# dafyddstephenson/ucla-roms

Hardware: AMD Instinct MI355X
Metric: grid-cell-updates/sec (higher is better)
Workload: dtype f64; 1 GPU; C3: basin 1024x1024x100, NONLIN+SPLIT EOS, T+S, LMD KPP/BKPP/RIMIX/NONLOCAL, dt=300s, ndtfast=60 (nfast=82); NT=2, nfast=82, parallelism=domain decomposition 1x1, halo_transport=none (single rank), fast_exchange_interval=1, exchange_order=none (single rank), s2d_window=True, comm_bootstrap=none (single rank)

## Files before the change

include/roms_gpu.h:

```cpp
#ifndef ROMS_GPU_H
#define ROMS_GPU_H

#ifdef __cplusplus
extern "C" {
#endif

#define ROMS_GPU_ABI_VERSION 21
#define ROMS_MAX_FAST 288

typedef struct roms_dims {
  int Lm, Mm, N, NT;
  int LLm, MMm;
  int np_xi, np_eta, inode, jnode;
  int iSW_corn, jSW_corn;
  int ew_periodic, ns_periodic;
  int west_exchng, east_exchng, south_exchng, north_exchng;
} roms_dims;

#define ROMS_LMD_MIXING   1
#define ROMS_LMD_KPP      2
#define ROMS_LMD_BKPP     4
#define ROMS_LMD_RIMIX    8
#define ROMS_LMD_CONVEC   16
#define ROMS_LMD_NONLOCAL 32
#define ROMS_LMD_ALL      63
#define ROMS_LMD_ICELAND  47
#define ROMS_LMD_DDMIX    64

typedef struct roms_cfg {
  int nonlin_eos;
  int salinity;
  int lmd_mixing;
  int uv_vis2, ts_dif2;
  double dt;
  int ndtfast, nfast;
  double weight[2][ROMS_MAX_FAST];
  double g, rho0, rdrg, rdrg2, Zob, gamma2;
  double Akv_bak, Akt_bak[2];
  double Tcoef, T0, Scoef, S0;
  double theta_s, theta_b, hc;
  int obc;
  double ubind;
  int curvgrid;
  int uv_adv, uv_cor;
  int pot_tides;
  int bulk_frc;
  int adv_isoneutral;
} roms_cfg;

typedef struct roms_tlev {
  int iic, ntstart, forw_start, iif, nfast, kstp, knew, nstp, nrhs, nnew;
} roms_tlev;

enum roms_field {
  ROMS_ALL = -1,
  ROMS_h = 0, ROMS_hinv, ROMS_f, ROMS_fomn, ROMS_pm, ROMS_pn, ROMS_dm_r, ROMS_dn_r, ROMS_dm_u, ROMS_dn_u,
  ROMS_dm_v, ROMS_dn_v, ROMS_dm_p, ROMS_dn_p, ROMS_pmon_u, ROMS_pnom_v, ROMS_rmask, ROMS_pmask, ROMS_umask,
  ROMS_vmask,
  ROMS_Cs_w, ROMS_Cs_r,
  ROMS_zeta, ROMS_ubar, ROMS_vbar, ROMS_u, ROMS_v, ROMS_t, ROMS_FlxU, ROMS_FlxV, ROMS_We, ROMS_Wi,
  ROMS_Hz, ROMS_Hz_u, ROMS_Hz_v, ROMS_z_r, ROMS_z_w,
  ROMS_rufrc, ROMS_rvfrc, ROMS_rhoA, ROMS_rhoS, ROMS_r_D, ROMS_Zt_avg1, ROMS_DU_avg1, ROMS_DV_avg1,
  ROMS_DU_avg2, ROMS_DV_avg2, ROMS_DU_avg_bak, ROMS_DV_avg_bak,
  ROMS_rho, ROMS_rho1, ROMS_qp1, ROMS_bvf, ROMS_Akv, ROMS_Akt, ROMS_visc2_r, ROMS_visc2_p, ROMS_diff2,
  ROMS_hbls, ROMS_hbbl, ROMS_ghat, ROMS_swr_frac,
  ROMS_sustr, ROMS_svstr, ROMS_stflx, ROMS_srflx, ROMS_swflx,
  ROMS_ru, ROMS_rv,
  ROMS_zeta_west, ROMS_zeta_east, ROMS_zeta_south, ROMS_zeta_north,
  ROMS_ubar_west, ROMS_ubar_east, ROMS_ubar_south, ROMS_ubar_north,
  ROMS_vbar_west, ROMS_vbar_east, ROMS_vbar_south, ROMS_vbar_north,
  ROMS_u_west, ROMS_u_east, ROMS_u_south, ROMS_u_north,
  ROMS_v_west, ROMS_v_east, ROMS_v_south, ROMS_v_north,
  ROMS_t_west, ROMS_t_east, ROMS_t_south, ROMS_t_north,
  ROMS_dndx, ROMS_dmde,
  ROMS_ptide,
  ROMS_uwnd, ROMS_vwnd, ROMS_tair, ROMS_qair, ROMS_prate, ROMS_swrad, ROMS_lwrad, ROMS_sustr_r, ROMS_svstr_r,
  ROMS_NFIELDS
};

int  roms_gpu_abi_version(void);
int  roms_gpu_init(const roms_dims *dims, const roms_cfg *cfg, int device, void *comm);
int  roms_gpu_finalize(void);
const char *roms_gpu_last_error(void);
long roms_gpu_field_size(int field_id);
int  roms_gpu_register(int field_id, double *host_ptr, long count);
int  roms_gpu_upload(int field_id);
int  roms_gpu_download(int field_id);
int  roms_gpu_copy_in(int field_id, const double *src, long count);
int  roms_gpu_copy_out(int field_id, double *dst, long count);
int  roms_gpu_sync(void);
void *roms_gpu_stream(void);

int roms_gpu_rho_eos(int tidx, const roms_tlev *t);
int roms_gpu_set_huv(const roms_tlev *t);
int roms_gpu_omega(const roms_tlev *t);
int roms_gpu_lmd_vmix(int tind, const roms_tlev *t);
int roms_gpu_prsgrd(const roms_tlev *t);
int roms_gpu_pre_step3d(const roms_tlev *t);
int roms_gpu_set_huv1(const roms_tlev *t);
int roms_gpu_step3d_uv1(const roms_tlev *t);
int roms_gpu_visc3d(const roms_tlev *t);
int roms_gpu_step2d(const roms_tlev *t);
int roms_gpu_step3d_uv2(const roms_tlev *t);
int roms_gpu_step3d_t(const roms_tlev *t);
int roms_gpu_t3dmix(const roms_tlev *t);
int roms_gpu_swr_frac(const roms_tlev *t);
int roms_gpu_set_pipe_frc(int npip, const int *pipe_idx, const double *pipe_flx, const double *pipe_prf,
                          const double *pipe_trc);
int roms_gpu_set_river_frc(int nriv, const double *riv_uflx, const double *riv_vflx, const double *riv_vol,
                           const double *riv_trc);
int roms_gpu_bulk_flux(const roms_tlev *t);
int roms_gpu_set_ub_tune(const double *ub_west, const double *ub_east, const double *ub_south, const double *ub_north);
int roms_gpu_set_depth(const roms_tlev *t);

int roms_gpu_step(roms_tlev *t);
int roms_gpu_init_sequence(roms_tlev *t);

enum roms_case_id { ROMS_CASE_FILAMENT = 0, ROMS_CASE_BASIN = 1, ROMS_CASE_PIPES = 2, ROMS_CASE_RIVERS = 3 };
typedef struct roms_case {
  int case_id, LLm, MMm, N, NT;
  int salinity, nonlin_eos, lmd_mixing;
  double dt; int ndtfast;
  double sizex, sizey;
  int surf_flux;
  int obc;
  double v_sponge;
  int island;
  int curvgrid;
  int uv_adv, uv_cor;
  int bulk_frc;
  int adv_isoneutral;
} roms_case;
int roms_gpu_init_case(const roms_case *c, int device, roms_tlev *t);
int roms_gpu_init_case_comm(const roms_case *c, int np_xi, int np_eta, void *comm, int device, roms_tlev *t);

int roms_gpu_comm_unique_id(void *id128);
int roms_gpu_comm_create(const void *id128, int nranks, int rank, int device, void **comm);
int roms_gpu_comm_create_local(int group, int nranks, int rank, void **comm);
typedef int (*roms_host_allgather_fn)(void *ctx, const void *send, long nbytes, void *recv);
int roms_gpu_comm_create_host(int nranks, int rank, int device, roms_host_allgather_fn allgather, void *ctx,
                              void **comm);
int roms_gpu_comm_destroy(void *comm);
int roms_gpu_halo_transport(void);
int roms_gpu_halo_exchanges(long *per_step, int *fast_interval);
int roms_gpu_halo_overlap(void);
int roms_gpu_s2d_window(void);
#define ROMS_COLPATH_SEG 1
#define ROMS_COLPATH_GLOBAL 2
int roms_gpu_column_path(void);
int roms_gpu_kpp_lean(void);
int roms_gpu_vgrid(void);
int roms_gpu_vgrid2(void);
int roms_gpu_vgrid_check(long out[3]);
int roms_gpu_horizontal_path(int out[8]);
int roms_gpu_selftest_zero_fill(long n, int chunks, long *bad);
int roms_gpu_halo_plan(int Lm, int Mm, int np_xi, int np_eta, int inode, int jnode, int ew_periodic,
                       int ns_periodic, int peer[8], long count[8], int strip[4]);
long roms_gpu_halo_map(int Lm, int Mm, int np_xi, int np_eta, int inode, int jnode, int ew_periodic,
                       int ns_periodic, int dir, int unpack, int *i, int *j, long cap);
long roms_gpu_halo_map_wide(int Lm, int Mm, int np_xi, int np_eta, int inode, int jnode, int ew_periodic,
                            int ns_periodic, int width, int dir, int unpack, int *i, int *j, long cap);

#define ROMS_FRC_SURFACE 1
#define ROMS_FRC_BRY     2
int roms_gpu_frc_record(int field_id, int slot, double rec_time, const double *data);
int roms_gpu_frc_interp(double modtime, int kinds);
int roms_gpu_frc_clock(double start_time, int on);
int roms_gpu_set_tide_data(int ntides, const double *ftide, const double *pot_re, const double *pot_im,
                           const double *ztide_re, const double *ztide_im, const double *utide_re,
                           const double *utide_im, const double *vtide_re, const double *vtide_im);
int roms_gpu_set_tides(double time);

#define ROMS_WRT_Z    1
#define ROMS_WRT_UB   2
#define ROMS_WRT_VB   4
#define ROMS_WRT_U    8
#define ROMS_WRT_V    16
#define ROMS_WRT_T    32
#define ROMS_WRT_R    64
#define ROMS_WRT_O    128
#define ROMS_WRT_AKV  256
#define ROMS_WRT_AKT  512
#define ROMS_WRT_AKS  1024
#define ROMS_WRT_HBLS 2048
#define ROMS_WRT_HBBL 4096
#define ROMS_WRT_DEFAULT 63
int roms_gpu_wrt_rst(const char *path, int rec, int total_rec, double time, const roms_tlev *t);
int roms_gpu_wrt_his(const char *path, int rec, int total_rec, double time, const roms_tlev *t, int wrt_mask);
int roms_gpu_io_wait(void);
int roms_gpu_io_tracer_name(int itrc, const char *name, const char *units, const char *long_name);
int roms_gpu_get_init(const char *path, int req_rec, int tindx, roms_tlev *t, double *start_time);

int roms_gpu_diag(const roms_tlev *t, double norms[4]);
int roms_gpu_set_weights(int ndtfast, double weight[2][ROMS_MAX_FAST]);
int roms_gpu_time_steps(roms_tlev *t, int n, double *ms);
enum roms_routine {
  ROMS_R_RHO_EOS = 0, ROMS_R_SET_HUV, ROMS_R_OMEGA, ROMS_R_PRSGRD, ROMS_R_PRE_STEP3D, ROMS_R_SET_HUV1,
  ROMS_R_STEP3D_UV1, ROMS_R_VISC3D, ROMS_R_STEP2D, ROMS_R_STEP3D_UV2, ROMS_R_STEP3D_T, ROMS_R_T3DMIX,
  ROMS_R_LMD_VMIX,
  ROMS_R_K_S2D_FB,
  ROMS_R_K_PRE_UV_SEG,
  ROMS_R_K_UV1_SEG,
  ROMS_R_K_STEP3D_T_SEG,
  ROMS_R_K_PRSGRD_UV,
  ROMS_R_K_HALO_PACK,
  ROMS_R_K_HALO_WAIT,
  ROMS_R_K_HALO_UNPACK,
  ROMS_R_COUNT
};
int roms_gpu_time_routine(int routine, int nsteps, roms_tlev *t, double *avg_ms, long *launches);

#ifdef __cplusplus
}
#endif
#endif
```

ucla-roms_amd/csrc/k_colseg.h:

```cpp
#pragma once
#include "k_common.h"

namespace roms {


struct SegSpan {
  int s, S, c0, n;
  int col;
  int row;
  int l;
};
template <int CW = kSegCW>
__device__ __forceinline__ SegSpan seg_span(int N) {
  SegSpan r;
  const int t = (int)(threadIdx.x + blockDim.x * threadIdx.y);
  r.col = t % CW;
  r.row = (int)threadIdx.z;
  r.l = r.col + CW * r.row;
  r.s = t / CW;
  r.S = (int)(blockDim.x * blockDim.y) / CW;
  const int base = N / r.S, rem = N % r.S;
  r.c0 = 1 + r.s * base + min(r.s, rem);
  r.n = base + (r.s < rem ? 1 : 0);
  return r;
// ... 72 lines not shown
#ifndef ROMS_SEG_FASTDIV
#define ROMS_SEG_FASTDIV 1
#endif
#if ROMS_SEG_FASTDIV
#define SEG_DIV(a, b) ((a) * seg_rcp(b))
#else
#define SEG_DIV(a, b) ((a) / (b))
#endif

template <int KR>
struct SegTri {
  double C[KR], D[KR], E[KR];
  template <int G = kSegLoadGroup, class RowF>
  __device__ __forceinline__ void eliminate(int n, RowF row) {
    double Cp = 0.0, Dp = 0.0, Ep = 1.0;
#pragma unroll
    for (int q = 0; q < KR; q++) {
      double a, b, c, d;
      row(q, a, b, c, d);
      const double rm = seg_rcp(b - a * Cp);
      const double Cq = c * rm, Dq = (d - a * Dp) * rm, Eq = -a * Ep * rm;
      const bool live = seg_live(q, n);
      C[q] = live ? Cq : 0.0;
      D[q] = live ? Dq : 0.0;
      E[q] = live ? Eq : 0.0;
      Cp = C[q]; Dp = D[q]; Ep = E[q];
      if (q % G == G - 1) __builtin_amdgcn_sched_barrier(0);
    }
  }
  __device__ __forceinline__ void couple(const SegSpan& sp, int n, SegXchg& X, double& xL, double& xR) {
    const int s = sp.s, S = sp.S, l = sp.l;
    double y = 0.0, al = 0.0, be = 0.0, yl = 0.0, all = 0.0, bel = 0.0;
#pragma unroll
    for (int q = KR - 1; q >= 0; q--) {
      const bool last = seg_last(q, n), live = seg_live(q, n);
      const double yn = D[q] - C[q] * y, aln = E[q] - C[q] * al, ben = -C[q] * be;
      y = last ? D[q] : (live ? yn : y);
      al = last ? E[q] : (live ? aln : al);
      be = last ? -C[q] : (live ? ben : be);
      yl = last ? D[q] : yl;
      all = last ? E[q] : all;
      bel = last ? -C[q] : bel;
    }
    X.v[0][s][l] = y; X.v[1][s][l] = al; X.v[2][s][l] = be;
    X.v[3][s][l] = yl; X.v[4][s][l] = all; X.v[5][s][l] = bel;
    __syncthreads();
    double Pp = 0.0, Qp = 0.0, Ps = 0.0, Qs = 0.0, Us = 0.0, Vs = 0.0, ga = 0.0, gb = 1.0;
#pragma unroll
    for (int t = 0; t < kSegMaxS; t++) {
      if (t < S) {
        const double yf = X.v[0][t][l], af = X.v[1][t][l], bf = X.v[2][t][l];
        const double yL = X.v[3][t][l], aL = X.v[4][t][l], bL = X.v[5][t][l];
        const double rden = seg_rcp(1.0 - af * Qp);
        const double Ut = (yf + af * Pp) * rden;
        const double Vt = bf * rden;
        Us = t == s ? Ut : Us;
        Vs = t == s ? Vt : Vs;
        const double gan = ga + gb * Ut, gbn = gb * Vt;
        ga = t > s ? gan : ga;
        gb = t > s ? gbn : gb;
        const double Pn = yL + aL * Pp + aL * Qp * Ut;
        Qp = aL * Qp * Vt + bL;
        Pp = Pn;
        Ps = t == s - 1 ? Pp : Ps;
        Qs = t == s - 1 ? Qp : Qs;
      }
      if (t % kSegCoupleGroup == kSegCoupleGroup - 1) __builtin_amdgcn_sched_barrier(0);
    }
    xR = ga;
    xL = Ps + Qs * (Us + Vs * ga);
  }
  __device__ __forceinline__ void solve(int n, double xL, double xR) {
    double xn = xR;
#pragma unroll
    for (int q = KR - 1; q >= 0; q--) {
      const double v = D[q] + E[q] * xL - C[q] * xn;
      const bool live = seg_live(q, n);
      xn = live ? v : xn;
      D[q] = live ? v : D[q];
    }
  }
};

template <int KR>
__device__ __forceinline__ void spline_fc_seg(const SegSpan& sg, int N, SegXchg& X, const double (&w)[KR + 1],
                                              const double (&f)[KR], double (&fc)[KR]) {
  const int c0 = sg.c0, n = sg.n;
  const int ns = n + (sg.s == sg.S - 1 ? 1 : 0);
  SegTri<KR> T;
  T.eliminate(ns, [&](int q, double& a, double& bb, double& c, double& dd) {
    const int r = c0 - 1 + q;
    const int q1 = q + 1 < KR ? q + 1 : KR - 1;
    const double ai = w[q + 1], bi = 2.0 * (w[q] + w[q + 1]), ci = w[q];
    const double di = 3.0 * (w[q] * f[q1] + w[q + 1] * f[q]);
    a = r == 0 ? 0.0 : (r == N ? 1.0 : ai);
    bb = (r == 0 || r == N) ? 1.0 : bi;
    c = r == 0 ? 1.0 : (r == N ? 0.0 : ci);
    dd = r == 0 ? 2.0 * f[1] : (r == N ? 2.0 * f[q] : di);
  });
  double xL, xR;
  T.couple(sg, ns, X, xL, xR);
  T.solve(ns, xL, xR);
#pragma unroll
  for (int q = 0; q < KR; q++) fc[q] = seg_live(q, ns) ? T.D[q] : xR;
}

struct NoSplineRow {
  __device__ __forceinline__ void operator()(int, long, double, double, double) const {}
};
template <int KR, class RowF = NoSplineRow>
__device__ __forceinline__ void uv_spline_seg(const Dev& d, const SegSpan& sg, SegXchg& X, long ij, int nrhs, int dir,
                                              double (&fl)[KR], RowF row = RowF()) {
  const Bounds& b = d.b;
  const Fields& F = d.f;
  const int N = b.N, c0 = sg.c0, n = sg.n;
  if (!d.p.uv_adv) {
#pragma unroll
    for (int q = 0; q < KR; q++) fl[q] = 0.0;
    return;
  }
  const long n2 = b.n2, s = dir == 0 ? 1 : b.nx2;
  const double* __restrict__ Uv = (dir == 0 ? F.u : F.v) + (long)(nrhs - 1) * b.n3 + ij;
  const double* __restrict__ Hz = F.Hz + ij;
  const double* __restrict__ We = F.We + ij;
  const double* mask = dir == 0 ? F.umask : F.vmask;
  double dc[KR + 1], uu[KR];
#pragma unroll
  for (int q = 0; q < KR + 1; q++) {
    const long L = (long)(min(max(c0 - 1 + q, 1), N) - 1) * n2;
    const double h0 = Hz[L], h1 = Hz[L - s];
    dc[q] = 0.5625 * (h0 + h1) - 0.0625 * (Hz[L + s] + Hz[L - 2 * s]);
    if (q < KR) uu[q] = Uv[L];
    row(q, L, h0, h1, q < KR ? uu[q] : 0.0);
    if (q % kSegLoadGroup == kSegLoadGroup - 1) __builtin_amdgcn_sched_barrier(0);
  }
  spline_fc_seg<KR>(sg, N, X, dc, uu, fl);
  const double m1 = mask[ij + s], m0 = mask[ij - s];
  double wf[KR];
#pragma unroll
  for (int q = 0; q < KR; q++) {
    const long w = (long)min(max(c0 - 1 + q, 1), N - 1) * n2;
    wf[q] = We[w] + We[w - s] - 0.125 * ((We[w + s] - We[w]) * m1 - (We[w - s] - We[w - 2 * s]) * m0);
    if (q % kSegLoadGroup == kSegLoadGroup - 1) __builtin_amdgcn_sched_barrier(0);
  }
#pragma unroll
  for (int q = 0; q < KR; q++) pin(wf[q]);
#pragma unroll
  for (int q = 0; q < KR; q++) {
    const int r = c0 - 1 + q;
    fl[q] = (r == 0 || r == N) ? 0.0 : fl[q] * 0.5 * wf[q];
  }
}

struct NoSplineRowB {
  __device__ __forceinline__ void operator()(int, unsigned, double, double, double) const {}
};
template <int KR, class RowF = NoSplineRowB>
__device__ __forceinline__ void uv_spline_segb(const Dev& d, const SegSpan& sg, SegXchg& X, long ij, int nrhs, int dir,
                                               double (&fl)[KR], RowF row = RowF()) {
  const Bounds& b = d.b;
  const Fields& F = d.f;
  const int N = b.N, c0 = sg.c0, n = sg.n;
  if (!d.p.uv_adv) {
#pragma unroll
    for (int q = 0; q < KR; q++) fl[q] = 0.0;
    return;
  }
  const long s = dir == 0 ? 1 : b.nx2;
  const unsigned lv = (unsigned)b.n2 * 8u, vo = (unsigned)ij * 8u, ds = (unsigned)s * 8u;
  const unsigned vm = vo - ds, vp = vo + ds, vm2 = vo - 2u * ds;
  const BufF64 Uv((dir == 0 ? F.u : F.v) + (long)(nrhs - 1) * b.n3), Hz(F.Hz), We(F.We);
  const double* mask = dir == 0 ? F.umask : F.vmask;
  auto LD = [&](const BufF64& B, unsigned v, unsigned l) { return B.ld(v + l, 0u); };
  double dc[KR + 1], uu[KR];
#pragma unroll
  for (int q = 0; q < KR + 1; q++) {
    const unsigned L = (unsigned)(min(max(c0 - 1 + q, 1), N) - 1) * lv;
    const double h0 = LD(Hz, vo, L), h1 = LD(Hz, vm, L);
    dc[q] = 0.5625 * (h0 + h1) - 0.0625 * (LD(Hz, vp, L) + LD(Hz, vm2, L));
    if (q < KR) uu[q] = LD(Uv, vo, L);
    row(q, L, h0, h1, q < KR ? uu[q] : 0.0);
    if (q % kSegLoadGroup == kSegLoadGroup - 1) __builtin_amdgcn_sched_barrier(0);
  }
  spline_fc_seg<KR>(sg, N, X, dc, uu, fl);
  const double m1 = mask[ij + s], m0 = mask[ij - s];
  double wf[KR];
#pragma unroll
  for (int q = 0; q < KR; q++) {
    const unsigned w = (unsigned)min(max(c0 - 1 + q, 1), N - 1) * lv;
    const double we0 = LD(We, vo, w), wem = LD(We, vm, w);
    wf[q] = we0 + wem - 0.125 * ((LD(We, vp, w) - we0) * m1 - (wem - LD(We, vm2, w)) * m0);
    if (q % kSegLoadGroup == kSegLoadGroup - 1) __builtin_amdgcn_sched_barrier(0);
  }
#pragma unroll
  for (int q = 0; q < KR; q++) pin(wf[q]);
#pragma unroll
  for (int q = 0; q < KR; q++) {
    const int r = c0 - 1 + q;
    fl[q] = (r == 0 || r == N) ? 0.0 : fl[q] * 0.5 * wf[q];
  }
}

template <int KR>
__device__ __forceinline__ void tracer_spline_seg(const SegSpan& sg, int N, long n2, SegXchg& X,
                                                  const double (&hz)[KR + 1], const double (&tt)[KR],
                                                  const double* __restrict__ We, double (&fl)[KR]) {
  spline_fc_seg<KR>(sg, N, X, hz, tt, fl);
  double we[KR];
#pragma unroll
  for (int q = 0; q < KR; q++) we[q] = We[(long)min(max(sg.c0 - 1 + q, 1), N - 1) * n2];
#pragma unroll
  for (int q = 0; q < KR; q++) pin(we[q]);
#pragma unroll
  for (int q = 0; q < KR; q++) {
    const int r = sg.c0 - 1 + q;
    fl[q] = (r == 0 || r == N) ? 0.0 : fl[q] * we[q];
  }
}

struct SegCol {
  int i, j, dir;
  bool act, idle;
};
__device__ __forceinline__ void seg_uv_col(const Dev& d, const Range& R, const uint3& bI, const SegSpan& sg,
                                           SegCol& c) {
  const Bounds& b = d.b;
  c.dir = (int)bI.z;
  const int ilo = c.dir == 0 ? b.istrU : b.istr;
  const int jlo = c.dir == 1 ? (b.jstrV > R.j0 ? b.jstrV : R.j0) : R.j0;
  const int iu = tile_i0(R.i0) + (int)bI.x * kSegCW + sg.col;
  const int ju = R.j0 + (int)bI.y * (int)blockDim.z + sg.row;
  c.idle = R.j0 + (int)bI.y * (int)blockDim.z > R.j1;
  c.act = iu >= ilo && iu <= R.i1 && ju >= jlo && ju <= R.j1;
  c.i = iu < ilo ? ilo : (iu > R.i1 ? R.i1 : iu);
  c.j = ju < jlo ? jlo : (ju > R.j1 ? R.j1 : ju);
}
inline dim3 seg_grid_of(const Range& R, int nz, int jrows = 1) {
  return dim3((R.i1 - tile_i0(R.i0) + kSegCW) / kSegCW, (R.j1 - R.j0 + jrows) / jrows, nz);
}
inline dim3 seg_uv_grid(const Dev& d, const Range& R, int jrows) { return seg_grid_of(R, 2, jrows); }

}
```

ucla-roms_amd/csrc/k_pre_step3d.hip:

```cpp
#include "k_colseg.h"

namespace roms {

struct PreCoef {
  double dtau, cf_stp, cf_bak;
};

__global__ void __launch_bounds__(256) k_pre_tracer_h(Dev d, Range R, PreCoef c, int nstp, int nnew, int nrhs) {
  const uint3 bI = xcd_tile();
  __shared__ TracerWin W;
  const Bounds& b = d.b;
  const Fields& F = d.f;
  const int k = 1 + (int)bI.z, indx = 3 - nstp;
  const int i0 = tile_i0(R.i0) + (int)bI.x * kBX, j0 = R.j0 + (int)bI.y * kBY;
  const int ib = i0 - 2, jb = j0 - 2;
  const long kk = (long)(k - 1) * b.n2;
  tracer_win_fill(b, F, W, ib, jb, kk, nullptr);
  const int i = i0 + (int)threadIdx.x, j = j0 + (int)threadIdx.y;
  const bool act = i >= R.i0 && i <= R.i1 && j <= R.j1;
  const long ij = IJ(b, i, j), o = ij + kk;
  double hb = 0.0;
  if (act) {
    double hf;
    hz_bak_fwd(d, i, j, k, 0.5 * c.dtau, hb, hf);
    F.c2[o] = hf;
    F.c3[o] = hb;
  }
  const bool in = act && i >= b.istr && j >= b.jstr;
  const double hz = in ? F.Hz[o] : 0.0;
  const AccTL a{W.T, W.UM, W.VM, W.FU, W.FV, ib, jb};
  for (int itrc = 1; itrc <= b.NT; itrc++) {
    const long tb = (long)(itrc - 1) * 3 * b.n3;
    const double* Tr = F.t + (long)(nrhs - 1) * b.n3 + tb;
    __syncthreads();
    tracer_win_fill(b, F, W, ib, jb, kk, Tr);
    __syncthreads();
    if (!in) continue;
    double* Tn = F.t + (long)(nnew - 1) * b.n3 + tb;
    double* Ti = F.t + (long)(indx - 1) * b.n3 + tb;
    const double* Ts = F.t + (long)(nstp - 1) * b.n3 + tb;
    double FX0 = tracer_fx(b, a, i, j, false), FX1 = tracer_fx(b, a, i + 1, j, false);
    double FE0 = tracer_fe(b, a, i, j, false), FE1 = tracer_fe(b, a, i, j + 1, false);
    if (d.p.nriv > 0) {
      river_tracer_flux(d, 0, i, j, k, itrc, FX0); river_tracer_flux(d, 0, i + 1, j, k, itrc, FX1);
      river_tracer_flux(d, 1, i, j, k, itrc, FE0); river_tracer_flux(d, 1, i, j + 1, k, itrc, FE1);
    }
    const double tsk = Ts[o];
    Tn[o] = hb * (c.cf_stp * tsk + c.cf_bak * Ti[o]) - c.dtau * F.pm[ij] * F.pn[ij] * (FX1 - FX0 + FE1 - FE0);
    Ti[o] = hz * tsk;
  }
}

template <int NTT>
struct TracerWinN {
  static constexpr int kN = kUVW * (kBY + 4);
  double UM[kN], VM[kN], FU[kN], FV[kN], T[NTT][kN];
};
template <int NTT, bool kHB>
__global__ void __launch_bounds__(kBX * kBY) k_pre_tracer_h1(Dev d, Range R, PreCoef c, int nstp, int nnew, int nrhs) {
  const uint3 bI = xcd_tile();
  __shared__ TracerWinN<NTT> W;
  const Bounds& b = d.b;
  const Fields& F = d.f;
  const int k = 1 + (int)bI.z, indx = 3 - nstp;
  const int i0 = tile_i0(R.i0) + (int)bI.x * kBX, j0 = R.j0 + (int)bI.y * kBY;
  const int ib = i0 - 2, jb = j0 - 2;
  const long kk = (long)(k - 1) * b.n2, n2 = b.n2;
  const int tid = threadIdx.x + kBX * threadIdx.y;
  constexpr int NW = kUVW * (kBY + 4), NR = (NW + kBX * kBY - 1) / (kBX * kBY);
  double wUM[NR], wVM[NR], wFU[NR], wFV[NR], wT[NTT][NR];
#pragma unroll
  for (int r = 0; r < NR; r++) {
    const int q = tid + r * kBX * kBY;
    const int i = ib + q % kUVW, j = jb + q / kUVW;
    const bool ok = q < NW && i >= -1 && i <= b.Lm + 2 && j >= -1 && j <= b.Mm + 2;
    const long o = ok ? IJ(b, i, j) : 0;
    wUM[r] = ok ? F.umask[o] : 0.0;
    wVM[r] = ok ? F.vmask[o] : 0.0;
    wFU[r] = ok ? F.FlxU[o + kk] : 0.0;
    wFV[r] = ok ? F.FlxV[o + kk] : 0.0;
#pragma unroll
    for (int t = 0; t < NTT; t++)
      wT[t][r] = ok ? F.t[(long)(nrhs - 1) * b.n3 + (long)t * 3 * b.n3 + o + kk] : 0.0;
  }
  const int i = i0 + (int)threadIdx.x, j = j0 + (int)threadIdx.y;
  const bool act = i >= R.i0 && i <= R.i1 && j <= R.j1;
  const bool in = act && i >= b.istr && j >= b.jstr;
  const long ij = act ? IJ(b, i, j) : IJ(b, R.i0, R.j0), o = ij + kk, w = ij + (long)k * n2;
  const bool formed = kHB && in;
  double fu0 = 0.0, fu1 = 0.0, fv0 = 0.0, fv1 = 0.0, we1 = 0.0, wi1 = 0.0, we0 = 0.0, wi0 = 0.0, hbo = 0.0;
  if (formed) {
    hbo = F.c3[o];
  } else {
    fu0 = F.FlxU[o]; fu1 = F.FlxU[o + 1]; fv0 = F.FlxV[o]; fv1 = F.FlxV[o + b.nx2];
    we1 = F.We[w]; wi1 = F.Wi[w]; we0 = F.We[w - n2]; wi0 = F.Wi[w - n2];
  }
  const double pm = F.pm[ij], pn = F.pn[ij], hzo = F.Hz[o];
  double ts[NTT], ti[NTT];
#pragma unroll
  for (int t = 0; t < NTT; t++) {
    const long tb = (long)t * 3 * b.n3;
    ts[t] = F.t[(long)(nstp - 1) * b.n3 + tb + o];
    ti[t] = F.t[(long)(indx - 1) * b.n3 + tb + o];
  }
#pragma unroll
  for (int r = 0; r < NR; r++) {
    const int q = tid + r * kBX * kBY;
    if (q < NW) {
      W.UM[q] = wUM[r]; W.VM[q] = wVM[r]; W.FU[q] = wFU[r]; W.FV[q] = wFV[r];
#pragma unroll
      for (int t = 0; t < NTT; t++) W.T[t][q] = wT[t][r];
    }
  }
  __syncthreads();
  if (!act) return;
  double hb;
  if (formed) {
    hb = hbo;
  } else {
    const double cff = 0.5 * c.dtau;
    const double FlxDiv = cff * pm * pn * (fu1 - fu0 + fv1 - fv0 + we1 + wi1 - we0 - wi0);
    hb = hzo + FlxDiv;
    const double hf = hzo - FlxDiv;
    F.c2[o] = hf;
    F.c3[o] = hb;
  }
  if (!in) return;
  const double hz = hzo;
#pragma unroll
  for (int t = 0; t < NTT; t++) {
    const int itrc = t + 1;
    const AccTL a{W.T[t], W.UM, W.VM, W.FU, W.FV, ib, jb};
    double FX0 = tracer_fx(b, a, i, j, false), FX1 = tracer_fx(b, a, i + 1, j, false);
    double FE0 = tracer_fe(b, a, i, j, false), FE1 = tracer_fe(b, a, i, j + 1, false);
    if (d.p.nriv > 0) {
      river_tracer_flux(d, 0, i, j, k, itrc, FX0); river_tracer_flux(d, 0, i + 1, j, k, itrc, FX1);
      river_tracer_flux(d, 1, i, j, k, itrc, FE0); river_tracer_flux(d, 1, i, j + 1, k, itrc, FE1);
    }
    const long tb = (long)t * 3 * b.n3;
    const double tsk = ts[t];
    F.t[(long)(nnew - 1) * b.n3 + tb + o] =
        hb * (c.cf_stp * tsk + c.cf_bak * ti[t]) - c.dtau * pm * pn * (FX1 - FX0 + FE1 - FE0);
    F.t[(long)(indx - 1) * b.n3 + tb + o] = hz * tsk;
  }
}

template <int NTT>
struct TracerRing {
  double UM[kRingH * kUVW], VM[kRingH * kUVW], FU[kRingH * kUVW], FV[kRingH * kUVW], T[NTT][kRingH * kUVW];
};
template <int NTT, int NR>
struct TracerRows {
  double um[NR], vm[NR], fu[NR], fv[NR], t[NTT][NR];
  __device__ __forceinline__ void load(const Bounds& b, const Fields& F, int tid, int ib, int r0, int nr, long kk,
                                       long tlev) {
#pragma unroll
    for (int m = 0; m < NR; m++) {
      const int q = tid + m * kBX * kBY;
      const int i = ib + q % kUVW, j = r0 + q / kUVW;
      const bool ok = q < nr * kUVW && i >= -1 && i <= b.Lm + 2 && j >= -1 && j <= b.Mm + 2;
      const long o = ok ? IJ(b, i, j) : 0;
      um[m] = ok ? F.umask[o] : 0.0;
      vm[m] = ok ? F.vmask[o] : 0.0;
      fu[m] = ok ? F.FlxU[o + kk] : 0.0;
      fv[m] = ok ? F.FlxV[o + kk] : 0.0;
#pragma unroll
      for (int t = 0; t < NTT; t++) this->t[t][m] = ok ? F.t[tlev + (long)t * 3 * b.n3 + o + kk] : 0.0;
    }
  }
  __device__ __forceinline__ void store(TracerRing<NTT>& W, int tid, int r0, int nr, int jb) const {
#pragma unroll
    for (int m = 0; m < NR; m++) {
      const int q = tid + m * kBX * kBY;
      if (q < nr * kUVW) {
        const int s = (q % kUVW) + ((r0 + q / kUVW - jb) & (kRingH - 1)) * kUVW;
        W.UM[s] = um[m]; W.VM[s] = vm[m]; W.FU[s] = fu[m]; W.FV[s] = fv[m];
#pragma unroll
        for (int t = 0; t < NTT; t++) W.T[t][s] = this->t[t][m];
      }
    }
  }
};
template <int NTT, bool kHB>
__global__ void __launch_bounds__(kBX * kBY) k_pre_tracer_hj(Dev d, Range R, PreCoef c, int nstp, int nnew, int nrhs,
                                                           int jc) {
  const uint3 bI = xcd_tile();
  __shared__ TracerRing<NTT> W;
  const Bounds& b = d.b;
  const Fields& F = d.f;
  const int k = 1 + (int)bI.z, indx = 3 - nstp;
  const int i0 = tile_i0(R.i0) + (int)bI.x * kBX, jc0 = R.j0 + (int)bI.y * jc;
  const int jend = min(jc0 + jc - 1, R.j1);
  const int ib = i0 - 2, jb = jc0 - 2;
  const long kk = (long)(k - 1) * b.n2, n2 = b.n2, tlev = (long)(nrhs - 1) * b.n3;
  const int tid = threadIdx.x + kBX * threadIdx.y;
  constexpr int NT = kBX * kBY;
  constexpr int NR0 = (kRingH * kUVW + NT - 1) / NT, NR4 = (kBY * kUVW + NT - 1) / NT;
  struct Lane {
    double fu0, fu1, fv0, fv1, we1, wi1, we0, wi0, hbo, pm, pn, hzo, ts[NTT], ti[NTT];
  };
  const int i = i0 + (int)threadIdx.x;
  auto load_lane = [&](Lane& L, int j) {
    const bool act = i >= R.i0 && i <= R.i1 && j <= jend;
    const bool formed = kHB && act && i >= b.istr && j >= b.jstr;
    const long ij = act ? IJ(b, i, j) : IJ(b, R.i0, R.j0), o = ij + kk, w = ij + (long)k * n2;
    L.fu0 = L.fu1 = L.fv0 = L.fv1 = L.we1 = L.wi1 = L.we0 = L.wi0 = L.hbo = 0.0;
    if (formed) {
      L.hbo = F.c3[o];
// ... 411 lines not shown
}

template <class C>
__global__ void __launch_bounds__(64) k_pre_uv(Dev d, Range R, PreCoef c, int nstp, int nnew, int nrhs) {
  ROMS_IJC_OR_RETURN(R)
  col_lds_poison<C>(2, d.b.N);
  const Bounds& b = d.b;
  const long ij = IJ(b, i, j);
  const C A = ColMake<C>::at(d, 0, (int)bI.z, ij), B = ColMake<C>::at(d, 1, (int)bI.z, ij);
  if (bI.z == 0) {
    if (i >= b.istrU && i <= b.iend && j >= b.jstr && j <= b.jend) pre_uv_col(d, i, j, 0, c, nstp, nnew, nrhs, A, B);
  } else {
    if (i >= b.istr && i <= b.iend && j >= b.jstrV && j <= b.jend) pre_uv_col(d, i, j, 1, c, nstp, nnew, nrhs, A, B);
  }
}

__global__ void __launch_bounds__(kSegBlock, 2) k_pre_tracer_seg(Dev d, Range R, PreCoef c, int nnew, int nrhs) {
  const uint3 bI = seg_tile(d.p.seg_order, d.p.seg_xg);
  __shared__ SegXchg X;
  constexpr int KR = kSegRows + 1;
  const Bounds& b = d.b;
  const Fields& F = d.f;
  const int N = b.N;
  const SegSpan sg = seg_span(N);
  const int iu = tile_i0(R.i0) + (int)bI.x * kSegCW + sg.col;
  const bool act = iu >= R.i0 && iu <= R.i1;
  const int i = act ? iu : (iu < R.i0 ? R.i0 : R.i1), j = R.j0 + (int)bI.y;
  const int itrc = 1 + (int)bI.z;
  const long n2 = b.n2, ij = IJ(b, i, j);
  const int c0 = sg.c0, n = sg.n;
  auto cell = [&](int k) { return (long)(min(max(k, 1), N) - 1) * n2; };
  const double* __restrict__ Hz = F.Hz + ij;
  const double* __restrict__ Hf = F.c2 + ij;
  const long tb = (long)(itrc - 1) * 3 * b.n3;
  const double* __restrict__ Tr = F.t + (long)(nrhs - 1) * b.n3 + tb + ij;
  double* __restrict__ Tn = F.t + (long)(nnew - 1) * b.n3 + tb + ij;
  double hz[KR + 1], tt[KR], fl[KR];
#pragma unroll
  for (int q = 0; q < KR + 1; q++) {
    hz[q] = Hz[cell(c0 - 1 + q)];
    if (q < KR) tt[q] = Tr[cell(c0 - 1 + q)];
  }
  tracer_spline_seg<KR>(sg, N, n2, X, hz, tt, F.We + ij, fl);
  __builtin_amdgcn_sched_barrier(0);
#pragma unroll
  for (int q = 0; q < KR + 1; q++) hz[q] = Hf[cell(c0 - 1 + q)];
  const int iAkt = itrc < b.nTS ? itrc : b.nTS;
  const double* __restrict__ Akt = F.Akt + (long)(iAkt - 1) * b.n3w + ij;
  const double* __restrict__ Wi = F.Wi + ij;
  const double DC0 = c.dtau * F.pm[ij] * F.pn[ij];
  auto fcw = [&](int q, double& fc, double& wc) {
    const int r = c0 - 1 + q;
    const long w = (long)min(max(r, 1), N - 1) * n2;
    const bool in = r > 0 && r < N;
    const int qa = q + 1 < KR + 1 ? q + 1 : KR;
    const double f = SEG_DIV(2.0 * c.dtau * Akt[w], hz[qa] + hz[q]);
    const double wv = DC0 * Wi[w];
    fc = in ? f : 0.0;
    wc = in ? wv : 0.0;
  };
  double fcl, wcl;
  fcw(0, fcl, wcl);
  __syncthreads();
  SegTri<KR> T;
  T.eliminate(n, [&](int p, double& a, double& bb, double& cc, double& dd) {
    double fcu, wcu;
    fcw(p + 1, fcu, wcu);
    a = -(fcl + fmax0(wcl));
    bb = hz[p + 1] + fcu + fmax0(wcu) + fcl - fmin0(wcl);
    cc = -(fcu - fmin0(wcu));
    dd = Tn[cell(c0 + p)] - c.dtau * F.pm[ij] * F.pn[ij] * (fl[p + 1 < KR ? p + 1 : KR - 1] - fl[p]);
    fcl = fcu; wcl = wcu;
  });
  double xL, xR;
  T.couple(sg, n, X, xL, xR);
  T.solve(n, xL, xR);
  if (act) {
#pragma unroll
    for (int p = 0; p < KR; p++)
      if (p < n) Tn[cell(c0 + p)] = T.D[p];
  }
}

__global__ void __launch_bounds__(kSegBlock, ROMS_PRE_T_SEG_WAVES) k_pre_tracer_segb(Dev d, Range R, PreCoef c, int nnew,
                                                                                   int nrhs) {
  const uint3 bI = seg_tile(d.p.seg_order, d.p.seg_xg);
  __shared__ SegXchg X;
  constexpr int KR = kSegRows + 1;
  const Bounds& b = d.b;
  const Fields& F = d.f;
  const int N = b.N;
  const SegSpan sg = seg_span(N);
  auto LD = [&](const BufF64& B, unsigned v, unsigned l) { return B.ld(v + l, 0u); };
  const int iu = tile_i0(R.i0) + (int)bI.x * kSegCW + sg.col;
  const bool act = iu >= R.i0 && iu <= R.i1;
  const int i = act ? iu : (iu < R.i0 ? R.i0 : R.i1), j = R.j0 + (int)bI.y;
  const int itrc = 1 + (int)bI.z;
  const long n2 = b.n2, ij = IJ(b, i, j);
  const int c0 = sg.c0, n = sg.n;
  const unsigned vo = (unsigned)ij * 8u;
  auto lev = [&](int k) { return (unsigned)(min(max(k, 1), N) - 1) * (unsigned)n2 * 8u; };
  auto wlev = [&](int r) { return (unsigned)min(max(r, 1), N - 1) * (unsigned)n2 * 8u; };
  const BufF64 Hz(F.Hz), Hf(F.c2), We(F.We), Wi(F.Wi);
  const long tb = (long)(itrc - 1) * 3 * b.n3;
  const BufF64 Tr(F.t + (long)(nrhs - 1) * b.n3 + tb), Tn(F.t + (long)(nnew - 1) * b.n3 + tb);
  double hz[KR + 1], tt[KR], fl[KR];
#pragma unroll
  for (int q = 0; q < KR + 1; q++) {
    hz[q] = LD(Hz, vo, lev(c0 - 1 + q));
    if (q < KR) tt[q] = LD(Tr, vo, lev(c0 - 1 + q));
  }
  spline_fc_seg<KR>(sg, N, X, hz, tt, fl);
  {
    double we[KR];
#pragma unroll
    for (int q = 0; q < KR; q++) we[q] = LD(We, vo, wlev(c0 - 1 + q));
#pragma unroll
    for (int q = 0; q < KR; q++) pin(we[q]);
#pragma unroll
    for (int q = 0; q < KR; q++) {
      const int r = c0 - 1 + q;
      fl[q] = (r == 0 || r == N) ? 0.0 : fl[q] * we[q];
    }
  }
  __builtin_amdgcn_sched_barrier(0);
#pragma unroll
  for (int q = 0; q < KR + 1; q++) hz[q] = LD(Hf, vo, lev(c0 - 1 + q));
  const int iAkt = itrc < b.nTS ? itrc : b.nTS;
  const BufF64 Akt(F.Akt + (long)(iAkt - 1) * b.n3w);
  const BufF64 Pm(F.pm), Pn(F.pn);
  const double pm = LD(Pm, vo, 0), pn = LD(Pn, vo, 0);
  const double DC0 = c.dtau * pm * pn;
  auto fcw = [&](int q, double& fc, double& wc) {
    const int r = c0 - 1 + q;
    const unsigned w = wlev(r);
    const bool in = r > 0 && r < N;
    const int qa = q + 1 < KR + 1 ? q + 1 : KR;
    const double f = SEG_DIV(2.0 * c.dtau * LD(Akt, vo, w), hz[qa] + hz[q]);
    const double wv = DC0 * LD(Wi, vo, w);
    fc = in ? f : 0.0;
    wc = in ? wv : 0.0;
  };
  double fcl, wcl;
  fcw(0, fcl, wcl);
  __syncthreads();
  SegTri<KR> T;
  T.eliminate(n, [&](int p, double& a, double& bb, double& cc, double& dd) {
    double fcu, wcu;
    fcw(p + 1, fcu, wcu);
    a = -(fcl + fmax0(wcl));
    bb = hz[p + 1] + fcu + fmax0(wcu) + fcl - fmin0(wcl);
    cc = -(fcu - fmin0(wcu));
    dd = LD(Tn, vo, lev(c0 + p)) - c.dtau * pm * pn * (fl[p + 1 < KR ? p + 1 : KR - 1] - fl[p]);
    fcl = fcu; wcl = wcu;
  });
  double xL, xR;
  T.couple(sg, n, X, xL, xR);
  T.solve(n, xL, xR);
  const unsigned vs = act ? vo : kBufOff;
#pragma unroll
  for (int p = 0; p < KR; p++)
    if (p < n) Tn.st(T.D[p], vs + lev(c0 + p), 0u);
}

template <bool kLds>
__global__ void __launch_bounds__(kSegBlock * kSegJMax, 2) k_pre_uv_seg(Dev d, Range R, PreCoef c, int nstp, int nnew, int nrhs) {
  const uint3 bI = seg_tile(d.p.seg_order, d.p.seg_xg);
  __shared__ SegXchg X;
  constexpr int KR = kSegRows + 1;
  const Bounds& b = d.b;
  const Fields& F = d.f;
  const int N = b.N, indx = 3 - nstp;
  const SegSpan sg = seg_span(N);
  SegCol col;
  seg_uv_col(d, R, bI, sg, col);
  if (col.idle) return;
  const int dir = col.dir;
  const bool act = col.act;
  const long n2 = b.n2, ij = IJ(b, col.i, col.j), s = dir == 0 ? 1 : b.nx2;
  const int c0 = sg.c0, n = sg.n;
  auto cell = [&](int k) { return (long)(min(max(k, 1), N) - 1) * n2; };
  double* Uall = dir == 0 ? F.u : F.v;
  const int nthr = (int)(blockDim.x * blockDim.y * blockDim.z);
  const int tid = (int)(threadIdx.x + blockDim.x * (threadIdx.y + blockDim.y * threadIdx.z));
  double* const Sb = roms_smem + tid;
  double* const Su = roms_smem + (long)(KR - 1) * nthr + tid;
  double fl[KR];
  if constexpr (kLds) {
    const double* __restrict__ Uix = Uall + (long)(indx - 1) * b.n3 + ij;
    uv_spline_seg<KR>(d, sg, X, ij, nrhs, dir, fl, [&](int q, long L, double h0, double h1, double u) {
      if (q >= 1 && q < KR) {
        Sb[(q - 1) * nthr] = c.cf_stp * u + c.cf_bak * Uix[L];
        Su[(q - 1) * nthr] = 0.5 * (h0 + h1) * u;
      }
    });
  } else {
    uv_spline_seg<KR>(d, sg, X, ij, nrhs, dir, fl);
  }
  __builtin_amdgcn_sched_barrier(0);
  const double* __restrict__ rr = (dir == 0 ? F.ru : F.rv) + ij;
  const double* __restrict__ Ustp = Uall + (long)(nstp - 1) * b.n3 + ij;
  double* __restrict__ Uidx = Uall + (long)(indx - 1) * b.n3 + ij;
  double* __restrict__ Unew = Uall + (long)(nnew - 1) * b.n3 + ij;
  const double* __restrict__ Hz = F.Hz + ij;
  const double* __restrict__ Akv = F.Akv + ij;
  const double* __restrict__ Wi = F.Wi + ij;
  const double* __restrict__ Hf = F.c2 + ij;
  const double* __restrict__ Hb = F.c3 + ij;
  const double sstr = dir == 0 ? F.sustr[ij] : F.svstr[ij];
  const double DC0 = c.dtau * 0.25 * (F.pm[ij] + F.pm[ij - s]) * (F.pn[ij] + F.pn[ij - s]);
  auto rhs = [&](int p) {
    const int k = c0 + p;
    const long o = cell(k);
    const double r = k == 1 ? rr[o] - fl[1] : rr[o] - fl[p + 1 < KR ? p + 1 : KR - 1] + fl[p];
    double ub;
    if constexpr (kLds) ub = Sb[(p < KR - 1 ? p : KR - 2) * nthr];
    else ub = c.cf_stp * Ustp[o] + c.cf_bak * Uidx[o];
    const double v = 0.5 * (Hb[o] + Hb[o - s]) * ub + DC0 * r;
    return k == N ? v + c.dtau * sstr : v;
  };
  double hf[KR + 1], hfm[KR + 1];
#pragma unroll
  for (int q = 0; q < KR + 1; q++) {
    const long L = cell(c0 - 1 + q);
    hf[q] = Hf[L];
    hfm[q] = Hf[L - s];
  }
  auto fcw = [&](int q, double& fc, double& wc) {
    const int r = c0 - 1 + q;
    const long w = (long)min(max(r, 1), N - 1) * n2;
    const bool in = r > 0 && r < N;
    const int qa = q + 1 < KR + 1 ? q + 1 : KR;
    const double f = SEG_DIV(2.0 * c.dtau * (Akv[w] + Akv[w - s]), hf[qa] + hfm[qa] + hf[q] + hfm[q]);
    const double wv = DC0 * 0.5 * (Wi[w] + Wi[w - s]);
    fc = in ? f : 0.0;
    wc = in ? wv : 0.0;
  };
  const double rd = F.r_D[ij], rdm = F.r_D[ij - s];
  double fcl, wcl;
  fcw(0, fcl, wcl);
  __syncthreads();
  SegTri<KR> T;
  T.eliminate(n, [&](int p, double& a, double& bb, double& cc, double& dd) {
    double fcu, wcu;
    fcw(p + 1, fcu, wcu);
    const int k = c0 + p;
    a = -(fcl + fmax0(wcl));
    cc = -(fcu - fmin0(wcu));
    const double b1 = 0.5 * (hf[p + 1] + hfm[p + 1]) + 0.5 * c.dtau * (rd + rdm) + fcu + fmax0(wcu);
    const double bk = 0.5 * (hf[p + 1] + hfm[p + 1]) + fcl - fmin0(wcl) + fcu + fmax0(wcu);
    bb = k == 1 ? b1 : bk;
    dd = rhs(p);
    fcl = fcu; wcl = wcu;
  });
  double xL, xR;
  T.couple(sg, n, X, xL, xR);
  T.solve(n, xL, xR);
  if (act) {
    double uix[KR];
#pragma unroll
    for (int p = 0; p < KR; p++) {
      const long o = cell(c0 + p);
      if constexpr (kLds) uix[p] = Su[(p < KR - 1 ? p : KR - 2) * nthr];
      else uix[p] = 0.5 * (Hz[o] + Hz[o - s]) * Ustp[o];
    }
#pragma unroll
    for (int p = 0; p < KR; p++)
      if (p < n) {
        Unew[cell(c0 + p)] = T.D[p];
        Uidx[cell(c0 + p)] = uix[p];
      }
  }
}

__global__ void __launch_bounds__(kSegBlock * kSegJMax, 2) k_pre_uv_segb(Dev d, Range R, PreCoef c, int nstp, int nnew,
                                                                         int nrhs) {
  const uint3 bI = seg_tile(d.p.seg_order, d.p.seg_xg);
  __shared__ SegXchg X;
  constexpr int KR = kSegRows + 1;
  const Bounds& b = d.b;
  const Fields& F = d.f;
  const int N = b.N, indx = 3 - nstp;
  const SegSpan sg = seg_span(N);
  auto LD = [&](const BufF64& B, unsigned v, unsigned l) { return B.ld(v + l, 0u); };
  SegCol col;
  seg_uv_col(d, R, bI, sg, col);
  if (col.idle) return;
  const int dir = col.dir;
  const bool act = col.act;
  const long n2 = b.n2, ij = IJ(b, col.i, col.j), s = dir == 0 ? 1 : b.nx2;
  const int c0 = sg.c0, n = sg.n;
  const unsigned lv = (unsigned)n2 * 8u, vo = (unsigned)ij * 8u, vm = vo - (unsigned)s * 8u;
  auto lev = [&](int k) { return (unsigned)(min(max(k, 1), N) - 1) * lv; };
  double* Uall = dir == 0 ? F.u : F.v;
  const int nthr = (int)(blockDim.x * blockDim.y * blockDim.z);
  const int tid = (int)(threadIdx.x + blockDim.x * (threadIdx.y + blockDim.y * threadIdx.z));
  double* const Sb = roms_smem + tid;
  double* const Su = roms_smem + (long)(KR - 1) * nthr + tid;
  const BufF64 Uix(Uall + (long)(indx - 1) * b.n3), Unew(Uall + (long)(nnew - 1) * b.n3), Hf(F.c2);
  double hf[KR + 1], hfm[KR + 1];
  double fl[KR];
  uv_spline_segb<KR>(d, sg, X, ij, nrhs, dir, fl, [&](int q, unsigned L, double h0, double h1, double u) {
    if (q >= 1 && q < KR) {
      Sb[(q - 1) * nthr] = c.cf_stp * u + c.cf_bak * LD(Uix, vo, L);
      Su[(q - 1) * nthr] = 0.5 * (h0 + h1) * u;
    }
  });
  __builtin_amdgcn_sched_barrier(0);
  const BufF64 rr(dir == 0 ? F.ru : F.rv), Akv(F.Akv), Wi(F.Wi), Hb(F.c3);
  const double sstr = dir == 0 ? F.sustr[ij] : F.svstr[ij];
  const double DC0 = c.dtau * 0.25 * (F.pm[ij] + F.pm[ij - s]) * (F.pn[ij] + F.pn[ij - s]);
  auto rhs = [&](int p) {
    const int k = c0 + p;
    const unsigned o = lev(k);
    const double rro = LD(rr, vo, o);
    const double r = k == 1 ? rro - fl[1] : rro - fl[p + 1 < KR ? p + 1 : KR - 1] + fl[p];
    const double ub = Sb[(p < KR - 1 ? p : KR - 2) * nthr];
    const double v = 0.5 * (LD(Hb, vo, o) + LD(Hb, vm, o)) * ub + DC0 * r;
    return k == N ? v + c.dtau * sstr : v;
  };
#pragma unroll
  for (int q = 0; q < KR + 1; q++) {
    const unsigned L = lev(c0 - 1 + q);
    hf[q] = LD(Hf, vo, L);
    hfm[q] = LD(Hf, vm, L);
  }
  auto fcw = [&](int q, double& fc, double& wc) {
    const int r = c0 - 1 + q;
    const unsigned w = (unsigned)min(max(r, 1), N - 1) * lv;
    const bool in = r > 0 && r < N;
    const int qa = q + 1 < KR + 1 ? q + 1 : KR;
    const double f = SEG_DIV(2.0 * c.dtau * (LD(Akv, vo, w) + LD(Akv, vm, w)), hf[qa] + hfm[qa] + hf[q] + hfm[q]);
    const double wv = DC0 * 0.5 * (LD(Wi, vo, w) + LD(Wi, vm, w));
    fc = in ? f : 0.0;
    wc = in ? wv : 0.0;
  };
  const double rd = F.r_D[ij], rdm = F.r_D[ij - s];
  double fcl, wcl;
  fcw(0, fcl, wcl);
  __syncthreads();
  SegTri<KR> T;
  T.eliminate(n, [&](int p, double& a, double& bb, double& cc, double& dd) {
    double fcu, wcu;
    fcw(p + 1, fcu, wcu);
    const int k = c0 + p;
    a = -(fcl + fmax0(wcl));
    cc = -(fcu - fmin0(wcu));
    const double b1 = 0.5 * (hf[p + 1] + hfm[p + 1]) + 0.5 * c.dtau * (rd + rdm) + fcu + fmax0(wcu);
    const double bk = 0.5 * (hf[p + 1] + hfm[p + 1]) + fcl - fmin0(wcl) + fcu + fmax0(wcu);
    bb = k == 1 ? b1 : bk;
    dd = rhs(p);
    fcl = fcu; wcl = wcu;
  });
  double xL, xR;
  T.couple(sg, n, X, xL, xR);
  T.solve(n, xL, xR);
  const unsigned vs = act ? vo : kBufOff;
#pragma unroll
  for (int p = 0; p < KR; p++)
    if (p < n) {
      const unsigned o = lev(c0 + p);
      Unew.st(T.D[p], vs + o, 0u);
      Uix.st(Su[(p < KR - 1 ? p : KR - 2) * nthr], vs + o, 0u);
    }
}

static size_t pre_uv_seg_lds_bytes(unsigned nthr) {
  return (size_t)2 * kSegRows * nthr * sizeof(double);
}
void setup_pre_uv_seg() {
  (void)hipFuncSetAttribute((const void*)k_pre_uv_seg<true>, hipFuncAttributeMaxDynamicSharedMemorySize,
                            (int)pre_uv_seg_lds_bytes(kSegBlock * kSegJMax));
  (void)hipFuncSetAttribute((const void*)k_pre_uv_segb, hipFuncAttributeMaxDynamicSharedMemorySize,
                            (int)pre_uv_seg_lds_bytes(kSegBlock * kSegJMax));
}

void setup_column_kernels_t(size_t bytes);
void setup_column_kernels_uv1(size_t bytes);
bool setup_column_kernels(int N) {
  const size_t bytes = col_lds_bytes(2, N);
  if (bytes > 160 * 1024) return false;
  if (bytes > 64 * 1024) {
    (void)hipFuncSetAttribute((const void*)k_pre_tracer_v<ColLds>, hipFuncAttributeMaxDynamicSharedMemorySize,
                              (int)bytes);
    (void)hipFuncSetAttribute((const void*)k_pre_uv<ColLds>, hipFuncAttributeMaxDynamicSharedMemorySize, (int)bytes);
    setup_column_kernels_t(bytes);
    setup_column_kernels_uv1(bytes);
  }
  return true;
}

double pre_step3d_dtau(const Dev& d, const Tlev& t) {
  const double AM3_crv = 1.0 / 6.0;
  return t.iic == t.forw_start ? 0.5 * d.p.dt : d.p.dt * (1.0 - AM3_crv);
}

void launch_pre_step3d(const Dev& d, hipStream_t s, const Tlev& t, bool uv_done, bool hb_done, const Side* side) {
  const Bounds& b = d.b;
  PreCoef c;
  const double AM3_crv = 1.0 / 6.0;
  if (t.iic == t.forw_start) { c.dtau = 0.5 * d.p.dt; c.cf_stp = 1.0; c.cf_bak = 0.0; }
  else { c.dtau = d.p.dt * (1.0 - AM3_crv); c.cf_stp = 0.5 + AM3_crv; c.cf_bak = 0.5 - AM3_crv; }
  c.dtau = pre_step3d_dtau(d, t);
  hb_done = hb_done && d.p.hoist && b.NT <= 2;
  Range RI{b.istr, b.iend, b.jstr, b.jend};
  Range RH{b.istr - 1, b.iend, b.jstr - 1, b.jend};
  auto horiz_tiles = [&](const Range& rh) {
    const dim3 gh = grid3_of(rh, b.N), bh(kBX, kBY);
    if (d.p.hoist && d.p.h_jc > 0 && (b.NT == 1 || b.NT == 2)) {
      const dim3 g = grid3_jc(rh, b.N, d.p.h_jc);
      const int jc = d.p.h_jc;
      if (b.NT == 2 && hb_done)
        hipLaunchKernelGGL((k_pre_tracer_hj<2, true>), g, bh, 0, s, d, rh, c, t.nstp, t.nnew, t.nrhs, jc);
      else if (b.NT == 2)
        hipLaunchKernelGGL((k_pre_tracer_hj<2, false>), g, bh, 0, s, d, rh, c, t.nstp, t.nnew, t.nrhs, jc);
      else if (hb_done)
        hipLaunchKernelGGL((k_pre_tracer_hj<1, true>), g, bh, 0, s, d, rh, c, t.nstp, t.nnew, t.nrhs, jc);
      else
        hipLaunchKernelGGL((k_pre_tracer_hj<1, false>), g, bh, 0, s, d, rh, c, t.nstp, t.nnew, t.nrhs, jc);
    } else if (d.p.hoist && b.NT == 2 && hb_done)
      hipLaunchKernelGGL((k_pre_tracer_h1<2, true>), gh, bh, 0, s, d, rh, c, t.nstp, t.nnew, t.nrhs);
    else if (d.p.hoist && b.NT == 2)
      hipLaunchKernelGGL((k_pre_tracer_h1<2, false>), gh, bh, 0, s, d, rh, c, t.nstp, t.nnew, t.nrhs);
    else if (d.p.hoist && b.NT == 1 && hb_done)
      hipLaunchKernelGGL((k_pre_tracer_h1<1, true>), gh, bh, 0, s, d, rh, c, t.nstp, t.nnew, t.nrhs);
    else if (d.p.hoist && b.NT == 1)
      hipLaunchKernelGGL((k_pre_tracer_h1<1, false>), gh, bh, 0, s, d, rh, c, t.nstp, t.nnew, t.nrhs);
    else
      hipLaunchKernelGGL(k_pre_tracer_h, gh, bh, 0, s, d, rh, c, t.nstp, t.nnew, t.nrhs);
  };
  {
    int jA = 0, jB = -1;
    if (d.p.hoist && d.p.h_jc == 0 &&
        launch_tracer_strip(d, s, RH, 1, false, hb_done, t.nnew, t.nrhs, c.dtau, c.cf_stp, c.cf_bak, t.nstp, jA, jB)) {
      if (jA > RH.j0) horiz_tiles(Range{RH.i0, RH.i1, RH.j0, jA - 1});
      if (jB < RH.j1) horiz_tiles(Range{RH.i0, RH.i1, jB + 1, RH.j1});
    } else {
      horiz_tiles(RH);
    }
  }
  hipStream_t st = s;
  if (side) {
    (void)hipEventRecord(side->efork, s);
    (void)hipStreamWaitEvent(side->s2, side->efork, 0);
    st = side->s2;
  }
  dim3 gt = gridc_of(RI);
  gt.z = b.NT;
  if (d.p.colseg && d.p.seg_buf)
    hipLaunchKernelGGL(k_pre_tracer_segb, seg_grid_of(RI, b.NT), dim3(kCX, seg_waves(b.N)), 0, st, d, RI, c, t.nnew,
                       t.nrhs);
  else if (d.p.colseg)
    hipLaunchKernelGGL(k_pre_tracer_seg, seg_grid_of(RI, b.NT), dim3(kCX, seg_waves(b.N)), 0, st, d, RI, c, t.nnew,
                       t.nrhs);
  else if ((d.p.colreg & 2) && b.N == 50 && !d.f.colscr)
    hipLaunchKernelGGL(k_pre_tracer_v_reg<50>, gt, dim3(kCX), col_lds_bytes(1, 50), st, d, RI, c, t.nnew, t.nrhs);
  else if (d.f.colscr)
    hipLaunchKernelGGL(k_pre_tracer_v<ColGlb>, gt, dim3(kCX), 0, st, d, RI, c, t.nnew, t.nrhs);
  else
    hipLaunchKernelGGL(k_pre_tracer_v<ColLds>, gt, dim3(kCX), col_lds_bytes(2, b.N), st, d, RI, c, t.nnew, t.nrhs);
  for (int itrc = 1; itrc <= b.NT && side; itrc++) launch_t3dbc(d, st, t, itrc);
  if (side) launch_exchange_tracers(d, st, t.nnew);
  if (!uv_done) launch_uv_horiz(d, s, t.nrhs, 0);
  Range Rd{b.istrU - 1, b.iend, b.jstrV - 1, b.jend};
  hipLaunchKernelGGL(k_rd, grid_of(Rd), dim3(kBX, kBY), 0, s, d, Rd, t.nstp);
  dim3 gu = gridc_of(RI);
  gu.z = 2;
  if (d.p.colseg) {
    const dim3 gs = seg_uv_grid(d, RI, d.p.seg_jrows), bs(kCX, seg_waves(b.N), d.p.seg_jrows);
    const bool lds = d.p.preuv_lds && d.p.uv_adv && t.nrhs == t.nstp;
    ktimer_mark(s, kTimedPreUvSeg, 0);
    if (lds && d.p.seg_buf)
      hipLaunchKernelGGL(k_pre_uv_segb, gs, bs, pre_uv_seg_lds_bytes(bs.x * bs.y * bs.z), s, d, RI, c, t.nstp, t.nnew,
                         t.nrhs);
    else if (lds)
      hipLaunchKernelGGL(k_pre_uv_seg<true>, gs, bs, pre_uv_seg_lds_bytes(bs.x * bs.y * bs.z), s, d, RI, c, t.nstp,
                         t.nnew, t.nrhs);
    else
      hipLaunchKernelGGL(k_pre_uv_seg<false>, gs, bs, 0, s, d, RI, c, t.nstp, t.nnew, t.nrhs);
    ktimer_mark(s, kTimedPreUvSeg, 1, 1);
  }
  else if (d.f.colscr)
    hipLaunchKernelGGL(k_pre_uv<ColGlb>, gu, dim3(kCX), 0, s, d, RI, c, t.nstp, t.nnew, t.nrhs);
  else
    hipLaunchKernelGGL(k_pre_uv<ColLds>, gu, dim3(kCX), col_lds_bytes(2, b.N), s, d, RI, c, t.nstp, t.nnew, t.nrhs);
  launch_river_uv(d, s, t.nnew, 1);
  launch_u3dbc(d, s, t);
  launch_v3dbc(d, s, t);
  if (side) {
    (void)hipEventRecord(side->ejoin, st);
    (void)hipStreamWaitEvent(s, side->ejoin, 0);
    return;
  }
  for (int itrc = 1; itrc <= b.NT; itrc++) launch_t3dbc(d, s, t, itrc);
  launch_exchange_tracers(d, s, t.nnew);
}

}
```

ucla-roms_amd/csrc/k_step3d_t.hip:

```cpp
#include "k_colseg.h"

namespace roms {

__global__ void __launch_bounds__(256) k_step3d_t_h(Dev d, Range R, int nnew, int nrhs, int up) {
  const uint3 bI = xcd_tile();
  __shared__ TracerWin W;
  const Bounds& b = d.b;
  const Fields& F = d.f;
  const int k = 1 + (int)bI.z;
  const int i0 = tile_i0(R.i0) + (int)bI.x * kBX, j0 = R.j0 + (int)bI.y * kBY;
  const int ib = i0 - 2, jb = j0 - 2;
  const long kk = (long)(k - 1) * b.n2;
  tracer_win_fill(b, F, W, ib, jb, kk, nullptr);
  const int i = i0 + (int)threadIdx.x, j = j0 + (int)threadIdx.y;
  const bool act = i >= R.i0 && i <= R.i1 && j <= R.j1;
  const long ij = IJ(b, i, j), o = ij + kk;
  const AccTL a{W.T, W.UM, W.VM, W.FU, W.FV, ib, jb};
  for (int itrc = 1; itrc <= b.NT; itrc++) {
    const long tb = (long)(itrc - 1) * 3 * b.n3;
    const double* Tr = F.t + (long)(nrhs - 1) * b.n3 + tb;
    __syncthreads();
    tracer_win_fill(b, F, W, ib, jb, kk, Tr);
    __syncthreads();
    if (!act) continue;
// ... 231 lines not shown
  const double stf = F.stflx[ij + (long)(itrc - 1) * n2];
  double rhs[KR];
#pragma unroll
  for (int p = 0; p < KR; p++) rhs[p] = Tn[cell(c0 + p)] - dt * F.pm[ij] * F.pn[ij] * (tt[p + 1 < KR ? p + 1 : KR - 1] - tt[p]);
  if (P.npip > 0) {
    const int pidx = F.pipe_idx[ij];
    if (pidx > 0) {
      const double pflx = F.pipe_flx[ij], ptrc = F.pipe_trc[(pidx - 1) + (itrc - 1) * P.npip];
#pragma unroll
      for (int p = 0; p < KR; p++) {
        const int k = min(c0 + p, N);
        rhs[p] = rhs[p] + dt * F.pm[ij] * F.pn[ij] * pflx * F.pipe_prf[(pidx - 1) + (k - 1) * P.npip] * ptrc;
      }
    }
  }
  {
    const bool top = last;
    double t = 0.0;
#pragma unroll
    for (int p = 0; p < KR; p++) t = p == n - 1 ? rhs[p] : t;
    const double swf = F.swflx[ij], hzN = Hz[cell(N)];
    if (itrc == 1) t = t + dt * swf * (P.bulk_frc ? F.tair[ij] : t / hzN);
    t = t + dt * stf;
#pragma unroll
    for (int p = 0; p < KR; p++) rhs[p] = (top && p == n - 1) ? t : rhs[p];
  }
  if (kppT || kppS) {
    auto gh = [&](long o) { return P.lmd_nonlocal ? F.ghat[ij + o] : 0.0; };
#pragma unroll
    for (int p = 0; p < KR; p++) {
      const int k = min(c0 + p, N);
      const long ou = (long)min(k, N - 1) * n2, ol = (long)max(k - 1, 1) * n2;
      double t = rhs[p];
      if (kppT) {
        const double up = dt * (sr * F.swr_frac[ij + ou] - gh(ou) * (stf - sr));
        const double lo = dt * (sr * F.swr_frac[ij + ol] - gh(ol) * (stf - sr));
        t = k <= N - 1 ? t + up : t;
        t = k >= 2 ? t - lo : t;
      } else {
        const double up = -dt * F.ghat[ij + ou] * stf, lo = -dt * F.ghat[ij + ol] * stf;
        t = k <= N - 1 ? t + up : t;
        t = k >= 2 ? t - lo : t;
      }
      rhs[p] = t;
    }
  }
  auto fcw = [&](int q, double& fc, double& wc) {
    const int r = c0 - 1 + q;
    const long w = (long)min(max(r, 1), N - 1) * n2;
    const bool in = r > 0 && r < N;
    const int qa = q + 1 < KR + 1 ? q + 1 : KR;
    const double f = SEG_DIV(2.0 * dt * Akt[w], hz[q] + hz[qa]);
    const double c = DC0 * Wi[w];
    fc = in ? f : 0.0;
    wc = in ? c : 0.0;
  };
  double fcl, wcl;
  fcw(0, fcl, wcl);
  __syncthreads();
  SegTri<KR> T;
  T.eliminate(n, [&](int p, double& a, double& bb, double& c, double& dd) {
    double fcu, wcu;
    fcw(p + 1, fcu, wcu);
    a = -(fcl + fmax0(wcl));
    bb = hz[p + 1] + fcu + fmax0(wcu) + fcl - fmin0(wcl);
    c = -(fcu - fmin0(wcu));
    dd = rhs[p];
    fcl = fcu; wcl = wcu;
  });
  double xL, xR;
  T.couple(sg, n, X, xL, xR);
  T.solve(n, xL, xR);
  if (act) {
    const double rm = F.rmask[ij];
#pragma unroll
    for (int p = 0; p < KR; p++)
      if (p < n) Tn[cell(c0 + p)] = T.D[p] * rm;
  }
}

#ifndef ROMS_SEG_T_GROUP
#define ROMS_SEG_T_GROUP kSegLoadGroup
#endif
__global__ void __launch_bounds__(kSegBlock, ROMS_T_SEG_WAVES) k_step3d_t_segb(Dev d, Range R, int nnew, int nrhs) {
  const uint3 bI = seg_tile(d.p.seg_order, d.p.seg_xg);
  __shared__ SegXchg X;
  constexpr int KR = kSegRows + 1;
  const Bounds& b = d.b;
  const Fields& F = d.f;
  const Params& P = d.p;
  const int N = b.N;
  const double dt = P.dt;
  const SegSpan sg = seg_span(N);
  auto LD = [&](const BufF64& B, unsigned v, unsigned l) { return B.ld(v + l, 0u); };
  const int iu = tile_i0(R.i0) + (int)bI.x * kSegCW + sg.col;
  const bool act = iu >= R.i0 && iu <= R.i1;
  const int i = act ? iu : (iu < R.i0 ? R.i0 : R.i1), j = R.j0 + (int)bI.y;
  const int itrc = 1 + (int)bI.z;
  const long n2 = b.n2, ij = IJ(b, i, j);
  const int c0 = sg.c0, n = sg.n;
  const bool last = sg.s == sg.S - 1;
  const unsigned vo = (unsigned)ij * 8u;
  auto lev = [&](int k) { return (unsigned)(min(max(k, 1), N) - 1) * (unsigned)n2 * 8u; };
  auto wlev = [&](int r, int lo, int hi) { return (unsigned)min(max(r, lo), hi) * (unsigned)n2 * 8u; };
  const BufF64 Hz(F.Hz), We(F.We), Wi(F.Wi);
  const BufF64 Tr(F.t + (long)(nrhs - 1) * b.n3 + (long)(itrc - 1) * 3 * b.n3);
  const BufF64 Tn(F.t + (long)(nnew - 1) * b.n3 + (long)(itrc - 1) * 3 * b.n3);
  double hz[KR + 1], tt[KR], tn[KR];
#pragma unroll
  for (int q = 0; q < KR + 1; q++) {
    hz[q] = LD(Hz, vo, lev(c0 - 1 + q));
    if (q < KR) tt[q] = LD(Tr, vo, lev(c0 - 1 + q));
  }
#pragma unroll
  for (int p = 0; p < KR; p++) tn[p] = LD(Tn, vo, lev(c0 + p));
  {
    double fc[KR];
    spline_fc_seg<KR>(sg, N, X, hz, tt, fc);
    double we[KR];
#pragma unroll
    for (int q = 0; q < KR; q++) we[q] = LD(We, vo, wlev(c0 - 1 + q, 1, N - 1));
#pragma unroll
    for (int q = 0; q < KR; q++) pin(we[q]);
#pragma unroll
    for (int q = 0; q < KR; q++) {
      const int r = c0 - 1 + q;
      tt[q] = (r == 0 || r == N) ? 0.0 : fc[q] * we[q];
    }
  }
  __builtin_amdgcn_sched_barrier(0);
  const int iAkt = itrc < b.nTS ? itrc : b.nTS;
  const BufF64 Akt(F.Akt + (long)(iAkt - 1) * b.n3w);
  const BufF64 Pm(F.pm), Pn(F.pn);
  const double pm = Pm.ld(vo, 0), pn = Pn.ld(vo, 0);
  const double DC0 = dt * pm * pn;
  const bool kppT = P.lmd && itrc == 1, kppS = P.lmd_nonlocal && itrc == 2 && P.salinity;
  const double sr = BufF64(F.srflx).ld(vo, 0);
  const double stf = BufF64(F.stflx).ld(vo, (unsigned)(itrc - 1) * (unsigned)n2 * 8u);
  double rhs[KR];
#pragma unroll
  for (int p = 0; p < KR; p++)
    rhs[p] = tn[p] - dt * pm * pn * (tt[p + 1 < KR ? p + 1 : KR - 1] - tt[p]);
  if (P.npip > 0) {
    const int pidx = F.pipe_idx[ij];
    if (pidx > 0) {
      const double pflx = F.pipe_flx[ij], ptrc = F.pipe_trc[(pidx - 1) + (itrc - 1) * P.npip];
#pragma unroll
      for (int p = 0; p < KR; p++) {
        const int k = min(c0 + p, N);
        rhs[p] = rhs[p] + dt * pm * pn * pflx * F.pipe_prf[(pidx - 1) + (k - 1) * P.npip] * ptrc;
      }
    }
  }
  if (last) {
    double t = 0.0;
#pragma unroll
    for (int p = 0; p < KR; p++) t = p == n - 1 ? rhs[p] : t;
    if (itrc == 1) {
      const double swf = BufF64(F.swflx).ld(vo, 0);
      t = t + dt * swf * (P.bulk_frc ? BufF64(F.tair).ld(vo, 0) : t / LD(Hz, vo, lev(N)));
    }
    t = t + dt * stf;
#pragma unroll
    for (int p = 0; p < KR; p++) rhs[p] = p == n - 1 ? t : rhs[p];
  }
  if (kppT || kppS) {
    const BufF64 Sw(F.swr_frac), Gh(F.ghat);
    const bool nl = P.lmd_nonlocal;
    double swv[KR + 1], ghv[KR + 1];
    if (kppT) {
#pragma unroll
      for (int q = 0; q < KR + 1; q++) {
        const unsigned o = wlev(c0 - 1 + q, 1, N - 1);
        swv[q] = LD(Sw, vo, o);
        ghv[q] = LD(Gh, vo, o);
      }
    } else {
#pragma unroll
      for (int q = 0; q < KR + 1; q++) {
        swv[q] = 0.0;
        ghv[q] = LD(Gh, vo, wlev(c0 - 1 + q, 1, N - 1));
      }
    }
    auto term = [&](int q) {
      return kppT ? dt * (sr * swv[q] - (nl ? ghv[q] : 0.0) * (stf - sr)) : -dt * ghv[q] * stf;
    };
    double lo = term(0);
#pragma unroll
    for (int p = 0; p < KR; p++) {
      const int k = min(c0 + p, N);
      const double up = term(p + 1);
      double t = rhs[p];
      t = k <= N - 1 ? t + up : t;
      t = k >= 2 ? t - lo : t;
      rhs[p] = t;
      lo = up;
    }
  }
  auto fcw = [&](int q, double& fc, double& wc) {
    const int r = c0 - 1 + q;
    const unsigned w = wlev(r, 1, N - 1);
    const bool in = r > 0 && r < N;
    const int qa = q + 1 < KR + 1 ? q + 1 : KR;
    const double f = SEG_DIV(2.0 * dt * LD(Akt, vo, w), hz[q] + hz[qa]);
    const double c = DC0 * LD(Wi, vo, w);
    fc = in ? f : 0.0;
    wc = in ? c : 0.0;
  };
  double fcl, wcl;
  fcw(0, fcl, wcl);
  __syncthreads();
  SegTri<KR> T;
  T.template eliminate<ROMS_SEG_T_GROUP>(n, [&](int p, double& a, double& bb, double& c, double& dd) {
    double fcu, wcu;
    fcw(p + 1, fcu, wcu);
    a = -(fcl + fmax0(wcl));
    bb = hz[p + 1] + fcu + fmax0(wcu) + fcl - fmin0(wcl);
    c = -(fcu - fmin0(wcu));
    dd = rhs[p];
    fcl = fcu; wcl = wcu;
  });
  double xL, xR;
  T.couple(sg, n, X, xL, xR);
  T.solve(n, xL, xR);
  const double rm = BufF64(F.rmask).ld(vo, 0);
  const unsigned vs = act ? vo : kBufOff;
#pragma unroll
  for (int p = 0; p < KR; p++) Tn.st(T.D[p] * rm, (p < n ? vs : kBufOff) + lev(c0 + p), 0u);
}

void setup_column_kernels_t(size_t bytes) {
  (void)hipFuncSetAttribute((const void*)k_step3d_t_v<ColLds>, hipFuncAttributeMaxDynamicSharedMemorySize,
                            (int)bytes);
  (void)hipFuncSetAttribute((const void*)k_step3d_t_v<ColLds, true>, hipFuncAttributeMaxDynamicSharedMemorySize,
                            (int)bytes);
}

void launch_step3d_t(const Dev& d, hipStream_t s, const Tlev& t, bool exchange) {
  const Bounds& b = d.b;
  Range R{b.istr, b.iend, b.jstr, b.jend};
  if (d.p.iso) {
    hipLaunchKernelGGL(k_step3d_t_h, grid3_of(R, b.N), dim3(kBX, kBY), 0, s, d, R, t.nnew, t.nrhs, 0);
    for (int itrc = 1; itrc <= b.NT; itrc++) launch_iso_tracer(d, s, t, itrc);
    dim3 gt = gridc_of(R);
    gt.z = b.NT;
    if (d.f.colscr)
      hipLaunchKernelGGL((k_step3d_t_v<ColGlb, true>), gt, dim3(kCX), 0, s, d, R, t.nnew, t.nrhs);
    else
      hipLaunchKernelGGL((k_step3d_t_v<ColLds, true>), gt, dim3(kCX), col_lds_bytes(2, b.N), s, d, R, t.nnew, t.nrhs);
    for (int itrc = 1; itrc <= b.NT; itrc++) launch_t3dbc(d, s, t, itrc);
    launch_exchange_tracers(d, s, t.nnew);
    return;
  }
  auto h_tiles = [&](const Range& r) {
    const dim3 gh = grid3_of(r, b.N), bh(kBX, kBY);
    if (d.p.hoist && b.NT == 2)
      hipLaunchKernelGGL(k_step3d_t_h1<2>, gh, bh, 0, s, d, r, t.nnew, t.nrhs);
    else if (d.p.hoist && b.NT == 1)
      hipLaunchKernelGGL(k_step3d_t_h1<1>, gh, bh, 0, s, d, r, t.nnew, t.nrhs);
    else
      hipLaunchKernelGGL(k_step3d_t_h, gh, bh, 0, s, d, r, t.nnew, t.nrhs, 1);
  };
  auto run = [&](const Range& r) {
    int jA = 0, jB = -1;
    if (d.p.hoist && launch_tracer_strip(d, s, r, 0, true, false, t.nnew, t.nrhs, 0.0, 0.0, 0.0, 0, jA, jB)) {
      if (jA > r.j0) h_tiles(Range{r.i0, r.i1, r.j0, jA - 1});
      if (jB < r.j1) h_tiles(Range{r.i0, r.i1, jB + 1, r.j1});
    } else {
      h_tiles(r);
    }
    dim3 gt = gridc_of(r);
    gt.z = b.NT;
    if (d.p.colseg) {
      ktimer_mark(s, kTimedStep3dTSeg, 0);
      if (d.p.seg_buf)
        hipLaunchKernelGGL(k_step3d_t_segb, seg_grid_of(r, b.NT), dim3(kCX, seg_waves(b.N)), 0, s, d, r, t.nnew, t.nrhs);
      else
        hipLaunchKernelGGL(k_step3d_t_seg, seg_grid_of(r, b.NT), dim3(kCX, seg_waves(b.N)), 0, s, d, r, t.nnew, t.nrhs);
      ktimer_mark(s, kTimedStep3dTSeg, 1, 1);
    }
    else if (d.f.colscr)
      hipLaunchKernelGGL(k_step3d_t_v<ColGlb>, gt, dim3(kCX), 0, s, d, r, t.nnew, t.nrhs);
    else
      hipLaunchKernelGGL(k_step3d_t_v<ColLds>, gt, dim3(kCX), col_lds_bytes(2, b.N), s, d, r, t.nnew, t.nrhs);
  };
  auto edges = [&] {
    for (int itrc = 1; itrc <= b.NT; itrc++) launch_t3dbc(d, s, t, itrc);
  };
  ExchList L;
  if (!exchange) {
    run(R);
    edges();
  } else if (tracer_exch_list(d, t.nnew, L)) {
    launch_rim_first(d, s, R, L, run, edges);
  } else {
    run(R);
    edges();
    launch_exchange_tracers(d, s, t.nnew);
  }
}

__global__ void __launch_bounds__(256) k_t3dmix(Dev d, Range R, int nnew, int nrhs) {
  ROMS_IJ_OR_RETURN(R)
  const Bounds& b = d.b;
  const Fields& F = d.f;
  const long ij = IJ(b, i, j), sj = b.nx2, n2 = b.n2;
  const double* __restrict__ Hz = F.Hz;
  const double pmn = d.p.dt * F.pm[ij] * F.pn[ij];
  if (b.NT == 2) {
    double ax0[2], ax1[2], ay0[2], ay1[2];
    const double* __restrict__ Tr[2];
    double* __restrict__ Tn[2];
#pragma unroll
    for (int q = 0; q < 2; q++) {
      const double* d2 = F.diff2 + (long)q * n2;
      Tr[q] = F.t + (long)(nrhs - 1) * b.n3 + (long)q * 3 * b.n3;
      Tn[q] = F.t + (long)(nnew - 1) * b.n3 + (long)q * 3 * b.n3;
      ax0[q] = 0.25 * (d2[ij] + d2[ij - 1]) * F.pmon_u[ij];
      ax1[q] = 0.25 * (d2[ij + 1] + d2[ij]) * F.pmon_u[ij + 1];
      ay0[q] = 0.25 * (d2[ij] + d2[ij - sj]) * F.pnom_v[ij];
      ay1[q] = 0.25 * (d2[ij + sj] + d2[ij]) * F.pnom_v[ij + sj];
    }
    const double um0 = F.umask[ij], um1 = F.umask[ij + 1], vm0 = F.vmask[ij], vm1 = F.vmask[ij + sj];
#pragma unroll 2
    for (int k = 1; k <= b.N; k++) {
      const long o = ij + (long)(k - 1) * n2;
#pragma unroll
      for (int q = 0; q < 2; q++) {
        const double FX1 = ax1[q] * (Hz[o + 1] + Hz[o]) * (Tr[q][o + 1] - Tr[q][o]) * um1;
        const double FX0 = ax0[q] * (Hz[o] + Hz[o - 1]) * (Tr[q][o] - Tr[q][o - 1]) * um0;
        const double FE1 = ay1[q] * (Hz[o + sj] + Hz[o]) * (Tr[q][o + sj] - Tr[q][o]) * vm1;
        const double FE0 = ay0[q] * (Hz[o] + Hz[o - sj]) * (Tr[q][o] - Tr[q][o - sj]) * vm0;
        Tn[q][o] = Tn[q][o] + pmn * (FX1 - FX0 + FE1 - FE0) / Hz[o];
      }
    }
    return;
  }
  for (int itrc = 1; itrc <= b.NT; itrc++) {
    const double* d2 = F.diff2 + (long)(itrc - 1) * n2;
    const double* __restrict__ Tr = F.t + (long)(nrhs - 1) * b.n3 + (long)(itrc - 1) * 3 * b.n3;
    double* __restrict__ Tn = F.t + (long)(nnew - 1) * b.n3 + (long)(itrc - 1) * 3 * b.n3;
    const double ax0 = 0.25 * (d2[ij] + d2[ij - 1]) * F.pmon_u[ij], ax1 = 0.25 * (d2[ij + 1] + d2[ij]) * F.pmon_u[ij + 1];
    const double ay0 = 0.25 * (d2[ij] + d2[ij - sj]) * F.pnom_v[ij], ay1 = 0.25 * (d2[ij + sj] + d2[ij]) * F.pnom_v[ij + sj];
    const double um0 = F.umask[ij], um1 = F.umask[ij + 1], vm0 = F.vmask[ij], vm1 = F.vmask[ij + sj];
#pragma unroll 2
    for (int k = 1; k <= b.N; k++) {
      const long o = ij + (long)(k - 1) * n2;
      const double FX1 = ax1 * (Hz[o + 1] + Hz[o]) * (Tr[o + 1] - Tr[o]) * um1;
      const double FX0 = ax0 * (Hz[o] + Hz[o - 1]) * (Tr[o] - Tr[o - 1]) * um0;
      const double FE1 = ay1 * (Hz[o + sj] + Hz[o]) * (Tr[o + sj] - Tr[o]) * vm1;
      const double FE0 = ay0 * (Hz[o] + Hz[o - sj]) * (Tr[o] - Tr[o - sj]) * vm0;
      Tn[o] = Tn[o] + pmn * (FX1 - FX0 + FE1 - FE0) / Hz[o];
    }
  }
}

constexpr int kTMW = kBX + 2, kTMN = kTMW * (kBY + 2), kTMQ = (3 * kTMN + kBX * kBY - 1) / (kBX * kBY);
constexpr int kTMG = (kTMN + kBX * kBY - 1) / (kBX * kBY);
template <bool VG>
// ... 119 lines not shown
```

ucla-roms_amd/csrc/k_step3d_uv.hip:

```cpp
#include <vector>

#include "k_colseg.h"
#include "k_chain.h"

namespace roms {

void launch_uv_horiz(const Dev& d, hipStream_t s, int nrhs, int up);

#ifndef ROMS_UV1_PF
#define ROMS_UV1_PF 8
#endif
constexpr int kUv1PF = ROMS_UV1_PF;
template <class C>
__device__ __forceinline__ void uv1_col(const Dev& d, int i, int j, int dir, int nnew, int nrhs, const C& A,
                                        const C& B) {
  const Bounds& b = d.b;
  const Fields& F = d.f;
  const int N = b.N;
  const double dt = d.p.dt;
  const long n2 = b.n2, ij = IJ(b, i, j);
  const long s = dir == 0 ? 1 : b.nx2;
  uv_vert_flux_lds<(kUv1PF > 0)>(d, ij, nrhs, dir, A, B);
  double* __restrict__ Un = (dir == 0 ? F.u : F.v) + (long)(nnew - 1) * b.n3 + ij;
  double* __restrict__ rr = (dir == 0 ? F.ru : F.rv) + ij;
// ... 160 lines not shown
  if constexpr (!kLds) {
#pragma unroll
    for (int q = 0; q < KR + 1; q++) {
      const long L = cell(c0 - 1 + q);
      hz[q] = Hz[L];
      hzm[q] = Hz[L - s];
    }
  }
  int tl = tid;
  __asm__ volatile("" : "+v"(tl));
  auto HZ = [&](int q) { if constexpr (kLds) return roms_smem[tl + q * nthr]; else return hz[q]; };
  auto HZM = [&](int q) { if constexpr (kLds) return roms_smem[(KR + 1 + q) * nthr + tl]; else return hzm[q]; };
  auto fcw = [&](int q, double& fc, double& wc) {
    const int r = c0 - 1 + q;
    const long w = (long)min(max(r, 1), N - 1) * n2;
    const bool in = r > 0 && r < N;
    const int qa = q + 1 < KR + 1 ? q + 1 : KR;
    const double f = SEG_DIV(2.0 * dt * (Akv[w] + Akv[w - s]), HZ(qa) + HZM(qa) + HZ(q) + HZM(q));
    const double wv = DC0 * 0.5 * (Wi[w] + Wi[w - s]);
    fc = in ? f : 0.0;
    wc = in ? wv : 0.0;
  };
  const double rD = F.r_D[ij], rDm = F.r_D[ij - s];
  double fcl, wcl;
  fcw(0, fcl, wcl);
  __syncthreads();
  SegTri<KR> T;
  T.eliminate(n, [&](int p, double& a, double& bb, double& cc, double& dd) {
    double fcu, wcu;
    fcw(p + 1, fcu, wcu);
    const int k = c0 + p;
    a = -(fcl + fmax0(wcl));
    cc = -(fcu - fmin0(wcu));
    const double b1 = 0.5 * (HZ(p + 1) + HZM(p + 1)) + 0.5 * dt * (rD + rDm) + fcu + fmax0(wcu);
    const double bk = 0.5 * (HZ(p + 1) + HZM(p + 1)) + fcl - fmin0(wcl) + fcu + fmax0(wcu);
    bb = k == 1 ? b1 : bk;
    if constexpr (kLds) {
      const double v = Un[cell(k)] + DC0 * rk[p];
      dd = k == N ? v + dt * sstr : v;
    } else {
      dd = rhs[p];
    }
    fcl = fcu; wcl = wcu;
  });
  double xL, xR;
  T.couple(sg, n, X, xL, xR);
  T.solve(n, xL, xR);
  const double dmdn = dir == 0 ? F.dm_u[ij] * F.dn_u[ij] : F.dm_v[ij] * F.dn_v[ij];
  if constexpr (kLds) {
    const int S = sg.S, sl = sg.l;
    for (int t = 0; t < S; t++) {
      if (sg.s == t) {
        double frc;
        if (t == 0) frc = rk[0] + dmdn * (sstr - 0.5 * (rDm + rD) * T.D[0]);
        else frc = Lf[t - 1][sl] + rk[0];
#pragma unroll
        for (int p = 1; p < KR; p++) frc = p < n ? frc + rk[p] : frc;
        Lf[t][sl] = frc;
      }
      __syncthreads();
    }
    if (!act) return;
#pragma unroll
    for (int p = 0; p < KR; p++)
      if (p < n) Un[cell(c0 + p)] = T.D[p] * 0.5 * (HZ(p + 1) + HZM(p + 1));
    if (sg.s == 0) {
      if (dir == 0) F.rufrc[ij] = Lf[S - 1][sl];
      else F.rvfrc[ij] = Lf[S - 1][sl];
    }
  } else {
    if (!act) return;
#pragma unroll
    for (int p = 0; p < KR; p++)
      if (p < n) Un[cell(c0 + p)] = T.D[p] * 0.5 * (hz[p + 1] + hzm[p + 1]);
    if (sg.s == 0) {
      double frc = Sr[sg.l] + dmdn * (sstr - 0.5 * (rDm + rD) * T.D[0]);
      for (int k = 2; k <= N; k++) frc = frc + Sr[(k - 1) * ncol + sg.l];
      if (dir == 0) F.rufrc[ij] = frc;
      else F.rvfrc[ij] = frc;
    }
  }
}

__global__ void __launch_bounds__(kSegBlock * kSegJMax, 2) k_uv1_segb(Dev d, Range R, int nnew, int nrhs) {
  const uint3 bI = seg_tile(d.p.seg_order, d.p.seg_xg);
  __shared__ SegXchg X;
  __shared__ double Lf[kSegMaxS][kSegCW * kSegJMax];
  constexpr int KR = kSegRows + 1;
  const Bounds& b = d.b;
  const Fields& F = d.f;
  const int N = b.N;
  const double dt = d.p.dt;
  const SegSpan sg = seg_span(N);
  SegCol col;
  seg_uv_col(d, R, bI, sg, col);
  if (col.idle) return;
  const int dir = col.dir;
  const bool act = col.act;
  const long n2 = b.n2, ij = IJ(b, col.i, col.j), s = dir == 0 ? 1 : b.nx2;
  const int c0 = sg.c0, n = sg.n;
  const unsigned lv = (unsigned)n2 * 8u, vo = (unsigned)ij * 8u, vm = vo - (unsigned)s * 8u;
  auto lev = [&](int k) { return (unsigned)(min(max(k, 1), N) - 1) * lv; };
  const int nthr = (int)(blockDim.x * blockDim.y * blockDim.z);
  const int tid = (int)(threadIdx.x + blockDim.x * (threadIdx.y + blockDim.y * threadIdx.z));
  double* const Sh = roms_smem + tid;
  double* const Shm = roms_smem + (long)(KR + 1) * nthr + tid;
  const BufF64 Un((dir == 0 ? F.u : F.v) + (long)(nnew - 1) * b.n3);
  auto LD = [&](const BufF64& B, unsigned v, unsigned l) { return B.ld(v + l, 0u); };
  double fl[KR];
  uv_spline_segb<KR>(d, sg, X, ij, nrhs, dir, fl, [&](int q, unsigned, double h0, double h1, double) {
    Sh[q * nthr] = h0;
    Shm[q * nthr] = h1;
  });
  __builtin_amdgcn_sched_barrier(0);
  const BufF64 rr(dir == 0 ? F.ru : F.rv), Akv(F.Akv), Wi(F.Wi);
  const double sstr = dir == 0 ? F.sustr[ij] : F.svstr[ij];
  const double DC0 = dt * 0.25 * (F.pm[ij] + F.pm[ij - s]) * (F.pn[ij] + F.pn[ij - s]);
  double rk[KR];
#pragma unroll
  for (int p = 0; p < KR; p++) {
    const int k = c0 + p;
    const double rro = LD(rr, vo, lev(k));
    rk[p] = k == 1 ? rro - fl[1] : rro - fl[p + 1 < KR ? p + 1 : KR - 1] + fl[p];
  }
  int tl = tid;
  __asm__ volatile("" : "+v"(tl));
  auto HZ = [&](int q) { return roms_smem[tl + q * nthr]; };
  auto HZM = [&](int q) { return roms_smem[(KR + 1 + q) * nthr + tl]; };
  auto fcw = [&](int q, double& fc, double& wc) {
    const int r = c0 - 1 + q;
    const unsigned w = (unsigned)min(max(r, 1), N - 1) * lv;
    const bool in = r > 0 && r < N;
    const int qa = q + 1 < KR + 1 ? q + 1 : KR;
    const double f = SEG_DIV(2.0 * dt * (LD(Akv, vo, w) + LD(Akv, vm, w)), HZ(qa) + HZM(qa) + HZ(q) + HZM(q));
    const double wv = DC0 * 0.5 * (LD(Wi, vo, w) + LD(Wi, vm, w));
    fc = in ? f : 0.0;
    wc = in ? wv : 0.0;
  };
  const double rD = F.r_D[ij], rDm = F.r_D[ij - s];
  double fcl, wcl;
  fcw(0, fcl, wcl);
  __syncthreads();
  SegTri<KR> T;
  T.eliminate(n, [&](int p, double& a, double& bb, double& cc, double& dd) {
    double fcu, wcu;
    fcw(p + 1, fcu, wcu);
    const int k = c0 + p;
    a = -(fcl + fmax0(wcl));
    cc = -(fcu - fmin0(wcu));
    const double b1 = 0.5 * (HZ(p + 1) + HZM(p + 1)) + 0.5 * dt * (rD + rDm) + fcu + fmax0(wcu);
    const double bk = 0.5 * (HZ(p + 1) + HZM(p + 1)) + fcl - fmin0(wcl) + fcu + fmax0(wcu);
    bb = k == 1 ? b1 : bk;
    const double v = LD(Un, vo, lev(k)) + DC0 * rk[p];
    dd = k == N ? v + dt * sstr : v;
    fcl = fcu; wcl = wcu;
  });
  double xL, xR;
  T.couple(sg, n, X, xL, xR);
  T.solve(n, xL, xR);
  const double dmdn = dir == 0 ? F.dm_u[ij] * F.dn_u[ij] : F.dm_v[ij] * F.dn_v[ij];
  const int S = sg.S, sl = sg.l;
  for (int t = 0; t < S; t++) {
    if (sg.s == t) {
      double frc;
      if (t == 0) frc = rk[0] + dmdn * (sstr - 0.5 * (rDm + rD) * T.D[0]);
      else frc = Lf[t - 1][sl] + rk[0];
#pragma unroll
      for (int p = 1; p < KR; p++) frc = p < n ? frc + rk[p] : frc;
      Lf[t][sl] = frc;
    }
    __syncthreads();
  }
#pragma unroll
  for (int p = 0; p < KR; p++)
    if (p < n) Un.st(T.D[p] * 0.5 * (HZ(p + 1) + HZM(p + 1)), act ? vo + lev(c0 + p) : kBufOff, 0u);
  if (act && sg.s == 0) {
    if (dir == 0) F.rufrc[ij] = Lf[S - 1][sl];
    else F.rvfrc[ij] = Lf[S - 1][sl];
  }
}

void setup_column_kernels_uv1(size_t bytes) {
  (void)hipFuncSetAttribute((const void*)k_uv1<ColLds>, hipFuncAttributeMaxDynamicSharedMemorySize, (int)bytes);
}
static size_t uv1_seg_lds_bytes(unsigned nthr) { return (size_t)2 * (kSegRows + 2) * nthr * sizeof(double); }
void setup_uv1_seg() {
  (void)hipFuncSetAttribute((const void*)k_uv1_seg<false>, hipFuncAttributeMaxDynamicSharedMemorySize,
                            (int)((size_t)kSegRows * kSegMaxS * kSegCW * kSegJMax * sizeof(double)));
  (void)hipFuncSetAttribute((const void*)k_uv1_seg<true>, hipFuncAttributeMaxDynamicSharedMemorySize,
                            (int)uv1_seg_lds_bytes(kSegBlock * kSegJMax));
  (void)hipFuncSetAttribute((const void*)k_uv1_segb, hipFuncAttributeMaxDynamicSharedMemorySize,
                            (int)uv1_seg_lds_bytes(kSegBlock * kSegJMax));
}

void launch_step3d_uv1(const Dev& d, hipStream_t s, const Tlev& t, bool uv_done) {
  const Bounds& b = d.b;
  if (!uv_done) launch_uv_horiz(d, s, t.nrhs, 1);
  Range R{b.istr, b.iend, b.jstr, b.jend};
  dim3 g = gridc_of(R);
  g.z = 2;
  if (d.p.colseg) {
    const dim3 gs = seg_uv_grid(d, R, d.p.seg_jrows), bs(kCX, seg_waves(b.N), d.p.seg_jrows);
    ktimer_mark(s, kTimedUv1Seg, 0);
    if (d.p.uv1_lds && d.p.uv_adv && d.p.seg_buf)
      hipLaunchKernelGGL(k_uv1_segb, gs, bs, uv1_seg_lds_bytes(bs.x * bs.y * bs.z), s, d, R, t.nnew, t.nrhs);
    else if (d.p.uv1_lds && d.p.uv_adv)
      hipLaunchKernelGGL(k_uv1_seg<true>, gs, bs, uv1_seg_lds_bytes(bs.x * bs.y * bs.z), s, d, R, t.nnew, t.nrhs);
    else
      hipLaunchKernelGGL(k_uv1_seg<false>, gs, bs, (size_t)b.N * kSegCW * d.p.seg_jrows * sizeof(double), s, d, R,
                         t.nnew, t.nrhs);
    ktimer_mark(s, kTimedUv1Seg, 1, 1);
  }
  else if (d.f.colscr)
    hipLaunchKernelGGL(k_uv1<ColGlb>, g, dim3(kCX), 0, s, d, R, t.nnew, t.nrhs);
  else
    hipLaunchKernelGGL(k_uv1<ColLds>, g, dim3(kCX), col_lds_bytes(2, b.N), s, d, R, t.nnew, t.nrhs);
}

__device__ __forceinline__ void visc_rho(const Dev& d, int i, int j, int k, int nstp, double& UFx, double& VFe) {
  const Bounds& b = d.b;
  const Fields& F = d.f;
  const long ij = IJ(b, i, j), o = ij + (long)(k - 1) * b.n2, l = (long)(nstp - 1) * b.n3;
  const double* pm = F.pm;
  const double* pn = F.pn;
  const long sj = b.nx2;
  const double cff = 0.5 * F.Hz[o] * F.visc2_r[ij] *
                     (F.dn_r[ij] * pm[ij] * ((pn[ij] + pn[ij + 1]) * F.u[o + 1 + l] - (pn[ij - 1] + pn[ij]) * F.u[o + l]) -
                      F.dm_r[ij] * pn[ij] * ((pm[ij] + pm[ij + sj]) * F.v[o + sj + l] - (pm[ij - sj] + pm[ij]) * F.v[o + l]));
  UFx = cff * F.dn_r[ij] * F.dn_r[ij];
  VFe = -cff * F.dm_r[ij] * F.dm_r[ij];
}
__device__ __forceinline__ void visc_psi(const Dev& d, int i, int j, int k, int nstp, double& UFe, double& VFx) {
  const Bounds& b = d.b;
  const Fields& F = d.f;
  const long sj = b.nx2;
  const long ij = IJ(b, i, j), o = ij + (long)(k - 1) * b.n2, l = (long)(nstp - 1) * b.n3;
  const double* pm = F.pm;
  const double* pn = F.pn;
  const double cff =
      0.125 * (F.Hz[o - 1] + F.Hz[o] + F.Hz[o - 1 - sj] + F.Hz[o - sj]) * F.visc2_p[ij] *
      (0.25 * (pm[ij - 1] + pm[ij] + pm[ij - 1 - sj] + pm[ij - sj]) * F.dn_p[ij] *
           ((pn[ij - sj] + pn[ij]) * F.v[o + l] - (pn[ij - 1 - sj] + pn[ij - 1]) * F.v[o - 1 + l]) +
       0.25 * (pn[ij - 1] + pn[ij] + pn[ij - 1 - sj] + pn[ij - sj]) * F.dm_p[ij] *
           ((pm[ij - 1] + pm[ij]) * F.u[o + l] - (pm[ij - 1 - sj] + pm[ij - sj]) * F.u[o - sj + l])) *
      F.pmask[ij];
  UFe = cff * F.dm_p[ij] * F.dm_p[ij];
  VFx = cff * F.dn_p[ij] * F.dn_p[ij];
}

constexpr int kVW = kBX + 1, kVN = kVW * (kBY + 1), kVQ = (kVN + kBX * kBY - 1) / (kBX * kBY);
struct ViscRho {
  double v2, X, sx1, sx0, Y, sy1, sy0, dn, dm;
  long ij;
  bool on;
};
struct ViscPsi {
  double v2, P1, P2, a1, a0, b1, b0, msk, dm, dn;
  long ij;
  bool on;
};
__global__ void __launch_bounds__(256) k_visc3d(Dev d, Range R, int nstp) {
  const uint3 bI = xcd_tile();
  __shared__ double sUFx[kVN], sVFe[kVN], sUFe[kVN], sVFx[kVN];
  const Bounds& b = d.b;
  const Fields& F = d.f;
  const int indx = 3 - nstp;
  const int i0 = tile_i0(R.i0) + (int)bI.x * kBX, j0 = R.j0 + (int)bI.y * kBY;
  const long sj = b.nx2;
  const double* pm = F.pm;
  const double* pn = F.pn;
  const int tid = threadIdx.x + kBX * threadIdx.y;
  ViscRho gr[kVQ];
  ViscPsi gp[kVQ];
#pragma unroll
  for (int m = 0; m < kVQ; m++) {
    const int q = tid + m * kBX * kBY;
    const int li = q % kVW, lj = q / kVW;
    const int ir = i0 - 1 + li, jr = j0 - 1 + lj;
    ViscRho& r = gr[m];
    r.on = q < kVN && ir >= 0 && ir <= b.Lm + 1 && jr >= 0 && jr <= b.Mm + 1;
    r.ij = IJ(b, ir, jr);
    if (r.on) {
      const long ij = r.ij;
      r.v2 = F.visc2_r[ij];
      r.X = F.dn_r[ij] * pm[ij]; r.sx1 = pn[ij] + pn[ij + 1]; r.sx0 = pn[ij - 1] + pn[ij];
      r.Y = F.dm_r[ij] * pn[ij]; r.sy1 = pm[ij] + pm[ij + sj]; r.sy0 = pm[ij - sj] + pm[ij];
      r.dn = F.dn_r[ij]; r.dm = F.dm_r[ij];
    }
// ... 664 lines not shown
```

ucla-roms_amd/csrc/k_vertical.hip:

```cpp
#include "roms_dev.h"
#include "k_chain.h"
#include "k_colseg.h"

namespace roms {

__global__ void __launch_bounds__(256) k_set_depth(Dev d, Range R, int iic, int knew, int last) {
  ROMS_IJ_OR_RETURN(R)
  const Bounds& b = d.b;
  const Fields& F = d.f;
  const long ij = IJ(b, i, j);
  if (iic == 0) {
    F.hinv[ij] = 1.0 / (F.h[ij] + d.p.hc);
    if (i >= b.istr)
      F.DU_avg1[ij] = 0.5 * (F.h[IJ(b, i - 1, j)] + F.h[ij] + F.zeta[IJL(b, i, j, 1)] + F.zeta[IJL(b, i - 1, j, 1)]) *
                      F.dn_u[ij] * (F.ubar[IJL(b, i, j, 1)]);
    if (j >= b.jstr)
      F.DV_avg1[ij] = 0.5 * (F.h[ij] + F.h[IJ(b, i, j - 1)] + F.zeta[IJL(b, i, j, 1)] + F.zeta[IJL(b, i, j - 1, 1)]) *
                      F.dm_v[ij] * (F.vbar[IJL(b, i, j, 1)]);
  }
  const int N = b.N;
  const double hh = F.h[ij];
  const double hi = iic == 0 ? 1.0 / (hh + d.p.hc) : F.hinv[ij];
  double z;
  if (last) {
// ... 327 lines not shown
    wi = wi - cur.fu1 + cur.fu0 - cur.fv1 + cur.fv0;
    if (pidx > 0) wi = wi + pflx * prf[(long)(k - 1) * d.p.npip];
    double w = wi - wrk * (up.zw - zw0);
    const double cx_up = fmax0(up.fu1) - fmin0(up.fu0) + fmax0(up.fv1) - fmin0(up.fv0);
    const double hz_up = up.hz;
    const double c2d = dmax(cx_k, cx_up);
    const double dh = dmin(hz_k, hz_up);
    const double cw_max = cu_max * dh - c2d * CX0;
    double we;
    if (cw_max > 0.0) {
      const double cw_max2 = cw_max * cw_max;
      const double cw_min = cw_max * cmnx_ratio;
      const double cw = fabs(w) * CX0;
      double cff;
      if (cw < cw_min) cff = cw_max2;
      else if (cw < cutoff * cw_max) cff = cw_max2 + r4cmx * ((cw - cw_min) * (cw - cw_min));
      else cff = cw_max * cw;
      we = cw_max2 * w / cff;
      w = w - we;
    } else {
      we = 0.0;
    }
    We[o1] = we;
    Wi[o1] = w;
    cx_k = cx_up;
    hz_k = hz_up;
    cur = up;
  };
  constexpr int PF = ROMS_OMEGA_PF;
  Lv ring[PF];
#pragma unroll
  for (int q = 0; q < PF; q++) ring[q] = ld(2 + q);
  int k0 = 1;
  for (; k0 + PF - 1 <= N - 1; k0 += PF) {
#pragma unroll
    for (int q = 0; q < PF; q++) {
      const Lv up = ring[q];
      ring[q] = ld(k0 + q + 1 + PF);
      lev(k0 + q, up);
    }
  }
#pragma unroll
  for (int q = 0; q < PF; q++)
    if (k0 + q <= N - 1) lev(k0 + q, ring[q]);
}
#else
  double cx_k = cx(0), hz_k = Hz[0];
  wi = 0.0;
#pragma unroll 8
  for (int k = 1; k <= N - 1; k++) {
    const long o1 = (long)k * n2;
    wi = div(k, wi);
    double w = wi - wrk * (zw[o1] - zw0);
    const double cx_up = cx(o1);
    const double hz_up = Hz[o1];
    const double c2d = dmax(cx_k, cx_up);
    const double dh = dmin(hz_k, hz_up);
    const double cw_max = cu_max * dh - c2d * CX0;
    double we;
    if (cw_max > 0.0) {
      const double cw_max2 = cw_max * cw_max;
      const double cw_min = cw_max * cmnx_ratio;
      const double cw = fabs(w) * CX0;
      double cff;
      if (cw < cw_min) cff = cw_max2;
      else if (cw < cutoff * cw_max) cff = cw_max2 + r4cmx * ((cw - cw_min) * (cw - cw_min));
      else cff = cw_max * cw;
      we = cw_max2 * w / cff;
      w = w - we;
    } else {
      we = 0.0;
    }
    We[o1] = we;
    Wi[o1] = w;
    cx_k = cx_up;
    hz_k = hz_up;
  }
}
#endif

constexpr int kOmR = kSegRows;
constexpr int kOmCW = kCX, kOmBlock = kSegMaxS * kOmCW;
template <bool kHB, int CW = kOmCW, bool VG = false>
__global__ void __launch_bounds__(kSegMaxS * CW, 2) k_omega_seg(Dev d, Range R, double dtau, double hcff) {
  const uint3 bI = xcd_tile();
  const Bounds& b = d.b;
  const Fields& F = d.f;
  const int N = b.N;
  const double cu_min = 0.6, cu_max = 1.0, cmnx_ratio = cu_min / cu_max, cutoff = 2.0 - cmnx_ratio,
               r4cmx = 0.25 / (1.0 - cmnx_ratio);
  SegSpan sg = seg_span<CW>(N);
  constexpr bool kU = CW == kCX;
  if constexpr (kU) seg_uniform<CW>(sg);
  const int s = sg.s, S = sg.S, c0 = sg.c0, n = sg.n, l = sg.col;
  const int iu = tile_i0(R.i0) + (int)bI.x * CW + l, ju = R.j0 + (int)bI.y;
  const bool act = iu >= R.i0 && iu <= R.i1 && ju <= R.j1;
  const int i = iu < R.i0 ? R.i0 : (iu < R.i1 ? iu : R.i1), j = ju < R.j1 ? ju : R.j1;
  const long ij = IJ(b, i, j), n2 = b.n2, sj = b.nx2;
  const unsigned vo = (unsigned)ij * 8u, lv = (unsigned)n2 * 8u;
  const BufF64 FU(F.FlxU), FV(F.FlxV), Hz(F.Hz), zw(F.z_w);
  auto LD = [&](const BufF64& B, unsigned v, unsigned o) { return kU ? B.ld(v, o) : B.ld(v + o, 0u); };
  auto ST = [&](const BufF64& B, double x, unsigned v, unsigned o) {
    if constexpr (kU) B.st(x, v, o);
    else B.st(x, v + o, 0u);
  };
  __shared__ double Lw[kSegMaxS][CW], Lcx[kSegMaxS][CW], Lhz[kSegMaxS][CW];
  __shared__ double Lte[kHB ? kSegMaxS : 1][CW], Lti[kHB ? kSegMaxS : 1][CW];
  double fu1[kOmR], fu0[kOmR], fv1[kOmR], fv0[kOmR], cx[kOmR], hz[kOmR], zk[kOmR];
  const int kb = min(c0, N) - 1;
  const double csb = VG ? F.Cs_w[kb] : 0.0, csN = VG ? F.Cs_w[N] : 0.0;
#pragma unroll
  for (int q = 0; q < kOmR; q++) {
    const int k = min(c0 + q, N);
    const unsigned o = (unsigned)(k - 1) * lv;
    fu1[q] = LD(FU, vo + 8u, o); fu0[q] = LD(FU, vo, o); fv1[q] = LD(FV, vo + (unsigned)sj * 8u, o); fv0[q] = LD(FV, vo, o);
    if constexpr (VG) {
      zk[q] = F.Cs_w[k];
    } else {
      hz[q] = LD(Hz, vo, o);
      zk[q] = LD(zw, vo, (unsigned)k * lv);
    }
  }
  double zw0, zwN;
  if constexpr (VG) {
    const VGrid g = vg_column(d, ij);
    zw0 = g.zw0();
    zwN = g.zw1(N, csN);
    double zb = g.zw(kb, csb);
#pragma unroll
    for (int q = 0; q < kOmR; q++) {
      const double z = g.zw1(min(c0 + q, N), zk[q]);
      hz[q] = q == 0 || c0 + q <= N ? z - zb : hz[q > 0 ? q - 1 : 0];
      zk[q] = z;
      zb = z;
    }
  } else {
    zw0 = zw.ld(vo, 0);
    zwN = zw.ld(vo, (unsigned)N * lv);
  }
  const double wsrf = F.swflx[ij] * F.dm_r[ij] * F.dn_r[ij];
  const double CX0 = dtau * F.pm[ij] * F.pn[ij];
  const int pidx = d.p.npip > 0 ? F.pipe_idx[ij] : 0;
  const double pflx = pidx > 0 ? F.pipe_flx[ij] : 0.0;
  const double* __restrict__ prf = pidx > 0 ? F.pipe_prf + (pidx - 1) : nullptr;
#pragma unroll
  for (int q = 0; q < kOmR; q++) cx[q] = fmax0(fu1[q]) - fmin0(fu0[q]) + fmax0(fv1[q]) - fmin0(fv0[q]);
  const int nthr = (int)(blockDim.x * blockDim.y);
  int tl = (int)(threadIdx.x + blockDim.x * threadIdx.y);
  __asm__ volatile("" : "+v"(tl));
  if constexpr (kHB) {
#pragma unroll
    for (int q = 0; q < kOmR; q++) roms_smem[q * nthr + tl] = fu1[q] - fu0[q] + fv1[q] - fv0[q];
  }
  Lcx[s][l] = cx[0];
  Lhz[s][l] = hz[0];
  double wk[kOmR];
  for (int t = 0; t < S; t++) {
    if (s == t) {
      double wi = t == 0 ? 0.0 : Lw[t - 1][l];
#pragma unroll
      for (int q = 0; q < kOmR; q++) {
        double v = wi - fu1[q] + fu0[q] - fv1[q] + fv0[q];
        if (pidx > 0) v = v + pflx * prf[(long)(min(c0 + q, N) - 1) * d.p.npip];
        wi = q < n ? v : wi;
        wk[q] = wi;
      }
      Lw[t][l] = wi;
    }
    __syncthreads();
  }
  const double wrk = (Lw[S - 1][l] + wsrf) / (zwN - zw0);
  const double cx_top = s + 1 < S ? Lcx[s + 1][l] : 0.0, hz_top = s + 1 < S ? Lhz[s + 1][l] : 0.0;
  if (!kHB && !act) return;
  const BufF64 Wi(F.Wi), We(F.We);
  const unsigned vs = act ? vo : kBufOff;
  const double hbf = kHB ? hcff * F.pm[ij] * F.pn[ij] : 0.0;
  const BufF64 Hf(F.c2), Hb(F.c3);
  double we_p = 0.0, wi_p = 0.0, we_f = 0.0, wi_f = 0.0;
  int tr = tl;
  __asm__ volatile("" : "+v"(tr));
  auto hb_store = [&](int q, double we1, double wi1, double we0, double wi0) {
    const double div = roms_smem[q * nthr + tr];
    const double FlxDiv = hbf * (div + we1 + wi1 - we0 - wi0);
    const unsigned o = (unsigned)(c0 + q - 1) * lv;
    ST(Hf, hz[q] - FlxDiv, vs, o);
    ST(Hb, hz[q] + FlxDiv, vs, o);
  };
  if (s == 0) {
    ST(Wi, 0.0, vs, 0);
    ST(We, 0.0, vs, 0);
    ST(Wi, 0.0, vs, (unsigned)N * lv);
    ST(We, 0.0, vs, (unsigned)N * lv);
  }
#pragma unroll
  for (int q = 0; q < kOmR; q++) {
    const int k = c0 + q;
    double w = wk[q] - wrk * (zk[q] - zw0);
    const double cx_up = q + 1 < n ? cx[q + 1 < kOmR ? q + 1 : kOmR - 1] : cx_top;
    const double hz_up = q + 1 < n ? hz[q + 1 < kOmR ? q + 1 : kOmR - 1] : hz_top;
    const double c2d = dmax(cx[q], cx_up);
    const double dh = dmin(hz[q], hz_up);
    const double cw_max = cu_max * dh - c2d * CX0;
    double we;
    if (cw_max > 0.0) {
      const double cw_max2 = cw_max * cw_max;
      const double cw_min = cw_max * cmnx_ratio;
      const double cw = fabs(w) * CX0;
      double cff;
      if (cw < cw_min) cff = cw_max2;
      else if (cw < cutoff * cw_max) cff = cw_max2 + r4cmx * ((cw - cw_min) * (cw - cw_min));
      else cff = cw_max * cw;
      we = cw_max2 * w / cff;
      w = w - we;
    } else {
      we = 0.0;
    }
    if (q < n && k <= N - 1) {
      ST(We, we, vs, (unsigned)k * lv);
      ST(Wi, w, vs, (unsigned)k * lv);
    }
    if constexpr (kHB) {
      const double we1 = k <= N - 1 ? we : 0.0, wi1 = k <= N - 1 ? w : 0.0;
      if (q == 0) { we_f = we1; wi_f = wi1; }
      if (q >= 1 && q < n) hb_store(q, we1, wi1, we_p, wi_p);
      if (q == n - 1) { Lte[s][l] = we1; Lti[s][l] = wi1; }
      we_p = we1; wi_p = wi1;
    }
  }
  if constexpr (kHB) {
    __syncthreads();
    const double we0 = s > 0 ? Lte[s - 1][l] : 0.0, wi0 = s > 0 ? Lti[s - 1][l] : 0.0;
    hb_store(0, we_f, wi_f, we0, wi0);
  }
}

__global__ void k_omega_edges(Dev d) {
  const Bounds& b = d.b;
  const Fields& F = d.f;
  const int p = blockIdx.x * blockDim.x + threadIdx.x, k = (int)blockIdx.y;
  const int nj = b.jend - b.jstr + 1, ni = b.iend - b.istr + 1;
  int di = 0, dj = 0, si = 0, sj = 0;
  if (p < nj) {
    if (!b.west_edge) return;
    dj = sj = b.jstr + p; di = b.istr - 1; si = b.istr;
  } else if (p < 2 * nj) {
    if (!b.east_edge) return;
    dj = sj = b.jstr + p - nj; di = b.iend + 1; si = b.iend;
  } else if (p < 2 * nj + ni) {
    if (!b.south_edge) return;
    di = si = b.istr + p - 2 * nj; dj = b.jstr - 1; sj = b.jstr;
  } else if (p < 2 * nj + 2 * ni) {
    if (!b.north_edge) return;
    di = si = b.istr + p - 2 * nj - ni; dj = b.jend + 1; sj = b.jend;
  } else {
    const int c = p - 2 * nj - 2 * ni;
    if (c == 0 && b.west_edge && b.south_edge) { di = b.istr - 1; dj = b.jstr - 1; si = b.istr; sj = b.jstr; }
    else if (c == 1 && b.west_edge && b.north_edge) { di = b.istr - 1; dj = b.jend + 1; si = b.istr; sj = b.jend; }
    else if (c == 2 && b.east_edge && b.south_edge) { di = b.iend + 1; dj = b.jstr - 1; si = b.iend; sj = b.jstr; }
    else if (c == 3 && b.east_edge && b.north_edge) { di = b.iend + 1; dj = b.jend + 1; si = b.iend; sj = b.jend; }
    else return;
  }
  const long dst = IJ(b, di, dj) + (long)k * b.n2, src = IJ(b, si, sj) + (long)k * b.n2;
  F.We[dst] = F.We[src];
  F.Wi[dst] = F.Wi[src];
}

static size_t omega_hb_lds_bytes(unsigned nthr) { return (size_t)kOmR * nthr * sizeof(double); }
void setup_omega_seg() {
  (void)hipFuncSetAttribute((const void*)k_omega_seg<true>, hipFuncAttributeMaxDynamicSharedMemorySize,
                            (int)omega_hb_lds_bytes(kOmBlock));
  (void)hipFuncSetAttribute((const void*)k_omega_seg<true, kOmCW, true>, hipFuncAttributeMaxDynamicSharedMemorySize,
                            (int)omega_hb_lds_bytes(kOmBlock));
}

template <bool kHB, int CW>
static void omega_seg_cw(const Dev& d, hipStream_t s, const Range& r, double dtau, double hcff) {
  const Bounds& b = d.b;
  const dim3 gs((r.i1 - tile_i0(r.i0) + CW) / CW, r.j1 - r.j0 + 1), bs(kCX, seg_waves<CW>(b.N));
  const size_t lds = kHB ? omega_hb_lds_bytes(bs.x * bs.y) : 0;
  if (d.p.vg & (kVg2Omega << kVg2Shift)) hipLaunchKernelGGL((k_omega_seg<kHB, CW, true>), gs, bs, lds, s, d, r, dtau, hcff);
  else hipLaunchKernelGGL((k_omega_seg<kHB, CW, false>), gs, bs, lds, s, d, r, dtau, hcff);
}
template <bool kHB>
static void omega_seg(const Dev& d, hipStream_t s, const Range& r, double dtau, double hcff) {
  if (d.p.omega_cw == 16) omega_seg_cw<kHB, 16>(d, s, r, dtau, hcff);
  else if (d.p.omega_cw == 32) omega_seg_cw<kHB, 32>(d, s, r, dtau, hcff);
  else omega_seg_cw<kHB, kOmCW>(d, s, r, dtau, hcff);
}

bool omega_takes_seg(const Dev& d, int width) {
  return d.p.omega_seg && d.b.N <= kSegRows * kSegMaxS && width >= 32;
}
bool launch_omega(const Dev& d, hipStream_t s, const Tlev& t, double hcff) {
  const Bounds& b = d.b;
  double dtau;
  if (t.nrhs == 3) dtau = d.p.dt;
  else if (t.iic == t.forw_start) dtau = 0.5 * d.p.dt;
  else dtau = 0.6 * d.p.dt;
  Range R{b.istr, b.iend, b.jstr, b.jend};
  const bool hb = hcff > 0.0 && omega_takes_seg(d, R.i1 - R.i0 + 1) && !rim_overlap_on(d, R);
  launch_rim_first(
      d, s, R, ExchList{{d.f.We, d.f.Wi}, {b.N + 1, b.N + 1}, 2},
      [&](const Range& r) {
        if (hb)
          omega_seg<true>(d, s, r, dtau, hcff);
        else if (omega_takes_seg(d, r.i1 - r.i0 + 1))
          omega_seg<false>(d, s, r, dtau, 0.0);
        else
          hipLaunchKernelGGL(k_omega, grid_of(r), dim3(kBX, kBY), 0, s, d, r, dtau);
      },
      [&] {
        if (b.west_edge || b.east_edge || b.south_edge || b.north_edge) {
          const int n = 2 * (b.jend - b.jstr + 1) + 2 * (b.iend - b.istr + 1) + 4;
          hipLaunchKernelGGL(k_omega_edges, dim3((n + 255) / 256, b.N + 1), dim3(256), 0, s, d);
        }
      });
  return hb;
}

struct PColumn {
  double g, grho, HalfGRho, qp2, zwN, ptide;
  bool split, tides;
  BufF64 Pb{nullptr};
  unsigned vP, lv;
  int N;
  double zC, rC, qC;
  double eZk, eRk, dZ1, dR1, P1, z1, v1;
  __device__ __forceinline__ double rhov(double r1, double q1, double z) const {
    if (split) {
      const double dpth = -z;
      return r1 + q1 * dpth * (1.0 - qp2 * dpth);
    }
    return r1;
  }
  __device__ __forceinline__ double eRof(double ru, double rl, double qu, double ql, double zu, double zl) const {
    if (split) {
      const double dpth = -0.5 * (zu + zl);
      return ru - rl + (qu - ql) * dpth * (1.0 - qp2 * dpth);
    }
    return ru - rl;
  }
  __device__ __forceinline__ void iter(int m, double zM, double rM, double qM) {
    const double OneFifth = 0.2, OneTwelfth = 1.0 / 12.0;
    if (m == N) {
      eZk = zC - zM;
      eRk = eRof(rC, rM, qC, qM, zC, zM);
      dZ1 = 0.0; dR1 = 0.0; P1 = 0.0; z1 = 0.0; v1 = 0.0;
    }
    double eZm, eRm;
    if (m >= 2) { eZm = zC - zM; eRm = eRof(rC, rM, qC, qM, zC, zM); }
    else { eZm = eZk; eRm = eRk; }
    const double dZk = [&] { const double c = 2.0 * eZk * eZm; return c / (eZk + eZm); }();
    double dRk;
    {
      const double c = 2.0 * eRk * eRm;
      dRk = c > 0.0 ? c / (eRk + eRm) : 0.0;
    }
    const double v0 = rhov(rC, qC, zC);
    if (split) {
      const double dpth = -zC;
      dRk = dRk - qC * dZk * (1.0 - 2.0 * qp2 * dpth);
    }
    double Pk;
    if (m == N) {
      const double rNm = rhov(rM, qM, zM);
      Pk = g * zwN + grho * (v0 + 0.5 * (v0 - rNm) * (zwN - zC) / (zC - zM)) * (zwN - zC);
      if (tides) Pk = Pk - g * ptide;
    } else {
      Pk = P1 + HalfGRho * ((v1 + v0) * (z1 - zC) -
                            OneFifth * ((dR1 - dRk) * (z1 - zC - OneTwelfth * (dZ1 + dZk)) -
                                        (dZ1 - dZk) * (v1 - v0 - OneTwelfth * (dR1 + dRk))));
    }
    Pb.st(Pk, vP, (unsigned)(m - 1) * lv);
    P1 = Pk;
    dZ1 = dZk; dR1 = dRk;
    eZk = eZm; eRk = eRm;
    z1 = zC; v1 = v0;
  }
  __device__ __forceinline__ void level(int k, double z, double r, double q) {
    if (k < N) iter(k + 1, z, r, q);
    zC = z; rC = r; qC = q;
  }
  __device__ __forceinline__ void last() { iter(1, 0.0, 0.0, 0.0); }
};
__device__ __forceinline__ PColumn p_column(const Dev& d, int i, int j, long ij, bool split, bool have_zwN = false,
                                            double zwN = 0.0) {
  const Bounds& b = d.b;
  PColumn c;
// ... 212 lines not shown
```

ucla-roms_amd/csrc/roms_dev.h:

```cpp
#pragma once
#include <hip/hip_runtime.h>
#include <cstddef>
#include <cstdint>

namespace roms {

constexpr int kMaxFast = 288;
constexpr int kRowAlign = 16;
constexpr int kAlignOff = 14;

struct Bounds {
  int Lm, Mm, N, NT, nTS, nx2;
  long n2, n3, n3w;
  int gx;
  int istr, iend, jstr, jend;
  int istrU, istrR, iendR, jstrV, jstrR, jendR;
  int istrE, iendE, jstrE, jendE;
  int west_edge, east_edge, south_edge, north_edge;
  int ew_periodic, ns_periodic;
  int west_exch, east_exch, south_exch, north_exch;
};

struct Params {
  int nonlin_eos, salinity, lmd, uv_vis2, ts_dif2;
  int lmd_rimix, lmd_convec, lmd_nonlocal;
  int lmd_ddmix;
  int iso;
  int uv_adv, uv_cor;
  int tides;
  int bulk_frc;
  int prs_split;
  int s2d_split;
  int colseg;
  int colreg;
  int uv2_fused;
  int chain;
  int seg_order;
  int seg_xg;
  int s2d_fold;
  int hoist;
  int chain_dirz;
  int prs_fuse_uv;
  int h_jc;
  int prs_buf;
  int prs_strip;
  int t_strip;
  int visc_stg;
  int t3dmix_stg;
  int kpp_ty;
  int uv1_lds;
  int omega_seg;
  int omega_cw;
  int p_in_rho;
  int omega_hb;
  int preuv_lds;
  int seg_jrows;
  int seg_buf;
  int vgrid2;
  int reserved_[7];
  int s2d_k;
  int uv2e_nc, uv2e_nf;
  int npip;
  int nriv, nrivf;
  int curvgrid;
  int obc;
  short kpp_lean;
  short kpp_fckeep;
  short vgrid;
  short vg;
  double ubind;
  double dt, dtfast, g, rho0, vonKar, qp2, gamma2, hc;
  double rdrg, Zob, Tcoef, T0, Scoef, S0;
  double Akv_bak, Akt_bak[2];
};
static_assert(offsetof(Params, s2d_k) == 196 && offsetof(Params, ubind) == 240 && sizeof(Params) == 384,
              "Params: no member from s2d_k on may move");

struct Fields {
  double *h, *hinv, *f, *fomn, *pm, *pn, *dm_r, *dn_r, *dm_u, *dn_u, *dm_v, *dn_v, *dm_p, *dn_p,
      *pmon_u, *pnom_v, *rmask, *pmask, *umask, *vmask;
  double *dndx, *dmde;
  double* ptide;
  double *uwnd, *vwnd, *tair, *qair, *prate, *swrad, *lwrad, *sustr_r, *svstr_r;
  double *Cs_w, *Cs_r;
  double* z_sd;
  double *zeta, *ubar, *vbar, *u, *v, *t;
  double *FlxU, *FlxV, *We, *Wi, *Hz, *Hz_u, *Hz_v, *z_r, *z_w;
  double *rufrc, *rvfrc, *rhoA, *rhoS, *r_D, *Zt_avg1, *DU_avg1, *DV_avg1, *DU_avg2, *DV_avg2,
      *DU_avg_bak, *DV_avg_bak;
  double *rho, *rho1, *qp1, *bvf, *Akv, *Akt, *visc2_r, *visc2_p, *diff2;
  double *hbls, *hbbl, *ghat, *swr_frac;
  double *sustr, *svstr, *stflx, *srflx, *swflx;
  double *ru, *rv, *P, *rhos;
  double *c0, *c1, *c2, *c3;
  double *s0, *s1, *s2, *s3, *s4, *s5, *s6, *s7, *s8, *s9;
  double *lmd_rig, *lmd_hbl, *lmd_bbl, *lmd_Bo, *lmd_Bosol, *lmd_ustar;
  int* pipe_idx;
  double *pipe_flx, *pipe_prf, *pipe_trc;
  double *riv_uflx, *riv_vflx, *riv_vol, *riv_trc;
  int* riv_face;
  int *uv2e_couple, *uv2e_flux;
  double *bzeta[4], *bubar[4], *bvbar[4], *bu[4], *bv[4], *bt[4];
  double* ub[4];
  double* colscr;
  double *dRdx, *dRde, *idRz, *diff3u, *diff3v, *Akz;
  double *iso_dTdz, *iso_FSC, *iso_dTdx, *iso_dTde, *iso_LapT;
};

enum S2dWinField : int {
  kW_zeta, kW_ubar, kW_vbar, kW_h, kW_dn_u, kW_dm_v, kW_pm, kW_pn, kW_swflx, kW_rmask, kW_rhoS, kW_rhoA, kW_umask,
  kW_vmask, kW_rufrc, kW_rvfrc, kW_DU_avg1, kW_DV_avg1, kW_DU_avg2, kW_DV_avg2, kW_Zt_avg1, kW_DU_avg_bak,
  kW_DV_avg_bak, kW_s0, kW_s1, kWinN
};
struct S2dWin {
  const double* base;
  int lead;
  unsigned off[kWinN];
};

struct Halo;
struct Dev {
  Bounds b;
  Params p;
  Fields f;
  const Halo* halo;
  S2dWin w2;
};

__host__ __device__ __forceinline__ long IJ(const Bounds& b, int i, int j) {
  return (long)(i + 1) + (long)(j + 1) * b.nx2;
}
__host__ __device__ __forceinline__ long IJK(const Bounds& b, int i, int j, int k) {
  return IJ(b, i, j) + (long)(k - 1) * b.n2;
}
__host__ __device__ __forceinline__ long IJW(const Bounds& b, int i, int j, int k) {
  return IJ(b, i, j) + (long)k * b.n2;
}
__host__ __device__ __forceinline__ long IJL(const Bounds& b, int i, int j, int l) {
  return IJ(b, i, j) + (long)(l - 1) * b.n2;
}
__host__ __device__ __forceinline__ long IJKL(const Bounds& b, int i, int j, int k, int l) {
  return IJ(b, i, j) + (long)(k - 1) * b.n2 + (long)(l - 1) * b.n3;
}
__host__ __device__ __forceinline__ long TIDX(const Bounds& b, int i, int j, int k, int l, int itrc) {
  return IJKL(b, i, j, k, l) + (long)(itrc - 1) * 3 * b.n3;
}

__device__ __forceinline__ double fmax0(double a) { return a > 0.0 ? a : 0.0; }
__device__ __forceinline__ double fmin0(double a) { return a < 0.0 ? a : 0.0; }
__device__ __forceinline__ double dmax(double a, double b) { return a > b ? a : b; }
__device__ __forceinline__ double dmin(double a, double b) { return a < b ? a : b; }
__device__ __forceinline__ int iclamp(int x, int lo, int hi) { return x < lo ? lo : (x > hi ? hi : x); }

constexpr int kVgRho = 1, kVgKppExt = 2, kVgKppInt = 4, kVgHuv = 8, kVgAll = 15;
constexpr int kVgDefault = kVgRho | kVgKppExt | kVgHuv;
constexpr int kVg2Omega = 1, kVg2Huv1 = 2, kVg2Uv2 = 4, kVg2Visc = 8, kVg2T3dmix = 16, kVg2All = 31, kVg2Shift = 8;
constexpr int kVg2Default = kVg2All;
struct VGrid {
  const double *Cs_w, *Cs_r;
  double z, h, hinv, hc, ds;
  int N;
  __device__ __forceinline__ double zw0() const { return -h; }
  __device__ __forceinline__ double zw1(int k, double csw) const {
    const double cff_w = hc * ds * (double)(k - N);
    return z + (z + h) * (cff_w + csw * h) * hinv;
  }
  __device__ __forceinline__ double zr(int k, double csr) const {
    const double cff_r = hc * ds * ((double)(k - N) - 0.5);
    return z + (z + h) * (cff_r + csr * h) * hinv;
  }
  __device__ __forceinline__ double zw(int k, double csw) const { return k == 0 ? zw0() : zw1(k, csw); }
  __device__ __forceinline__ double zw1(int k) const { return zw1(k, Cs_w[k]); }
  __device__ __forceinline__ double zr(int k) const { return zr(k, Cs_r[k]); }
};
__device__ __forceinline__ double vg_zw(const VGrid& g, int k) { return k == 0 ? g.zw0() : g.zw1(k); }
__device__ __forceinline__ double vg_zr(const VGrid& g, int k) { return g.zr(k); }
__device__ __forceinline__ double vg_hz(const VGrid& g, int k) { return g.zw1(k) - vg_zw(g, k - 1); }
__device__ __forceinline__ VGrid vg_make(const Dev& d, double z, double h, double hinv) {
  return VGrid{d.f.Cs_w, d.f.Cs_r, z, h, hinv, d.p.hc, 1.0 / (double)d.b.N, d.b.N};
}
__device__ __forceinline__ VGrid vg_column(const Dev& d, long ij) {
  return vg_make(d, d.f.z_sd[ij], d.f.h[ij], d.f.hinv[ij]);
}

__device__ __forceinline__ uint3 xcd_tile() {
  const unsigned gx = gridDim.x, gy = gridDim.y;
  const unsigned total = gx * gy * gridDim.z;
  const unsigned phys = blockIdx.x + gx * (blockIdx.y + gy * blockIdx.z);
  const unsigned q = total >> 3, r = total & 7u, x = phys & 7u, slot = phys >> 3;
  const unsigned logical = x * q + (x < r ? x : r) + slot;
  uint3 t;
  t.x = logical % gx;
  t.y = (logical / gx) % gy;
  t.z = logical / (gx * gy);
  return t;
}

#define ROMS_LEVEL_FENCE() __asm__ volatile("" ::: "memory")
#ifndef ROMS_FENCE_EVERY
#define ROMS_FENCE_EVERY 1000
#endif
#define ROMS_LEVEL_FENCE_AT(k) do { if ((k) % ROMS_FENCE_EVERY == 0) ROMS_LEVEL_FENCE(); } while (0)

struct Range {
  int i0, i1, j0, j1;
};
constexpr int kBX = 64, kBY = 4;
#ifndef ROMS_TILE_ALIGN
#define ROMS_TILE_ALIGN 1
#endif
__host__ __device__ __forceinline__ int tile_i0(int i0) { return ROMS_TILE_ALIGN ? i0 - ((i0 - 1) & (kRowAlign - 1)) : i0; }
inline dim3 grid_of(const Range& r) {
  int ni = r.i1 - tile_i0(r.i0) + 1, nj = r.j1 - r.j0 + 1;
  if (ni < 1) ni = 1;
  if (nj < 1) nj = 1;
  return dim3((ni + kBX - 1) / kBX, (nj + kBY - 1) / kBY, 1);
}
inline dim3 grid3_of(const Range& r, int nk) {
  dim3 g = grid_of(r);
  g.z = nk;
  return g;
}
constexpr int kCX = 64;
#ifndef ROMS_SEG_ROWS
#define ROMS_SEG_ROWS 13
#endif
#ifndef ROMS_SEG_MAXS
#define ROMS_SEG_MAXS 8
#endif
constexpr int kSegRows = ROMS_SEG_ROWS;
constexpr int kSegMaxS = ROMS_SEG_MAXS;
#ifndef ROMS_SEG_CW
#define ROMS_SEG_CW 16
#endif
constexpr int kSegCW = ROMS_SEG_CW;
constexpr int kSegBlock = ((kSegMaxS * kSegCW + 63) / 64) * 64;
#ifndef ROMS_SEG_JMAX
#define ROMS_SEG_JMAX 1
#endif
constexpr int kSegJMax = ROMS_SEG_JMAX;
#ifndef ROMS_SEG_NMIN
#define ROMS_SEG_NMIN 11
#endif
constexpr int kSegNMin = ROMS_SEG_NMIN;
#ifndef ROMS_SEG_BUF_WAVES
#define ROMS_SEG_BUF_WAVES 2
#endif
#ifndef ROMS_PRE_T_SEG_WAVES
#define ROMS_PRE_T_SEG_WAVES ROMS_SEG_BUF_WAVES
#endif
#ifndef ROMS_T_SEG_WAVES
#define ROMS_T_SEG_WAVES ROMS_SEG_BUF_WAVES
#endif
inline int seg_count(int N) {
  const int per = kCX / kSegCW, S = (N + kSegRows - 1) / kSegRows;
  return (S + per - 1) / per * per;
}
inline bool seg_rows_ok(int N) { return N / seg_count(N) >= kSegNMin; }
inline dim3 gridc_of(const Range& r) {
  int ni = r.i1 - tile_i0(r.i0) + 1, nj = r.j1 - r.j0 + 1;
  if (ni < 1) ni = 1;
  if (nj < 1) nj = 1;
  return dim3((ni + kCX - 1) / kCX, nj, 1);
}
#define ROMS_IJC_OR_RETURN(R)                                       \
  const uint3 bI = xcd_tile();                                      \
  const int i = tile_i0((R).i0) + (int)(bI.x * kCX + threadIdx.x);  \
  const int j = (R).j0 + (int)bI.y;                                 \
  if (i < (R).i0 || i > (R).i1 || j > (R).j1) return;
#define ROMS_IJ_OR_RETURN(R)                                        \
  const uint3 bI = xcd_tile();                                      \
  const int i = tile_i0((R).i0) + (int)(bI.x * kBX + threadIdx.x); \
  const int j = (R).j0 + (int)(bI.y * kBY + threadIdx.y);           \
  if (i < (R).i0 || i > (R).i1 || j > (R).j1) return;

struct Tlev {
  int iic, ntstart, forw_start, iif, nfast, kstp, knew, nstp, nrhs, nnew;
};

constexpr int kTimedS2dFb = 13;
constexpr int kTimedPreUvSeg = 14, kTimedUv1Seg = 15, kTimedStep3dTSeg = 16;
constexpr int kTimedPrsgrdUv = 17;
constexpr int kTimedHaloPack = 18, kTimedHaloWait = 19, kTimedHaloUnpack = 20;
void ktimer_mark(hipStream_t s, int kernel_id, int end, int count = 0);

inline bool buffer_span_ok(const Bounds& b) { return b.n3w * 8 < 2147483648L; }

void launch_exchange(const Dev& d, hipStream_t s, double* a, int nlev);
constexpr int kExchMax = 16;
struct ExchList {
  double* p[kExchMax];
  int nlev[kExchMax];
  int n;
  int w = 2;
};
void launch_exchange_list(const Dev& d, hipStream_t s, const ExchList& L);
bool rim_overlap_on(const Dev& d, const Range& R);
void rim_fork(const Dev& d, hipStream_t s, const ExchList& L);
void rim_join(const Dev& d, hipStream_t s);
template <class Run, class Edges>
void launch_rim_first(const Dev& d, hipStream_t s, const Range& R, const ExchList& L, Run&& run, Edges&& edges) {
  if (!rim_overlap_on(d, R)) {
    run(R);
    edges();
    launch_exchange_list(d, s, L);
    return;
  }
  run(Range{R.i0, R.i0 + 1, R.j0, R.j1});
  run(Range{R.i1 - 1, R.i1, R.j0, R.j1});
  run(Range{R.i0 + 2, R.i1 - 2, R.j0, R.j0 + 1});
  run(Range{R.i0 + 2, R.i1 - 2, R.j1 - 1, R.j1});
  edges();
  rim_fork(d, s, L);
  run(Range{R.i0 + 2, R.i1 - 2, R.j0 + 2, R.j1 - 2});
  rim_join(d, s);
}
bool tracer_exch_list(const Dev& d, int tlev, ExchList& L);
void launch_exchange_tracers(const Dev& d, hipStream_t s, int tlev);
bool setup_column_kernels(int N);
void setup_uv1_seg();
void setup_pre_uv_seg();
inline size_t col_smem_bytes(const Dev& d, int nslots) {
  return d.f.colscr ? 0 : (size_t)nslots * (d.b.N + 1) * 64 * sizeof(double);
}
void launch_set_depth(const Dev& d, hipStream_t s, const Tlev& t, bool exchange = true, bool last = false);
void launch_set_huv(const Dev& d, hipStream_t s, const Tlev& t, bool store_huv = true);
void launch_vgrid_check(const Dev& d, hipStream_t s, unsigned long long* cnt);
void launch_set_huv1(const Dev& d, hipStream_t s, const Tlev& t);
bool launch_omega(const Dev& d, hipStream_t s, const Tlev& t, double hcff = 0.0);
void setup_omega_seg();
bool omega_takes_seg(const Dev& d, int width);
int s2d_edge_mode(const Dev& d);
int s2d_edge_modes_taken(bool reset = false);
bool prsgrd_takes_strips(const Dev& d, bool with_uv, int& jA, int& jB, int& nstrip);
double pre_step3d_dtau(const Dev& d, const Tlev& t);
void launch_rho_eos(const Dev& d, hipStream_t s, const Tlev& t, int tidx);
void launch_prsgrd(const Dev& d, hipStream_t s, const Tlev& t, int uv_up = -1, bool p_ready = false);
bool launch_tracer_strip(const Dev& d, hipStream_t s, const Range& R, int mode, bool up, bool hb_done, int nnew,
                         int nrhs, double dtau, double cf_stp, double cf_bak, int nstp, int& jA, int& jB);
bool p_in_rho(const Dev& d);
void launch_prsgrd_P(const Dev& d, hipStream_t s);
bool prsgrd_can_fuse_uv(const Dev& d);
struct Side {
  hipStream_t s2;
  hipEvent_t efork, ejoin;
};
void launch_pre_step3d(const Dev& d, hipStream_t s, const Tlev& t, bool uv_done = false, bool hb_done = false,
                       const Side* side = nullptr);
void launch_step3d_uv1(const Dev& d, hipStream_t s, const Tlev& t, bool uv_done = false);
void launch_visc3d(const Dev& d, hipStream_t s, const Tlev& t);
void launch_step2d(const Dev& d, hipStream_t s, const Tlev& t, const double* w1, const double* w2);
void launch_step3d_uv2(const Dev& d, hipStream_t s, const Tlev& t);
void launch_step3d_t(const Dev& d, hipStream_t s, const Tlev& t, bool exchange = true);
void launch_t3dmix(const Dev& d, hipStream_t s, const Tlev& t);
void launch_u3dbc(const Dev& d, hipStream_t s, const Tlev& t);
void launch_river_s2d(const Dev& d, hipStream_t s, int knew);
void launch_bulk_flux(const Dev& d, hipStream_t s, int nrhs);
void launch_river_uv(const Dev& d, hipStream_t s, int nnew, int pred);
void launch_v3dbc(const Dev& d, hipStream_t s, const Tlev& t);
void launch_t3dbc(const Dev& d, hipStream_t s, const Tlev& t, int itrc);
void launch_diag(const Dev& d, hipStream_t s, const Tlev& t, double* out);
// ... 10 lines not shown
```

ucla-roms_amd/csrc/roms_shim.cpp:

```cpp
#include <hip/hip_runtime.h>

#include <algorithm>
#include <cmath>
#include <cstdlib>
#include <cstdio>
#include <cstring>
#include <map>
#include <string>
#include <vector>

#include "../../include/roms_gpu.h"
#include "halo.h"
#include "host_init.h"
#include "roms_dev.h"
#include "shim_state.h"

using namespace roms;

namespace {

struct FieldDesc {
  double* d = nullptr;
  long count = 0;
  long hcount = 0;
// ... 3 lines not shown
};

struct Ctx {
  bool inited = false;
  Dev d{};
  hipStream_t s = nullptr;
  FieldDesc f[ROMS_NFIELDS];
  std::vector<double*> scratch;
  roms_dims dims{};
  roms_cfg cfg{};
  double w1[kMaxFast], w2[kMaxFast];
  double area = 0.0, volume = 0.0;
  bool have_volume = false;
  long riv_maxidx = 0;
  bool have_swr = false;
  long graph_frc_gen = 0;
  int rho_slot = 0;
  bool hzuv_env = false;
  bool hzuv_valid = true;
  bool rho_reuse = true;
  bool vgrid_valid = false;
  std::string err;
  std::map<long, hipGraphExec_t> graphs;
  bool use_graphs = true;
  double* h_diag = nullptr;
  double* d_diag = nullptr;
  Halo halo;
  int timed = -1;
  std::vector<hipEvent_t> ev;
  size_t nev = 0;
  long kcount = 0;
  bool guard = false;
  std::map<double*, double*> guard_base;
  double* arena = nullptr;
  long arena_n = 0, arena_used = 0;
  double* small = nullptr;
  long small_n = 0;
  long off = 0;
  Bounds hb{};
  double* stage = nullptr;
  long stage_n = 0;
  int par = 0;
  long step_exch = 0;
  hipStream_t s2 = nullptr;
  hipEvent_t pev[8] = {};
};
thread_local Ctx g;

double tree_sum(std::vector<double> v) {
  int size = (int)v.size();
  while (size > 1) {
    const int step = (size + 1) / 2;
    for (int r = 0; r < size - step; r++) v[r] = v[r] + v[r + step];
    size = step;
  }
  return v.empty() ? 0.0 : v[0];
}
void rank_extent(int LL, int np, int node, int& len, int& sw) {
  const int base = (LL + np - 1) / np, off = np * base - LL;
  sw = node == 0 ? 0 : node * base - off / 2;
  len = base;
  if (node == 0) len -= off / 2;
  if (node == np - 1) len -= (off + 1) / 2;
}
int min_rank_extent(int LL, int np) {
  int mn = LL, len, sw;
  for (int node : {0, np - 1}) {
    rank_extent(LL, np, node, len, sw);
    mn = len < mn ? len : mn;
  }
  if (np > 2) {
    rank_extent(LL, np, 1, len, sw);
    mn = len < mn ? len : mn;
  }
  return mn;
}

void drop_graphs() {
  for (auto& kv : g.graphs) (void)hipGraphExecDestroy(kv.second);
  g.graphs.clear();
}
void vg_set(bool valid) {
  g.vgrid_valid = valid;
  g.d.p.vg = valid ? (short)(g.d.p.vgrid | (g.d.p.vgrid2 << kVg2Shift)) : (short)0;
}
void vg_host_write(int id) {
  if (id != ROMS_Hz && id != ROMS_z_r && id != ROMS_z_w && id != ROMS_h && id != ROMS_hinv && id != ROMS_Cs_w &&
      id != ROMS_Cs_r)
    return;
  if (g.vgrid_valid && !g.graphs.empty()) {
    (void)hipStreamSynchronize(g.s);
    drop_graphs();
  }
  vg_set(false);
}

#define CHECK_HIP(x)                                                                  \
  do {                                                                                \
    hipError_t e_ = (x);                                                              \
    if (e_ != hipSuccess) {                                                           \
      g.err = std::string(#x) + ": " + hipGetErrorString(e_);                         \
      return -2;                                                                      \
    }                                                                                 \
  } while (0)

#define REQUIRE_INIT_NOJOIN()                           \
  do {                                                  \
    if (!g.inited) {                                    \
      g.err = "roms_gpu: not initialised";              \
      return -1;                                        \
    }                                                   \
  } while (0)
#define REQUIRE_HALO_OK()                                                                    \
  do {                                                                                       \
    if (g.d.halo && halo_failed(g.halo)) {                                                   \
      g.err = "roms_gpu: a halo exchange wait timed out (IPC transport, ROMS_GPU_IPC_TIMEOUT);" \
              " the state since is invalid";                                                 \
      return -6;                                                                             \
    }                                                                                        \
  } while (0)
#define REQUIRE_INIT()                                  \
  do {                                                  \
    REQUIRE_INIT_NOJOIN();                              \
    REQUIRE_HALO_OK();                                  \
    if (g.d.halo) halo_join(g.halo, g.s);               \
    g.rho_slot = 0;                                     \
  } while (0)
#define REQUIRE_INIT_RO()                               \
  const int rho_keep_ = g.rho_slot;                     \
  REQUIRE_INIT();                                       \
  g.rho_slot = rho_keep_

int post_launch() {
  hipError_t e = hipGetLastError();
  if (e != hipSuccess) {
    g.err = std::string("kernel launch: ") + hipGetErrorString(e);
    return -3;
  }
  return 0;
}

bool env_off(const char* name) {
  const char* e = getenv(name);
  return e && e[0] == '0';
}
bool env_on(const char* name) {
  const char* e = getenv(name);
  return e && e[0] == '1';
}
int env_int(const char* name, int def, int lo, int hi) {
  const char* e = getenv(name);
  if (!e || !((e[0] >= '0' && e[0] <= '9') || (e[0] == '-' && e[1] >= '0' && e[1] <= '9'))) return def;
  const int v = atoi(e);
  return v >= lo && v <= hi ? v : def;
}

Bounds make_bounds(const roms_dims& D, int pitch, int gx = 0) {
  Bounds b{};
  b.Lm = D.Lm; b.Mm = D.Mm; b.N = D.N; b.NT = D.NT;
  b.nTS = 1;
  b.nx2 = pitch;
  b.gx = gx;
  b.n2 = (long)pitch * (D.Mm + 4 + 2 * gx);
  b.n3 = b.n2 * D.N;
  b.n3w = b.n2 * (D.N + 1);
  b.istr = 1; b.iend = D.Lm; b.jstr = 1; b.jend = D.Mm;
  b.ew_periodic = D.ew_periodic; b.ns_periodic = D.ns_periodic;
// ... 480 lines not shown
    const int obc = cfg->obc & ((dims->ew_periodic ? 0 : 3) | (dims->ns_periodic ? 0 : 12));
    if (comm == nullptr || split || obc) k = 1;
    const int mext = std::min(min_rank_extent(dims->LLm, dims->np_xi), min_rank_extent(dims->MMm, dims->np_eta));
    while (k > 1 && mext < 2 * k + 2) k--;
    const int gx = 2 * (k - 1);
    g.off = pad ? kAlignOff : 0;
    const int w = hx + 2 * gx;
    g.d.b = make_bounds(*dims, pad ? (w + kRowAlign - 1) / kRowAlign * kRowAlign : w, gx);
    g.hb = make_bounds(*dims, hx);
    g.d.p.s2d_k = k;
  }
  if (!buffer_span_ok(g.d.b)) {
    g.err = "roms_gpu_init: subdomain too large for one GPU rank: a w-point field (n2*(N+1)*8 B) reaches 2 GiB, "
            "the limit of the kernels' 32-bit buffer offsets (k_common.h BufF64); split the grid over more ranks";
    return -1;
  }
  CHECK_HIP(hipSetDevice(device));
  g.d.b.nTS = g.hb.nTS = cfg->salinity ? 2 : 1;
  Params& P = g.d.p;
  {
    const int m = cfg->lmd_mixing, base = ROMS_LMD_MIXING | ROMS_LMD_KPP | ROMS_LMD_BKPP;
    if (m != 0 && ((m & ~(ROMS_LMD_ALL | ROMS_LMD_DDMIX)) || (m & base) != base ||
                   ((m & ROMS_LMD_CONVEC) && !(m & ROMS_LMD_RIMIX)) || ((m & ROMS_LMD_DDMIX) && !cfg->salinity))) {
      g.err = "roms_gpu_init: lmd_mixing must be 0 or LMD_MIXING|LMD_KPP|LMD_BKPP [|RIMIX|NONLOCAL|CONVEC(needs RIMIX)"
              "|DDMIX(needs SALINITY)]";
      return -1;
    }
  }
  P.nonlin_eos = cfg->nonlin_eos; P.salinity = cfg->salinity; P.lmd = cfg->lmd_mixing != 0;
  P.lmd_rimix = (cfg->lmd_mixing & ROMS_LMD_RIMIX) != 0;
  P.lmd_convec = (cfg->lmd_mixing & ROMS_LMD_CONVEC) != 0;
  P.lmd_nonlocal = (cfg->lmd_mixing & ROMS_LMD_NONLOCAL) != 0;
  P.lmd_ddmix = (cfg->lmd_mixing & ROMS_LMD_DDMIX) != 0;
  P.uv_adv = cfg->uv_adv != 0; P.uv_cor = cfg->uv_cor != 0;
  P.tides = cfg->pot_tides != 0;
  P.bulk_frc = cfg->bulk_frc != 0;
  P.iso = cfg->adv_isoneutral != 0;
  P.prs_split = !env_on("ROMS_GPU_PRSGRD_FUSED");
  P.uv_vis2 = cfg->uv_vis2; P.ts_dif2 = cfg->ts_dif2;
  P.s2d_split = env_on("ROMS_GPU_S2D_SPLIT");
  P.dt = cfg->dt; P.dtfast = cfg->dt / (double)cfg->ndtfast; P.g = cfg->g; P.rho0 = cfg->rho0;
  P.vonKar = 0.41; P.qp2 = 0.0000172; P.gamma2 = cfg->gamma2; P.hc = cfg->hc;
  P.rdrg = cfg->rdrg; P.Zob = cfg->Zob; P.Tcoef = cfg->Tcoef; P.T0 = cfg->T0; P.Scoef = cfg->Scoef; P.S0 = cfg->S0;
  P.Akv_bak = cfg->Akv_bak; P.Akt_bak[0] = cfg->Akt_bak[0]; P.Akt_bak[1] = cfg->Akt_bak[1];
  P.npip = 0;
  if (cfg->obc < 0 || cfg->obc > 15) { g.err = "roms_gpu_init: obc must be a 4-bit edge mask"; return -1; }
  P.obc = cfg->obc & ((dims->ew_periodic ? 0 : 3) | (dims->ns_periodic ? 0 : 12));
  P.ubind = cfg->ubind;
  P.curvgrid = cfg->curvgrid && cfg->uv_adv;
  if (P.obc) P.s2d_split = 1;
  for (int i = 0; i < kMaxFast; i++) { g.w1[i] = cfg->weight[0][i]; g.w2[i] = cfg->weight[1][i]; }
  const bool seg_fits = dims->N <= kSegRows * kSegMaxS && seg_rows_ok(dims->N);
  P.colseg = (size_t)2 * (dims->N + 1) * kCX * sizeof(double) > 64 * 1024 && seg_fits;
  if (env_off("ROMS_GPU_COLSEG")) P.colseg = 0;
  if (env_on("ROMS_GPU_COLSEG")) P.colseg = seg_fits;
  P.colreg = env_int("ROMS_GPU_COLREG", 2, 0, 3);
  P.uv2_fused = !env_off("ROMS_GPU_UV2_FUSED");
  P.chain = !env_off("ROMS_GPU_CHAIN");
  P.seg_order = env_int("ROMS_GPU_SEG_ORDER", 3, 0, 3);
  P.seg_xg = env_int("ROMS_GPU_SEG_XG", 8, 1, 1 << 30);
  P.s2d_fold = !env_on("ROMS_GPU_S2D_EDGES");
  P.chain_dirz = !env_off("ROMS_GPU_CHAIN_DIRZ");
  P.prs_fuse_uv = !env_off("ROMS_GPU_PRS_UV");
  P.uv1_lds = !env_off("ROMS_GPU_UV1_LDS");
  P.p_in_rho = !env_off("ROMS_GPU_P_IN_RHO");
  P.omega_hb = !env_off("ROMS_GPU_OMEGA_HB");
  P.omega_seg = !env_off("ROMS_GPU_OMEGA_SEG");
  {
    const int v = env_int("ROMS_GPU_OMEGA_CW", dims->N > 63 ? 16 : 64, 0, 1 << 30);
    P.omega_cw = v == 32 || v == 64 ? v : 16;
  }
  P.preuv_lds = !env_off("ROMS_GPU_PREUV_LDS");
  P.h_jc = env_int("ROMS_GPU_HJC", 0, 0, 1 << 30) / 4 * 4;
  P.visc_stg = !env_off("ROMS_GPU_VISC_STG");
  P.t3dmix_stg = !env_off("ROMS_GPU_T3DMIX_STG");
  {
    const int v = env_int("ROMS_GPU_KPP_TY", 4, 0, 43);
    P.kpp_ty = v == 0 || v == 2 || v == 8 || v == 43 ? v : 4;
  }
  P.kpp_lean = (short)env_int("ROMS_GPU_KPP_LEAN", 7, 0, 7);
  P.kpp_fckeep = (short)env_int("ROMS_GPU_KPP_FCKEEP", kKppFcKeepMax, 1, kKppFcKeepMax);
  P.vgrid = (short)env_int("ROMS_GPU_VGRID", kVgDefault, 0, kVgAll);
  P.vgrid2 = env_int("ROMS_GPU_VGRID2", kVg2Default, 0, kVg2All);
  P.vg = 0;
  g.vgrid_valid = false;
  P.hoist = !env_off("ROMS_GPU_HOIST");
  P.prs_buf = !env_off("ROMS_GPU_PRS_BUF");
  P.prs_strip = !env_off("ROMS_GPU_PRS_STRIP");
  P.t_strip = env_on("ROMS_GPU_T_STRIP");
  P.seg_buf = !env_off("ROMS_GPU_SEG_BUF");
  P.seg_jrows = env_int("ROMS_GPU_SEG_JROWS", kSegJMax < 2 ? kSegJMax : 2, 1, kSegJMax);
  bool col_global = (size_t)2 * (dims->N + 1) * kCX * sizeof(double) > 64 * 1024;
  if (env_on("ROMS_GPU_COL_GLOBAL")) col_global = true;
  if (env_off("ROMS_GPU_COL_GLOBAL")) col_global = false;
  setup_uv1_seg();
  setup_pre_uv_seg();
  setup_omega_seg();
  if (!col_global && !setup_column_kernels(dims->N)) {
    g.err = "roms_gpu_init: N too large for the LDS column kernels (2*(N+1)*512 B > 160 KB)";
    return -2;
  }
  CHECK_HIP(hipStreamCreateWithFlags(&g.s, hipStreamNonBlocking));
  CHECK_HIP(hipStreamCreateWithFlags(&g.s2, hipStreamNonBlocking));
  for (hipEvent_t& e : g.pev) CHECK_HIP(hipEventCreateWithFlags(&e, hipEventDisableTiming));
  {
    const char* em = getenv("ROMS_GPU_PAR_MASK");
    g.par = env_on("ROMS_GPU_PAR") ? 31 : 0;
    if (em) g.par = atoi(em) & 31;
  }
  g.guard = env_on("ROMS_GPU_GUARD");
  const Bounds& b = g.d.b;
  auto field = [&](int id) -> int {
    const long n = field_count(id, b);
    double* p = nullptr;
    CHECK_HIP(dev_alloc(p, n));
    g.f[id].d = p;
    g.f[id].count = n;
    g.f[id].hcount = field_count(id, g.hb);
    g.f[id].planar = planar_field(id);
    *field_slot(g.d.f, id) = p;
    return 0;
  };
  auto planar2d = [&](int id) { return planar_field(id) && field_count(id, b) <= 4 * b.n2; };
  {
    long n = 11 * dev_alloc_size(b.n2);
    for (int id = 0; id < ROMS_NFIELDS; id++)
      if (planar2d(id)) n += dev_alloc_size(field_count(id, b));
    if (n * 8 < 2147483648L - (1L << 20)) {
      CHECK_HIP(hipMalloc(&g.arena, (size_t)n * sizeof(double)));
      g.arena_n = n;
      g.arena_used = 0;
    }
  }
  for (int id = 0; id < ROMS_NFIELDS; id++)
    if (planar2d(id) && field(id)) return -2;
  auto scratch = [&](double*& p, long n) -> int {
    CHECK_HIP(dev_alloc(p, n));
    g.scratch.push_back(p);
    return 0;
  };
  Fields& F = g.d.f;
  double** s2[] = {&F.s0, &F.s1, &F.s2, &F.s3, &F.s4, &F.s5, &F.s6, &F.s7, &F.s8, &F.s9};
  for (double** q : s2)
    if (scratch(*q, b.n2)) return -2;
  if (scratch(F.z_sd, b.n2)) return -2;
  g.arena_n = g.arena_used;
  for (int id = 0; id < ROMS_NFIELDS; id++)
    if (!planar2d(id) && field(id)) return -2;
  if (scratch(F.P, b.n3) || scratch(F.rhos, b.n3) || scratch(F.c0, b.n3w) || scratch(F.c1, b.n3w) ||
      scratch(F.c2, b.n3w) || scratch(F.c3, b.n3w))
    return -2;
  {
    g.d.w2 = S2dWin{};
    const double* wp[kWinN] = {F.zeta,  F.ubar,  F.vbar,    F.h,       F.dn_u,    F.dm_v,       F.pm,
                               F.pn,    F.swflx, F.rmask,   F.rhoS,    F.rhoA,    F.umask,      F.vmask,
                               F.rufrc, F.rvfrc, F.DU_avg1, F.DV_avg1, F.DU_avg2, F.DV_avg2,    F.Zt_avg1,
                               F.DU_avg_bak, F.DV_avg_bak, F.s0, F.s1};
    const long lead = (long)b.gx * b.nx2 + b.gx + kRowAlign;
    uintptr_t lo = UINTPTR_MAX, hi = 0;
    for (int f = 0; f < kWinN; f++) {
      const long cnt = f <= kW_vbar ? 4 * b.n2 : b.n2;
      lo = std::min(lo, (uintptr_t)wp[f] - (uintptr_t)lead * 8u);
      hi = std::max(hi, (uintptr_t)wp[f] + (uintptr_t)cnt * 8u);
    }
    if (!env_off("ROMS_GPU_S2D_WIN") && hi - lo < (uintptr_t)2147483648u - (1u << 20)) {
      g.d.w2.base = (const double*)lo;
// ... 95 lines not shown
  }
  if (id < 0 || id >= ROMS_NFIELDS) { g.err = "bad field id"; return -1; }
  if (!g.f[id].host) { g.err = "field not registered"; return -1; }
  if (!up && !hzuv_readable(id)) return -5;
  if (up && (id == ROMS_Hz_u || id == ROMS_Hz_v)) g.hzuv_valid = true;
  if (up) vg_host_write(id);
  CHECK_HIP(up ? field_h2d(id, g.f[id].d, g.f[id].host) : field_d2h(id, g.f[id].host, g.f[id].d));
  return 0;
}
int roms_gpu_upload(int id) { REQUIRE_INIT(); return xfer(id, true); }
int roms_gpu_download(int id) { REQUIRE_INIT_RO(); return xfer(id, false); }

int roms_gpu_copy_in(int id, const double* src, long count) {
  REQUIRE_INIT();
  if (id < 0 || id >= ROMS_NFIELDS || count != g.f[id].hcount) { g.err = "roms_gpu_copy_in: bad field/size"; return -1; }
  if (id == ROMS_Hz_u || id == ROMS_Hz_v) g.hzuv_valid = true;
  vg_host_write(id);
  CHECK_HIP(field_h2d(id, g.f[id].d, src));
  return 0;
}
int roms_gpu_copy_out(int id, double* dst, long count) {
  REQUIRE_INIT_RO();
  if (id < 0 || id >= ROMS_NFIELDS || count != g.f[id].hcount) { g.err = "roms_gpu_copy_out: bad field/size"; return -1; }
  if (!hzuv_readable(id)) return -5;
  CHECK_HIP(field_d2h(id, dst, g.f[id].d));
  REQUIRE_HALO_OK();
  return 0;
}
int roms_gpu_sync(void) {
  REQUIRE_INIT_RO();
  CHECK_HIP(hipStreamSynchronize(g.s));
  REQUIRE_HALO_OK();
  return post_launch();
}

#define ROUTINE(name, call)           \
  int name(const roms_tlev* t) {      \
    REQUIRE_INIT();                   \
    const Tlev T = to_tlev(t);        \
    call;                             \
    return post_launch();             \
  }
ROUTINE(roms_gpu_set_huv, (launch_set_huv(g.d, g.s, T), g.hzuv_valid = true))
ROUTINE(roms_gpu_omega, launch_omega(g.d, g.s, T))
ROUTINE(roms_gpu_prsgrd, launch_prsgrd(g.d, g.s, T))
ROUTINE(roms_gpu_pre_step3d, launch_pre_step3d(g.d, g.s, T))
ROUTINE(roms_gpu_set_huv1, launch_set_huv1(g.d, g.s, T))
ROUTINE(roms_gpu_step3d_uv1, launch_step3d_uv1(g.d, g.s, T))
ROUTINE(roms_gpu_visc3d, launch_visc3d(g.d, g.s, T))
ROUTINE(roms_gpu_step3d_uv2, launch_step3d_uv2(g.d, g.s, T))
ROUTINE(roms_gpu_step3d_t, launch_step3d_t(g.d, g.s, T))
ROUTINE(roms_gpu_t3dmix, launch_t3dmix(g.d, g.s, T))
ROUTINE(roms_gpu_set_depth, (launch_set_depth(g.d, g.s, T), vg_set(true)))
#undef ROUTINE

int roms_gpu_halo_transport(void) {
  REQUIRE_INIT_NOJOIN();
  return g.d.halo ? halo_transport(g.halo) : 0;
}

int roms_gpu_halo_overlap(void) {
  REQUIRE_INIT_NOJOIN();
  return g.d.halo && g.halo.xoverlap > 0 ? 1 : 0;
}

int roms_gpu_s2d_window(void) {
  REQUIRE_INIT_NOJOIN();
  return g.d.w2.base ? 1 : 0;
}

int roms_gpu_column_path(void) {
  REQUIRE_INIT_NOJOIN();
  return (g.d.p.colseg ? ROMS_COLPATH_SEG : 0) | (g.d.f.colscr ? ROMS_COLPATH_GLOBAL : 0);
}

int roms_gpu_vgrid(void) {
  REQUIRE_INIT_NOJOIN();
  return g.d.p.vgrid + (g.vgrid_valid ? 256 : 0);
}

int roms_gpu_vgrid2(void) {
  REQUIRE_INIT_NOJOIN();
  return g.d.p.vgrid2 + (g.vgrid_valid ? 256 : 0);
}

int roms_gpu_vgrid_check(long out[3]) {
  REQUIRE_INIT_RO();
  if (!out) { g.err = "roms_gpu_vgrid_check: null argument"; return -1; }
  unsigned long long* cnt = (unsigned long long*)shim_scratch_small(3);
  if (!cnt) { g.err = "roms_gpu_vgrid_check: out of device memory"; return -2; }
  CHECK_HIP(hipMemsetAsync(cnt, 0, 3 * sizeof(unsigned long long), g.s));
  launch_vgrid_check(g.d, g.s, cnt);
  unsigned long long h[3] = {0, 0, 0};
  CHECK_HIP(copy_on(h, cnt, sizeof(h), hipMemcpyDeviceToHost, g.s));
  for (int q = 0; q < 3; q++) out[q] = (long)h[q];
  return post_launch();
}

int roms_gpu_kpp_lean(void) {
  REQUIRE_INIT_NOJOIN();
  return g.d.p.kpp_lean + 256 * g.d.p.kpp_fckeep;
}

int roms_gpu_horizontal_path(int out[8]) {
  REQUIRE_INIT_NOJOIN();
  if (!out) { g.err = "roms_gpu_horizontal_path: null argument"; return -1; }
  const Dev& d = g.d;
  int jA = 0, jB = -1, nstrip = 0;
  const bool strips = prsgrd_takes_strips(d, prsgrd_can_fuse_uv(d), jA, jB, nstrip);
  out[0] = s2d_edge_mode(d);
  out[1] = strips ? 1 : 0;
  out[2] = strips ? nstrip : 0;
  out[3] = strips ? jA : 0;
  out[4] = strips ? jB : -1;
  out[5] = omega_takes_seg(d, d.b.iend - d.b.istr + 1) ? 1 : 0;
  out[6] = s2d_edge_modes_taken();
  out[7] = 0;
  return 0;
}

int roms_gpu_halo_exchanges(long* per_step, int* fast_interval) {
  REQUIRE_INIT_NOJOIN();
  if (per_step) *per_step = g.step_exch;
  if (fast_interval) *fast_interval = g.d.p.s2d_k;
  return 0;
}

int roms_gpu_step2d(const roms_tlev* t) {
  REQUIRE_INIT_NOJOIN();
  REQUIRE_HALO_OK();
  const Tlev T = to_tlev(t);
  launch_step2d(g.d, g.s, T, g.w1, g.w2);
  if (T.iif == T.nfast) vg_set(true);
  return post_launch();
}

int roms_gpu_rho_eos(int tidx, const roms_tlev* t) {
  REQUIRE_INIT();
  launch_rho_eos(g.d, g.s, to_tlev(t), tidx);
  return post_launch();
}
int roms_gpu_lmd_vmix(int tind, const roms_tlev* t) {
  REQUIRE_INIT();
  if (!g.cfg.lmd_mixing) { g.err = "roms_gpu_lmd_vmix: library initialised without lmd_mixing"; return -4; }
  if (tind < 1 || tind > 3) { g.err = "roms_gpu_lmd_vmix: bad time index"; return -1; }
  launch_lmd_vmix(g.d, g.s, to_tlev(t), tind);
  return post_launch();
}
int roms_gpu_swr_frac(const roms_tlev* t) {
  (void)t;
  REQUIRE_INIT();
  launch_swr_frac(g.d, g.s);
  g.have_swr = true;
  return post_launch();
}
int roms_gpu_set_pipe_frc(int npip, const int* pipe_idx, const double* pipe_flx, const double* pipe_prf,
                          const double* pipe_trc) {
  REQUIRE_INIT();
  const Bounds& b = g.d.b;
  Fields& F = g.d.f;
  if (npip < 0 || (npip > 0 && (!pipe_idx || !pipe_flx || !pipe_prf || !pipe_trc))) {
    g.err = "roms_gpu_set_pipe_frc: bad argument";
    return -1;
  }
  if (npip == 0) { g.d.p.npip = 0; return 0; }
  for (long q = 0; q < g.hb.n2; q++)
// ... 517 lines not shown
```

ucla-roms_amd/romsgpu/__init__.py:

```python
import ctypes
import os

import numpy as np

_HERE = os.path.dirname(os.path.abspath(__file__))
_PKG = os.path.dirname(_HERE)
LIB_PATH = os.environ.get("ROMS_GPU_LIB") or os.path.join(_PKG, "libromsgpu.so")
MAX_FAST = 288

FIELDS = ["h", "hinv", "f", "fomn", "pm", "pn", "dm_r", "dn_r", "dm_u", "dn_u", "dm_v", "dn_v", "dm_p", "dn_p",
          "pmon_u", "pnom_v", "rmask", "pmask", "umask", "vmask", "Cs_w", "Cs_r",
          "zeta", "ubar", "vbar", "u", "v", "t", "FlxU", "FlxV", "We", "Wi", "Hz", "Hz_u", "Hz_v", "z_r", "z_w",
          "rufrc", "rvfrc", "rhoA", "rhoS", "r_D", "Zt_avg1", "DU_avg1", "DV_avg1", "DU_avg2", "DV_avg2",
          "DU_avg_bak", "DV_avg_bak", "rho", "rho1", "qp1", "bvf", "Akv", "Akt", "visc2_r", "visc2_p", "diff2",
          "hbls", "hbbl", "ghat", "swr_frac", "sustr", "svstr", "stflx", "srflx", "swflx", "ru", "rv"] + \
         ["%s_%s" % (v, e) for v in ("zeta", "ubar", "vbar", "u", "v", "t") for e in ("west", "east", "south", "north")] + \
         ["dndx", "dmde", "ptide", "uwnd", "vwnd", "tair", "qair", "prate", "swrad", "lwrad", "sustr_r", "svstr_r"]
FIELD_ID = {n: i for i, n in enumerate(FIELDS)}
CASE_FILAMENT, CASE_BASIN, CASE_PIPES, CASE_RIVERS = 0, 1, 2, 3
LMD_MIXING, LMD_KPP, LMD_BKPP, LMD_RIMIX, LMD_CONVEC, LMD_NONLOCAL = 1, 2, 4, 8, 16, 32
LMD_DDMIX = 64
LMD_ALL = 63
LMD_ICELAND = 47

# ... 386 lines not shown

    def frc_clock(self, start_time, on=True):
        self._chk(self.L.roms_gpu_frc_clock(start_time, int(on)), "frc_clock")

    def set_tide_data(self, ftide, pot=None, bry=None):
        D = ctypes.POINTER(ctypes.c_double)
        keep = [np.ascontiguousarray(ftide, dtype=np.float64)]
        def ptr(a):
            if a is None:
                return None
            keep.append(np.ascontiguousarray(a, dtype=np.float64))
            return keep[-1].ctypes.data_as(D)
        pr, pi = pot if pot is not None else (None, None)
        (zr, zi), (ur, ui), (vr, vi) = bry if bry is not None else ((None, None),) * 3
        self._chk(self.L.roms_gpu_set_tide_data(len(keep[0]), keep[0].ctypes.data_as(D), ptr(pr), ptr(pi), ptr(zr),
                                                ptr(zi), ptr(ur), ptr(ui), ptr(vr), ptr(vi)), "set_tide_data")

    def set_tides(self, time):
        self._chk(self.L.roms_gpu_set_tides(time), "set_tides")

    def bulk_flux(self):
        self._chk(self.L.roms_gpu_bulk_flux(ctypes.byref(self.t)), "bulk_flux")

    def _r(self, fn):
        self._chk(getattr(self.L, "roms_gpu_" + fn)(ctypes.byref(self.t)), fn)

    def set_HUV(self): self._r("set_huv")
    def omega(self): self._r("omega")
    def prsgrd(self): self._r("prsgrd")
    def pre_step3d(self): self._r("pre_step3d")
    def set_HUV1(self): self._r("set_huv1")
    def step3d_uv1(self): self._r("step3d_uv1")
    def visc3d(self): self._r("visc3d")
    def step2d(self): self._r("step2d")
    def step3d_uv2(self): self._r("step3d_uv2")
    def step3d_t(self): self._r("step3d_t")
    def t3dmix(self): self._r("t3dmix")
    def set_depth(self): self._r("set_depth")
    def swr_frac(self): self._r("swr_frac")
    def init_sequence(self): self._r("init_sequence")

    def step(self, n=1):
        for _ in range(n):
            self._r("step")

    def time_routine(self, routine, nsteps):
        ms = ctypes.c_double()
        n = ctypes.c_long()
        self._chk(self.L.roms_gpu_time_routine(ROUTINES.index(routine), nsteps, ctypes.byref(self.t), ctypes.byref(ms),
                                               ctypes.byref(n)), "time_routine")
        return ms.value, n.value

    def selftest_zero_fill(self, n, chunks=1):
        nz = ctypes.c_long()
        self._chk(self.L.roms_gpu_selftest_zero_fill(ctypes.c_long(n), ctypes.c_int(chunks), ctypes.byref(nz)),
                  "selftest_zero_fill")
        return nz.value

    def halo_transport(self):
        r = self.L.roms_gpu_halo_transport()
        return {1: "ipc", 0: "rccl", -1: "ipc-timeout"}.get(r, "error")

    def halo_overlap(self):
        return bool(self.L.roms_gpu_halo_overlap())

    def s2d_window(self):
        return bool(self.L.roms_gpu_s2d_window())

    def kpp_lean(self):
        r = self.L.roms_gpu_kpp_lean()
        self._chk(min(r, 0), "kpp_lean")
        return r % 256, r // 256

    def vgrid(self):
        r = self.L.roms_gpu_vgrid()
        self._chk(min(r, 0), "vgrid")
        return r % 256, bool(r // 256)

    def vgrid2(self):
        r = self.L.roms_gpu_vgrid2()
        self._chk(min(r, 0), "vgrid2")
        return r % 256, bool(r // 256)

    def vgrid_mismatch(self):
        out = (ctypes.c_long * 3)()
        self._chk(self.L.roms_gpu_vgrid_check(out), "vgrid_check")
        return out[0], out[1], out[2]

    def column_path(self):
        r = self.L.roms_gpu_column_path()
        self._chk(min(r, 0), "column_path")
        return bool(r & 1), bool(r & 2)

    def horizontal_path(self):
        out = (ctypes.c_int * 8)()
        self._chk(self.L.roms_gpu_horizontal_path(out), "horizontal_path")
        return {"edges": out[0], "strips": (out[2], out[3], out[4]) if out[1] else None, "omega_seg": bool(out[5])}

    def fast_step_edge_modes(self):
        out = (ctypes.c_int * 8)()
        self._chk(self.L.roms_gpu_horizontal_path(out), "horizontal_path")
        return {m for m in range(3) if out[6] >> m & 1}

    def halo_exchanges(self):
        n, k = ctypes.c_long(), ctypes.c_int()
        self._chk(self.L.roms_gpu_halo_exchanges(ctypes.byref(n), ctypes.byref(k)), "halo_exchanges")
        return n.value, k.value

    def diag(self):
        out = (ctypes.c_double * 4)()
        self._chk(self.L.roms_gpu_diag(ctypes.byref(self.t), out), "diag")
        return list(out)

    def time(self, dt):
        return dt * (self.t.iic - self.t.ntstart + 1) + getattr(self, "start_time", 0.0)

    def wrt_rst(self, path, rec, total_rec, time):
        self._chk(self.L.roms_gpu_wrt_rst(path.encode(), rec, total_rec, time, ctypes.byref(self.t)), "wrt_rst")

    def wrt_his(self, path, rec, total_rec, time, mask=WRT_DEFAULT):
        self._chk(self.L.roms_gpu_wrt_his(path.encode(), rec, total_rec, time, ctypes.byref(self.t), mask), "wrt_his")

    def io_wait(self):
        self._chk(self.L.roms_gpu_io_wait(), "io_wait")

    def get_init(self, path, req_rec, tindx):
        st = ctypes.c_double()
        rc = self.L.roms_gpu_get_init(path.encode(), req_rec, tindx, ctypes.byref(self.t), ctypes.byref(st))
        if rc < 0:
            self._chk(rc, "get_init")
        if tindx == 1:
            self.start_time = st.value
        return rc

    def restart(self, path, rec=0, exact=True):
        self.t.forw_start = 0
        if exact:
            nrec = rec if rec > 0 else self._nrecs(path)
            if nrec >= 2:
                self.get_init(path, nrec - 1, 2)
            rec = nrec
        self.get_init(path, rec, 1)
        self.init_sequence()

    @staticmethod
    def _nrecs(path):
        with open(path, "rb") as f:
            h = f.read(8)
        return int.from_bytes(h[4:8], "big")

    def time_steps(self, n):
        ms = ctypes.c_double()
        self._chk(self.L.roms_gpu_time_steps(ctypes.byref(self.t), n, ctypes.byref(ms)), "time_steps")
        return ms.value
```

Before: 2.381 billion cell-updates/s.

## Recompute Hz from vertical grid in segmented column kernels and store one HB buffer

Extends the analytic vertical-grid path to the segmented pre-step tracer, pre-step uv, step3d_t and uv1 kernels, so layer thicknesses are rebuilt from z_sd, h, hinv and Cs_w instead of loaded from the Hz array. Separately, an 'hb_one' mode makes omega and the horizontal pre-tracer kernel store only the flux divergence in one scratch buffer and rebuild both Hz±FlxDiv on the fly, cutting one 3D array write and read. Both paths are on by default. The cost is extra per-row arithmetic and register pressure in already heavy kernels, plus many more template instantiations.

```diff
diff --git a/include/roms_gpu.h b/include/roms_gpu.h
--- a/include/roms_gpu.h
+++ b/include/roms_gpu.h
@@ -5,7 +5,7 @@
 extern "C" {
 #endif
 
-#define ROMS_GPU_ABI_VERSION 21
+#define ROMS_GPU_ABI_VERSION 22
 #define ROMS_MAX_FAST 288
 
 typedef struct roms_dims {
@@ -151,6 +151,7 @@
 int roms_gpu_kpp_lean(void);
 int roms_gpu_vgrid(void);
 int roms_gpu_vgrid2(void);
+int roms_gpu_vgrid3(void);
 int roms_gpu_vgrid_check(long out[3]);
 int roms_gpu_horizontal_path(int out[8]);
 int roms_gpu_selftest_zero_fill(long n, int chunks, long *bad);
diff --git a/ucla-roms_amd/csrc/k_colseg.h b/ucla-roms_amd/csrc/k_colseg.h
--- a/ucla-roms_amd/csrc/k_colseg.h
+++ b/ucla-roms_amd/csrc/k_colseg.h
@@ -178,6 +178,30 @@
   }
 };
 
+__device__ __forceinline__ int seg_row_level(int c0, int q, int N) { return min(max(c0 - 1 + q, 1), N); }
+template <int KQ>
+__device__ __forceinline__ void seg_cs_rows(const Dev& d, int c0, double (&cs)[KQ], double& csb) {
+  const int N = d.b.N;
+  csb = d.f.Cs_w[seg_row_level(c0, 0, N) - 1];
+#pragma unroll
+  for (int q = 0; q < KQ; q++) cs[q] = d.f.Cs_w[seg_row_level(c0, q, N)];
+}
+__device__ __forceinline__ double seg_hz_row(const VGrid& g, int c0, int q, double cs, double& zb, double hzp) {
+  const int N = g.N, k = seg_row_level(c0, q, N);
+  const double z = g.zw1(k, cs);
+  const bool rep = q > 0 && k == seg_row_level(c0, q - 1, N);
+  const double hz = rep ? hzp : z - zb;
+  zb = z;
+  return hz;
+}
+template <int KQ>
+__device__ __forceinline__ void seg_hz_rows(const VGrid& g, int c0, const double (&cs)[KQ], double csb,
+                                            double (&hz)[KQ]) {
+  double zb = g.zw(seg_row_level(c0, 0, g.N) - 1, csb);
+#pragma unroll
+  for (int q = 0; q < KQ; q++) hz[q] = seg_hz_row(g, c0, q, cs[q], zb, hz[q > 0 ? q - 1 : 0]);
+}
+
 template <int KR>
 __device__ __forceinline__ void spline_fc_seg(const SegSpan& sg, int N, SegXchg& X, const double (&w)[KR + 1],
                                               const double (&f)[KR], double (&fc)[KR]) {
@@ -251,7 +275,7 @@
 struct NoSplineRowB {
   __device__ __forceinline__ void operator()(int, unsigned, double, double, double) const {}
 };
-template <int KR, class RowF = NoSplineRowB>
+template <int KR, bool VG = false, class RowF = NoSplineRowB>
 __device__ __forceinline__ void uv_spline_segb(const Dev& d, const SegSpan& sg, SegXchg& X, long ij, int nrhs, int dir,
                                                double (&fl)[KR], RowF row = RowF()) {
   const Bounds& b = d.b;
@@ -269,11 +293,29 @@
   const double* mask = dir == 0 ? F.umask : F.vmask;
   auto LD = [&](const BufF64& B, unsigned v, unsigned l) { return B.ld(v + l, 0u); };
   double dc[KR + 1], uu[KR];
+  VGrid g0{}, g1{}, gp{}, g2{};
+  double zb0 = 0.0, zb1 = 0.0, zbp = 0.0, zb2 = 0.0;
+  double h0 = 0.0, h1 = 0.0, hp = 0.0, h2 = 0.0;
+  if constexpr (VG) {
+    const BufF64 Zs(F.z_sd), Hh(F.h), Hi(F.hinv);
+    auto colg = [&](unsigned v) { return vg_make(d, Zs.ld(v, 0u), Hh.ld(v, 0u), Hi.ld(v, 0u)); };
+    g0 = colg(vo); g1 = colg(vm); gp = colg(vp); g2 = colg(vm2);
+    const int kb = seg_row_level(c0, 0, N) - 1;
+    const double csb = F.Cs_w[kb];
+    zb0 = g0.zw(kb, csb); zb1 = g1.zw(kb, csb); zbp = gp.zw(kb, csb); zb2 = g2.zw(kb, csb);
+  }
 #pragma unroll
   for (int q = 0; q < KR + 1; q++) {
     const unsigned L = (unsigned)(min(max(c0 - 1 + q, 1), N) - 1) * lv;
-    const double h0 = LD(Hz, vo, L), h1 = LD(Hz, vm, L);
-    dc[q] = 0.5625 * (h0 + h1) - 0.0625 * (LD(Hz, vp, L) + LD(Hz, vm2, L));
+    if constexpr (VG) {
+      const double cs = F.Cs_w[seg_row_level(c0, q, N)];
+      h0 = seg_hz_row(g0, c0, q, cs, zb0, h0); h1 = seg_hz_row(g1, c0, q, cs, zb1, h1);
+      hp = seg_hz_row(gp, c0, q, cs, zbp, hp); h2 = seg_hz_row(g2, c0, q, cs, zb2, h2);
+    } else {
+      h0 = LD(Hz, vo, L); h1 = LD(Hz, vm, L);
+      hp = LD(Hz, vp, L); h2 = LD(Hz, vm2, L);
+    }
+    dc[q] = 0.5625 * (h0 + h1) - 0.0625 * (hp + h2);
     if (q < KR) uu[q] = LD(Uv, vo, L);
     row(q, L, h0, h1, q < KR ? uu[q] : 0.0);
     if (q % kSegLoadGroup == kSegLoadGroup - 1) __builtin_amdgcn_sched_barrier(0);
diff --git a/ucla-roms_amd/csrc/k_pre_step3d.hip b/ucla-roms_amd/csrc/k_pre_step3d.hip
--- a/ucla-roms_amd/csrc/k_pre_step3d.hip
+++ b/ucla-roms_amd/csrc/k_pre_step3d.hip
@@ -57,7 +57,8 @@
   double UM[kN], VM[kN], FU[kN], FV[kN], T[NTT][kN];
 };
 template <int NTT, bool kHB>
-__global__ void __launch_bounds__(kBX * kBY) k_pre_tracer_h1(Dev d, Range R, PreCoef c, int nstp, int nnew, int nrhs) {
+__global__ void __launch_bounds__(kBX * kBY) k_pre_tracer_h1(Dev d, Range R, PreCoef c, int nstp, int nnew, int nrhs,
+                                                             int one) {
   const uint3 bI = xcd_tile();
   __shared__ TracerWinN<NTT> W;
   const Bounds& b = d.b;
@@ -90,7 +91,7 @@
   const bool formed = kHB && in;
   double fu0 = 0.0, fu1 = 0.0, fv0 = 0.0, fv1 = 0.0, we1 = 0.0, wi1 = 0.0, we0 = 0.0, wi0 = 0.0, hbo = 0.0;
   if (formed) {
-    hbo = F.c3[o];
+    hbo = one ? F.c2[o] : F.c3[o];
   } else {
     fu0 = F.FlxU[o]; fu1 = F.FlxU[o + 1]; fv0 = F.FlxV[o]; fv1 = F.FlxV[o + b.nx2];
     we1 = F.We[w]; wi1 = F.Wi[w]; we0 = F.We[w - n2]; wi0 = F.Wi[w - n2];
@@ -116,14 +117,14 @@
   if (!act) return;
   double hb;
   if (formed) {
-    hb = hbo;
+    hb = one ? hzo + hbo : hbo;
   } else {
     const double cff = 0.5 * c.dtau;
     const double FlxDiv = cff * pm * pn * (fu1 - fu0 + fv1 - fv0 + we1 + wi1 - we0 - wi0);
     hb = hzo + FlxDiv;
     const double hf = hzo - FlxDiv;
-    F.c2[o] = hf;
-    F.c3[o] = hb;
+    F.c2[o] = one ? FlxDiv : hf;
+    if (!one) F.c3[o] = hb;
   }
   if (!in) return;
   const double hz = hzo;
@@ -701,6 +702,7 @@
   }
 }
 
+template <bool VG, bool ONE>
 __global__ void __launch_bounds__(kSegBlock, ROMS_PRE_T_SEG_WAVES) k_pre_tracer_segb(Dev d, Range R, PreCoef c, int nnew,
                                                                                    int nrhs) {
   const uint3 bI = seg_tile(d.p.seg_order, d.p.seg_xg);
@@ -724,10 +726,16 @@
   const long tb = (long)(itrc - 1) * 3 * b.n3;
   const BufF64 Tr(F.t + (long)(nrhs - 1) * b.n3 + tb), Tn(F.t + (long)(nnew - 1) * b.n3 + tb);
   double hz[KR + 1], tt[KR], fl[KR];
+  double csb = 0.0;
+  if constexpr (VG) seg_cs_rows(d, c0, hz, csb);
 #pragma unroll
   for (int q = 0; q < KR + 1; q++) {
-    hz[q] = LD(Hz, vo, lev(c0 - 1 + q));
+    if constexpr (!VG) hz[q] = LD(Hz, vo, lev(c0 - 1 + q));
     if (q < KR) tt[q] = LD(Tr, vo, lev(c0 - 1 + q));
+  }
+  if constexpr (VG) {
+    const VGrid g = vg_make(d, BufF64(F.z_sd).ld(vo, 0), BufF64(F.h).ld(vo, 0), BufF64(F.hinv).ld(vo, 0));
+    seg_hz_rows(g, c0, hz, csb, hz);
   }
   spline_fc_seg<KR>(sg, N, X, hz, tt, fl);
   {
@@ -744,7 +752,10 @@
   }
   __builtin_amdgcn_sched_barrier(0);
 #pragma unroll
-  for (int q = 0; q < KR + 1; q++) hz[q] = LD(Hf, vo, lev(c0 - 1 + q));
+  for (int q = 0; q < KR + 1; q++) {
+    const double x = LD(Hf, vo, lev(c0 - 1 + q));
+    hz[q] = ONE ? hz[q] - x : x;
+  }
   const int iAkt = itrc < b.nTS ? itrc : b.nTS;
   const BufF64 Akt(F.Akt + (long)(iAkt - 1) * b.n3w);
   const BufF64 Pm(F.pm), Pn(F.pn);
@@ -892,6 +903,7 @@
   }
 }
 
+template <bool VG, bool ONE>
 __global__ void __launch_bounds__(kSegBlock * kSegJMax, 2) k_pre_uv_segb(Dev d, Range R, PreCoef c, int nstp, int nnew,
                                                                          int nrhs) {
   const uint3 bI = seg_tile(d.p.seg_order, d.p.seg_xg);
@@ -919,7 +931,7 @@
   const BufF64 Uix(Uall + (long)(indx - 1) * b.n3), Unew(Uall + (long)(nnew - 1) * b.n3), Hf(F.c2);
   double hf[KR + 1], hfm[KR + 1];
   double fl[KR];
-  uv_spline_segb<KR>(d, sg, X, ij, nrhs, dir, fl, [&](int q, unsigned L, double h0, double h1, double u) {
+  uv_spline_segb<KR, VG>(d, sg, X, ij, nrhs, dir, fl, [&](int q, unsigned L, double h0, double h1, double u) {
     if (q >= 1 && q < KR) {
       Sb[(q - 1) * nthr] = c.cf_stp * u + c.cf_bak * LD(Uix, vo, L);
       Su[(q - 1) * nthr] = 0.5 * (h0 + h1) * u;
@@ -935,14 +947,38 @@
     const double rro = LD(rr, vo, o);
     const double r = k == 1 ? rro - fl[1] : rro - fl[p + 1 < KR ? p + 1 : KR - 1] + fl[p];
     const double ub = Sb[(p < KR - 1 ? p : KR - 2) * nthr];
-    const double v = 0.5 * (LD(Hb, vo, o) + LD(Hb, vm, o)) * ub + DC0 * r;
+    const double v = (ONE ? ub : 0.5 * (LD(Hb, vo, o) + LD(Hb, vm, o)) * ub) + DC0 * r;
     return k == N ? v + c.dtau * sstr : v;
   };
+  VGrid g0{}, g1{};
+  double zb0 = 0.0, zb1 = 0.0, h0 = 0.0, h1 = 0.0;
+  if constexpr (VG && ONE) {
+    const BufF64 Zs(F.z_sd), Hh(F.h), Hi(F.hinv);
+    g0 = vg_make(d, Zs.ld(vo, 0u), Hh.ld(vo, 0u), Hi.ld(vo, 0u));
+    g1 = vg_make(d, Zs.ld(vm, 0u), Hh.ld(vm, 0u), Hi.ld(vm, 0u));
+    const int kb = seg_row_level(c0, 0, N) - 1;
+    const double csb = F.Cs_w[kb];
+    zb0 = g0.zw(kb, csb); zb1 = g1.zw(kb, csb);
+  }
 #pragma unroll
   for (int q = 0; q < KR + 1; q++) {
     const unsigned L = lev(c0 - 1 + q);
-    hf[q] = LD(Hf, vo, L);
-    hfm[q] = LD(Hf, vm, L);
+    const double x0 = LD(Hf, vo, L), x1 = LD(Hf, vm, L);
+    if constexpr (ONE) {
+      if constexpr (VG) {
+        const double cs = F.Cs_w[seg_row_level(c0, q, N)];
+        h0 = seg_hz_row(g0, c0, q, cs, zb0, h0); h1 = seg_hz_row(g1, c0, q, cs, zb1, h1);
+      } else {
+        const BufF64 Hz(F.Hz);
+        h0 = LD(Hz, vo, L); h1 = LD(Hz, vm, L);
+      }
+      hf[q] = h0 - x0;
+      hfm[q] = h1 - x1;
+      if (q >= 1 && q < KR) Sb[(q - 1) * nthr] = 0.5 * ((h0 + x0) + (h1 + x1)) * Sb[(q - 1) * nthr];
+    } else {
+      hf[q] = x0;
+      hfm[q] = x1;
+    }
   }
   auto fcw = [&](int q, double& fc, double& wc) {
     const int r = c0 - 1 + q;
@@ -975,10 +1011,12 @@
   T.couple(sg, n, X, xL, xR);
   T.solve(n, xL, xR);
   const unsigned vs = act ? vo : kBufOff;
+  int cs0 = c0;
+  if constexpr (VG) __asm__ volatile("" : "+v"(cs0));
 #pragma unroll
   for (int p = 0; p < KR; p++)
     if (p < n) {
-      const unsigned o = lev(c0 + p);
+      const unsigned o = lev(cs0 + p);
       Unew.st(T.D[p], vs + o, 0u);
       Uix.st(Su[(p < KR - 1 ? p : KR - 2) * nthr], vs + o, 0u);
     }
@@ -990,8 +1028,11 @@
 void setup_pre_uv_seg() {
   (void)hipFuncSetAttribute((const void*)k_pre_uv_seg<true>, hipFuncAttributeMaxDynamicSharedMemorySize,
                             (int)pre_uv_seg_lds_bytes(kSegBlock * kSegJMax));
-  (void)hipFuncSetAttribute((const void*)k_pre_uv_segb, hipFuncAttributeMaxDynamicSharedMemorySize,
-                            (int)pre_uv_seg_lds_bytes(kSegBlock * kSegJMax));
+  const int bytes = (int)pre_uv_seg_lds_bytes(kSegBlock * kSegJMax);
+  (void)hipFuncSetAttribute((const void*)k_pre_uv_segb<false, false>, hipFuncAttributeMaxDynamicSharedMemorySize, bytes);
+  (void)hipFuncSetAttribute((const void*)k_pre_uv_segb<false, true>, hipFuncAttributeMaxDynamicSharedMemorySize, bytes);
+  (void)hipFuncSetAttribute((const void*)k_pre_uv_segb<true, false>, hipFuncAttributeMaxDynamicSharedMemorySize, bytes);
+  (void)hipFuncSetAttribute((const void*)k_pre_uv_segb<true, true>, hipFuncAttributeMaxDynamicSharedMemorySize, bytes);
 }
 
 void setup_column_kernels_t(size_t bytes);
@@ -1022,6 +1063,7 @@
   else { c.dtau = d.p.dt * (1.0 - AM3_crv); c.cf_stp = 0.5 + AM3_crv; c.cf_bak = 0.5 - AM3_crv; }
   c.dtau = pre_step3d_dtau(d, t);
   hb_done = hb_done && d.p.hoist && b.NT <= 2;
+  const int one = pre_hb_one(d, t) ? 1 : 0;
   Range RI{b.istr, b.iend, b.jstr, b.jend};
   Range RH{b.istr - 1, b.iend, b.jstr - 1, b.jend};
   auto horiz_tiles = [&](const Range& rh) {
@@ -1038,13 +1080,13 @@
       else
         hipLaunchKernelGGL((k_pre_tracer_hj<1, false>), g, bh, 0, s, d, rh, c, t.nstp, t.nnew, t.nrhs, jc);
     } else if (d.p.hoist && b.NT == 2 && hb_done)
-      hipLaunchKernelGGL((k_pre_tracer_h1<2, true>), gh, bh, 0, s, d, rh, c, t.nstp, t.nnew, t.nrhs);
+      hipLaunchKernelGGL((k_pre_tracer_h1<2, true>), gh, bh, 0, s, d, rh, c, t.nstp, t.nnew, t.nrhs, one);
     else if (d.p.hoist && b.NT == 2)
-      hipLaunchKernelGGL((k_pre_tracer_h1<2, false>), gh, bh, 0, s, d, rh, c, t.nstp, t.nnew, t.nrhs);
+      hipLaunchKernelGGL((k_pre_tracer_h1<2, false>), gh, bh, 0, s, d, rh, c, t.nstp, t.nnew, t.nrhs, one);
     else if (d.p.hoist && b.NT == 1 && hb_done)
-      hipLaunchKernelGGL((k_pre_tracer_h1<1, true>), gh, bh, 0, s, d, rh, c, t.nstp, t.nnew, t.nrhs);
+      hipLaunchKernelGGL((k_pre_tracer_h1<1, true>), gh, bh, 0, s, d, rh, c, t.nstp, t.nnew, t.nrhs, one);
     else if (d.p.hoist && b.NT == 1)
-      hipLaunchKernelGGL((k_pre_tracer_h1<1, false>), gh, bh, 0, s, d, rh, c, t.nstp, t.nnew, t.nrhs);
+      hipLaunchKernelGGL((k_pre_tracer_h1<1, false>), gh, bh, 0, s, d, rh, c, t.nstp, t.nnew, t.nrhs, one);
     else
       hipLaunchKernelGGL(k_pre_tracer_h, gh, bh, 0, s, d, rh, c, t.nstp, t.nnew, t.nrhs);
   };
@@ -1066,10 +1108,14 @@
   }
   dim3 gt = gridc_of(RI);
   gt.z = b.NT;
-  if (d.p.colseg && d.p.seg_buf)
-    hipLaunchKernelGGL(k_pre_tracer_segb, seg_grid_of(RI, b.NT), dim3(kCX, seg_waves(b.N)), 0, st, d, RI, c, t.nnew,
-                       t.nrhs);
-  else if (d.p.colseg)
+  if (d.p.colseg && d.p.seg_buf) {
+    const dim3 gs = seg_grid_of(RI, b.NT), bs(kCX, seg_waves(b.N));
+    const bool vg = (d.p.vg & (kVg3PreT << kVg3Shift)) != 0;
+    if (vg && one) hipLaunchKernelGGL((k_pre_tracer_segb<true, true>), gs, bs, 0, st, d, RI, c, t.nnew, t.nrhs);
+    else if (vg) hipLaunchKernelGGL((k_pre_tracer_segb<true, false>), gs, bs, 0, st, d, RI, c, t.nnew, t.nrhs);
+    else if (one) hipLaunchKernelGGL((k_pre_tracer_segb<false, true>), gs, bs, 0, st, d, RI, c, t.nnew, t.nrhs);
+    else hipLaunchKernelGGL((k_pre_tracer_segb<false, false>), gs, bs, 0, st, d, RI, c, t.nnew, t.nrhs);
+  } else if (d.p.colseg)
     hipLaunchKernelGGL(k_pre_tracer_seg, seg_grid_of(RI, b.NT), dim3(kCX, seg_waves(b.N)), 0, st, d, RI, c, t.nnew,
                        t.nrhs);
   else if ((d.p.colreg & 2) && b.N == 50 && !d.f.colscr)
@@ -1089,9 +1135,14 @@
     const dim3 gs = seg_uv_grid(d, RI, d.p.seg_jrows), bs(kCX, seg_waves(b.N), d.p.seg_jrows);
     const bool lds = d.p.preuv_lds && d.p.uv_adv && t.nrhs == t.nstp;
     ktimer_mark(s, kTimedPreUvSeg, 0);
-    if (lds && d.p.seg_buf)
-      hipLaunchKernelGGL(k_pre_uv_segb, gs, bs, pre_uv_seg_lds_bytes(bs.x * bs.y * bs.z), s, d, RI, c, t.nstp, t.nnew,
-                         t.nrhs);
+    if (lds && d.p.seg_buf) {
+      const size_t ldsb = pre_uv_seg_lds_bytes(bs.x * bs.y * bs.z);
+      const bool vg = (d.p.vg & (kVg3PreUv << kVg3Shift)) != 0;
+      if (vg && one) hipLaunchKernelGGL((k_pre_uv_segb<true, true>), gs, bs, ldsb, s, d, RI, c, t.nstp, t.nnew, t.nrhs);
+      else if (vg) hipLaunchKernelGGL((k_pre_uv_segb<true, false>), gs, bs, ldsb, s, d, RI, c, t.nstp, t.nnew, t.nrhs);
+      else if (one) hipLaunchKernelGGL((k_pre_uv_segb<false, true>), gs, bs, ldsb, s, d, RI, c, t.nstp, t.nnew, t.nrhs);
+      else hipLaunchKernelGGL((k_pre_uv_segb<false, false>), gs, bs, ldsb, s, d, RI, c, t.nstp, t.nnew, t.nrhs);
+    }
     else if (lds)
       hipLaunchKernelGGL(k_pre_uv_seg<true>, gs, bs, pre_uv_seg_lds_bytes(bs.x * bs.y * bs.z), s, d, RI, c, t.nstp,
                          t.nnew, t.nrhs);
diff --git a/ucla-roms_amd/csrc/k_step3d_t.hip b/ucla-roms_amd/csrc/k_step3d_t.hip
--- a/ucla-roms_amd/csrc/k_step3d_t.hip
+++ b/ucla-roms_amd/csrc/k_step3d_t.hip
@@ -337,6 +337,7 @@
 #ifndef ROMS_SEG_T_GROUP
 #define ROMS_SEG_T_GROUP kSegLoadGroup
 #endif
+template <bool VG>
 __global__ void __launch_bounds__(kSegBlock, ROMS_T_SEG_WAVES) k_step3d_t_segb(Dev d, Range R, int nnew, int nrhs) {
   const uint3 bI = seg_tile(d.p.seg_order, d.p.seg_xg);
   __shared__ SegXchg X;
@@ -362,13 +363,17 @@
   const BufF64 Tr(F.t + (long)(nrhs - 1) * b.n3 + (long)(itrc - 1) * 3 * b.n3);
   const BufF64 Tn(F.t + (long)(nnew - 1) * b.n3 + (long)(itrc - 1) * 3 * b.n3);
   double hz[KR + 1], tt[KR], tn[KR];
+  double csb = 0.0;
+  if constexpr (VG) seg_cs_rows(d, c0, hz, csb);
 #pragma unroll
   for (int q = 0; q < KR + 1; q++) {
-    hz[q] = LD(Hz, vo, lev(c0 - 1 + q));
+    if constexpr (!VG) hz[q] = LD(Hz, vo, lev(c0 - 1 + q));
     if (q < KR) tt[q] = LD(Tr, vo, lev(c0 - 1 + q));
   }
 #pragma unroll
   for (int p = 0; p < KR; p++) tn[p] = LD(Tn, vo, lev(c0 + p));
+  if constexpr (VG)
+    seg_hz_rows(vg_make(d, BufF64(F.z_sd).ld(vo, 0), BufF64(F.h).ld(vo, 0), BufF64(F.hinv).ld(vo, 0)), c0, hz, csb, hz);
   {
     double fc[KR];
     spline_fc_seg<KR>(sg, N, X, hz, tt, fc);
@@ -413,7 +418,7 @@
     for (int p = 0; p < KR; p++) t = p == n - 1 ? rhs[p] : t;
     if (itrc == 1) {
       const double swf = BufF64(F.swflx).ld(vo, 0);
-      t = t + dt * swf * (P.bulk_frc ? BufF64(F.tair).ld(vo, 0) : t / LD(Hz, vo, lev(N)));
+      t = t + dt * swf * (P.bulk_frc ? BufF64(F.tair).ld(vo, 0) : t / (VG ? hz[KR] : LD(Hz, vo, lev(N))));
     }
     t = t + dt * stf;
 #pragma unroll
@@ -480,8 +485,10 @@
   T.solve(n, xL, xR);
   const double rm = BufF64(F.rmask).ld(vo, 0);
   const unsigned vs = act ? vo : kBufOff;
-#pragma unroll
-  for (int p = 0; p < KR; p++) Tn.st(T.D[p] * rm, (p < n ? vs : kBufOff) + lev(c0 + p), 0u);
+  int cs0 = c0;
+  if constexpr (VG) __asm__ volatile("" : "+v"(cs0));
+#pragma unroll
+  for (int p = 0; p < KR; p++) Tn.st(T.D[p] * rm, (p < n ? vs : kBufOff) + lev(cs0 + p), 0u);
 }
 
 void setup_column_kernels_t(size_t bytes) {
@@ -528,8 +535,10 @@
     gt.z = b.NT;
     if (d.p.colseg) {
       ktimer_mark(s, kTimedStep3dTSeg, 0);
-      if (d.p.seg_buf)
-        hipLaunchKernelGGL(k_step3d_t_segb, seg_grid_of(r, b.NT), dim3(kCX, seg_waves(b.N)), 0, s, d, r, t.nnew, t.nrhs);
+      if (d.p.seg_buf && (d.p.vg & (kVg3TSeg << kVg3Shift)))
+        hipLaunchKernelGGL(k_step3d_t_segb<true>, seg_grid_of(r, b.NT), dim3(kCX, seg_waves(b.N)), 0, s, d, r, t.nnew, t.nrhs);
+      else if (d.p.seg_buf)
+        hipLaunchKernelGGL(k_step3d_t_segb<false>, seg_grid_of(r, b.NT), dim3(kCX, seg_waves(b.N)), 0, s, d, r, t.nnew, t.nrhs);
       else
         hipLaunchKernelGGL(k_step3d_t_seg, seg_grid_of(r, b.NT), dim3(kCX, seg_waves(b.N)), 0, s, d, r, t.nnew, t.nrhs);
       ktimer_mark(s, kTimedStep3dTSeg, 1, 1);
diff --git a/ucla-roms_amd/csrc/k_step3d_uv.hip b/ucla-roms_amd/csrc/k_step3d_uv.hip
--- a/ucla-roms_amd/csrc/k_step3d_uv.hip
+++ b/ucla-roms_amd/csrc/k_step3d_uv.hip
@@ -266,6 +266,7 @@
   }
 }
 
+template <bool VG>
 __global__ void __launch_bounds__(kSegBlock * kSegJMax, 2) k_uv1_segb(Dev d, Range R, int nnew, int nrhs) {
   const uint3 bI = seg_tile(d.p.seg_order, d.p.seg_xg);
   __shared__ SegXchg X;
@@ -292,7 +293,7 @@
   const BufF64 Un((dir == 0 ? F.u : F.v) + (long)(nnew - 1) * b.n3);
   auto LD = [&](const BufF64& B, unsigned v, unsigned l) { return B.ld(v + l, 0u); };
   double fl[KR];
-  uv_spline_segb<KR>(d, sg, X, ij, nrhs, dir, fl, [&](int q, unsigned, double h0, double h1, double) {
+  uv_spline_segb<KR, VG>(d, sg, X, ij, nrhs, dir, fl, [&](int q, unsigned, double h0, double h1, double) {
     Sh[q * nthr] = h0;
     Shm[q * nthr] = h1;
   });
@@ -373,7 +374,9 @@
                             (int)((size_t)kSegRows * kSegMaxS * kSegCW * kSegJMax * sizeof(double)));
   (void)hipFuncSetAttribute((const void*)k_uv1_seg<true>, hipFuncAttributeMaxDynamicSharedMemorySize,
                             (int)uv1_seg_lds_bytes(kSegBlock * kSegJMax));
-  (void)hipFuncSetAttribute((const void*)k_uv1_segb, hipFuncAttributeMaxDynamicSharedMemorySize,
+  (void)hipFuncSetAttribute((const void*)k_uv1_segb<false>, hipFuncAttributeMaxDynamicSharedMemorySize,
+                            (int)uv1_seg_lds_bytes(kSegBlock * kSegJMax));
+  (void)hipFuncSetAttribute((const void*)k_uv1_segb<true>, hipFuncAttributeMaxDynamicSharedMemorySize,
                             (int)uv1_seg_lds_bytes(kSegBlock * kSegJMax));
 }
 
@@ -386,8 +389,10 @@
   if (d.p.colseg) {
     const dim3 gs = seg_uv_grid(d, R, d.p.seg_jrows), bs(kCX, seg_waves(b.N), d.p.seg_jrows);
     ktimer_mark(s, kTimedUv1Seg, 0);
-    if (d.p.uv1_lds && d.p.uv_adv && d.p.seg_buf)
-      hipLaunchKernelGGL(k_uv1_segb, gs, bs, uv1_seg_lds_bytes(bs.x * bs.y * bs.z), s, d, R, t.nnew, t.nrhs);
+    if (d.p.uv1_lds && d.p.uv_adv && d.p.seg_buf && (d.p.vg & (kVg3Uv1 << kVg3Shift)))
+      hipLaunchKernelGGL(k_uv1_segb<true>, gs, bs, uv1_seg_lds_bytes(bs.x * bs.y * bs.z), s, d, R, t.nnew, t.nrhs);
+    else if (d.p.uv1_lds && d.p.uv_adv && d.p.seg_buf)
+      hipLaunchKernelGGL(k_uv1_segb<false>, gs, bs, uv1_seg_lds_bytes(bs.x * bs.y * bs.z), s, d, R, t.nnew, t.nrhs);
     else if (d.p.uv1_lds && d.p.uv_adv)
       hipLaunchKernelGGL(k_uv1_seg<true>, gs, bs, uv1_seg_lds_bytes(bs.x * bs.y * bs.z), s, d, R, t.nnew, t.nrhs);
     else
diff --git a/ucla-roms_amd/csrc/k_vertical.hip b/ucla-roms_amd/csrc/k_vertical.hip
--- a/ucla-roms_amd/csrc/k_vertical.hip
+++ b/ucla-roms_amd/csrc/k_vertical.hip
@@ -433,7 +433,7 @@
 constexpr int kOmR = kSegRows;
 constexpr int kOmCW = kCX, kOmBlock = kSegMaxS * kOmCW;
 template <bool kHB, int CW = kOmCW, bool VG = false>
-__global__ void __launch_bounds__(kSegMaxS * CW, 2) k_omega_seg(Dev d, Range R, double dtau, double hcff) {
+__global__ void __launch_bounds__(kSegMaxS * CW, 2) k_omega_seg(Dev d, Range R, double dtau, double hcff, int hb_one) {
   const uint3 bI = xcd_tile();
   const Bounds& b = d.b;
   const Fields& F = d.f;
@@ -534,8 +534,8 @@
     const double div = roms_smem[q * nthr + tr];
     const double FlxDiv = hbf * (div + we1 + wi1 - we0 - wi0);
     const unsigned o = (unsigned)(c0 + q - 1) * lv;
-    ST(Hf, hz[q] - FlxDiv, vs, o);
-    ST(Hb, hz[q] + FlxDiv, vs, o);
+    ST(Hf, hb_one ? FlxDiv : hz[q] - FlxDiv, vs, o);
+    ST(Hb, hz[q] + FlxDiv, hb_one ? kBufOff : vs, o);
   };
   if (s == 0) {
     ST(Wi, 0.0, vs, 0);
@@ -625,18 +625,18 @@
 }
 
 template <bool kHB, int CW>
-static void omega_seg_cw(const Dev& d, hipStream_t s, const Range& r, double dtau, double hcff) {
+static void omega_seg_cw(const Dev& d, hipStream_t s, const Range& r, double dtau, double hcff, int one) {
   const Bounds& b = d.b;
   const dim3 gs((r.i1 - tile_i0(r.i0) + CW) / CW, r.j1 - r.j0 + 1), bs(kCX, seg_waves<CW>(b.N));
   const size_t lds = kHB ? omega_hb_lds_bytes(bs.x * bs.y) : 0;
-  if (d.p.vg & (kVg2Omega << kVg2Shift)) hipLaunchKernelGGL((k_omega_seg<kHB, CW, true>), gs, bs, lds, s, d, r, dtau, hcff);
-  else hipLaunchKernelGGL((k_omega_seg<kHB, CW, false>), gs, bs, lds, s, d, r, dtau, hcff);
+  if (d.p.vg & (kVg2Omega << kVg2Shift)) hipLaunchKernelGGL((k_omega_seg<kHB, CW, true>), gs, bs, lds, s, d, r, dtau, hcff, one);
+  else hipLaunchKernelGGL((k_omega_seg<kHB, CW, false>), gs, bs, lds, s, d, r, dtau, hcff, one);
 }
 template <bool kHB>
-static void omega_seg(const Dev& d, hipStream_t s, const Range& r, double dtau, double hcff) {
-  if (d.p.omega_cw == 16) omega_seg_cw<kHB, 16>(d, s, r, dtau, hcff);
-  else if (d.p.omega_cw == 32) omega_seg_cw<kHB, 32>(d, s, r, dtau, hcff);
-  else omega_seg_cw<kHB, kOmCW>(d, s, r, dtau, hcff);
+static void omega_seg(const Dev& d, hipStream_t s, const Range& r, double dtau, double hcff, int one = 0) {
+  if (d.p.omega_cw == 16) omega_seg_cw<kHB, 16>(d, s, r, dtau, hcff, one);
+  else if (d.p.omega_cw == 32) omega_seg_cw<kHB, 32>(d, s, r, dtau, hcff, one);
+  else omega_seg_cw<kHB, kOmCW>(d, s, r, dtau, hcff, one);
 }
 
 bool omega_takes_seg(const Dev& d, int width) {
@@ -654,7 +654,7 @@
       d, s, R, ExchList{{d.f.We, d.f.Wi}, {b.N + 1, b.N + 1}, 2},
       [&](const Range& r) {
         if (hb)
-          omega_seg<true>(d, s, r, dtau, hcff);
+          omega_seg<true>(d, s, r, dtau, hcff, pre_hb_one(d, t) ? 1 : 0);
         else if (omega_takes_seg(d, r.i1 - r.i0 + 1))
           omega_seg<false>(d, s, r, dtau, 0.0);
         else
diff --git a/ucla-roms_amd/csrc/roms_dev.h b/ucla-roms_amd/csrc/roms_dev.h
--- a/ucla-roms_amd/csrc/roms_dev.h
+++ b/ucla-roms_amd/csrc/roms_dev.h
@@ -57,7 +57,8 @@
   int seg_jrows;
   int seg_buf;
   int vgrid2;
-  int reserved_[7];
+  int vgrid3;
+  int reserved_[6];
   int s2d_k;
   int uv2e_nc, uv2e_nf;
   int npip;
@@ -156,6 +157,11 @@
 constexpr int kVgDefault = kVgRho | kVgKppExt | kVgHuv;
 constexpr int kVg2Omega = 1, kVg2Huv1 = 2, kVg2Uv2 = 4, kVg2Visc = 8, kVg2T3dmix = 16, kVg2All = 31, kVg2Shift = 8;
 constexpr int kVg2Default = kVg2All;
+constexpr int kVg3PreT = 1, kVg3TSeg = 2, kVg3PreUv = 4, kVg3Uv1 = 8, kVg3Seg = 15, kVg3Shift = 4;
+constexpr int kVg3HbOne = 16, kVg3All = 31;
+constexpr int kVg3Default = kVg3All;
+static_assert(kVgAll < (1 << kVg3Shift) && (kVg3Seg << kVg3Shift) < (1 << kVg2Shift) && (kVg2All << kVg2Shift) < (1 << 15),
+              "Params::vg: the three masks' bits stay apart and within a short");
 struct VGrid {
   const double *Cs_w, *Cs_r;
   double z, h, hinv, hc, ds;
@@ -277,6 +283,10 @@
 struct Tlev {
   int iic, ntstart, forw_start, iif, nfast, kstp, knew, nstp, nrhs, nnew;
 };
+inline bool pre_hb_one(const Dev& d, const Tlev& t) {
+  return (d.p.vgrid3 & kVg3HbOne) && d.p.hoist && d.p.h_jc == 0 && !d.p.t_strip && (d.b.NT == 1 || d.b.NT == 2) &&
+         d.p.colseg && d.p.seg_buf && d.p.preuv_lds && d.p.uv_adv && t.nrhs == t.nstp;
+}
 
 constexpr int kTimedS2dFb = 13;
 constexpr int kTimedPreUvSeg = 14, kTimedUv1Seg = 15, kTimedStep3dTSeg = 16;
diff --git a/ucla-roms_amd/csrc/roms_shim.cpp b/ucla-roms_amd/csrc/roms_shim.cpp
--- a/ucla-roms_amd/csrc/roms_shim.cpp
+++ b/ucla-roms_amd/csrc/roms_shim.cpp
@@ -109,7 +109,7 @@
 }
 void vg_set(bool valid) {
   g.vgrid_valid = valid;
-  g.d.p.vg = valid ? (short)(g.d.p.vgrid | (g.d.p.vgrid2 << kVg2Shift)) : (short)0;
+  g.d.p.vg = valid ? (short)(g.d.p.vgrid | ((g.d.p.vgrid3 & kVg3Seg) << kVg3Shift) | (g.d.p.vgrid2 << kVg2Shift)) : (short)0;
 }
 void vg_host_write(int id) {
   if (id != ROMS_Hz && id != ROMS_z_r && id != ROMS_z_w && id != ROMS_h && id != ROMS_hinv && id != ROMS_Cs_w &&
@@ -756,6 +756,7 @@
   P.kpp_fckeep = (short)env_int("ROMS_GPU_KPP_FCKEEP", kKppFcKeepMax, 1, kKppFcKeepMax);
   P.vgrid = (short)env_int("ROMS_GPU_VGRID", kVgDefault, 0, kVgAll);
   P.vgrid2 = env_int("ROMS_GPU_VGRID2", kVg2Default, 0, kVg2All);
+  P.vgrid3 = env_int("ROMS_GPU_VGRID3", kVg3Default, 0, kVg3All);
   P.vg = 0;
   g.vgrid_valid = false;
   P.hoist = !env_off("ROMS_GPU_HOIST");
@@ -1017,6 +1018,11 @@
 int roms_gpu_vgrid2(void) {
   REQUIRE_INIT_NOJOIN();
   return g.d.p.vgrid2 + (g.vgrid_valid ? 256 : 0);
+}
+
+int roms_gpu_vgrid3(void) {
+  REQUIRE_INIT_NOJOIN();
+  return g.d.p.vgrid3 + (g.vgrid_valid ? 256 : 0);
 }
 
 int roms_gpu_vgrid_check(long out[3]) {
diff --git a/ucla-roms_amd/romsgpu/__init__.py b/ucla-roms_amd/romsgpu/__init__.py
--- a/ucla-roms_amd/romsgpu/__init__.py
+++ b/ucla-roms_amd/romsgpu/__init__.py
@@ -492,6 +492,11 @@
         self._chk(min(r, 0), "vgrid2")
         return r % 256, bool(r // 256)
 
+    def vgrid3(self):
+        r = self.L.roms_gpu_vgrid3()
+        self._chk(min(r, 0), "vgrid3")
+        return r % 256, bool(r // 256)
+
     def vgrid_mismatch(self):
         out = (ctypes.c_long * 3)()
         self._chk(self.L.roms_gpu_vgrid_check(out), "vgrid_check")
```

Result: no change. 2.400 billion cell-updates/s, median of 6 (+0.8%).
